# acids-ircam/RAVE

Measured on AMD Instinct MI355X. Metric: audio samples/sec/GPU (RAVE v2 training step, 44.1 kHz, n_signal=65536), higher is better.
Workload: dtype f32; 1 GPU; v2 config, batch 32 mono 44.1 kHz n_signal=65536, VAE-phase training step per GPU (--phase vae); global_batch=32, parallelism=dp1, phase=vae

## Files before the change

### include/rave_hip.h

```cpp
#ifndef RAVE_HIP_H
#define RAVE_HIP_H

#include <stddef.h>
#include <stdint.h>

#ifdef __cplusplus
extern "C" {
#endif

#define RH_VERSION 100

#define RH_OK 0
#define RH_ERR_INVALID (-1)
#define RH_ERR_UNSUPPORTED (-2)
#define RH_ERR_WORKSPACE (-3)

typedef void* rh_stream_t;

enum rh_act {
    RH_ACT_NONE = 0,
    RH_ACT_LEAKY = 1,
    RH_ACT_SNAKE = 2
};

typedef struct rh_conv1d_desc {
    int32_t batch;
    int32_t c_in;
    int32_t c_out;
    int32_t l_in;
    int32_t l_out;
    int32_t kernel;
    int32_t stride;
    int32_t dilation;
    int32_t pad_left;
    int32_t transposed;
    int32_t groups;
    int32_t inner;
    int32_t in_valid;
    int32_t act;
    float act_slope;
    int32_t out_act;
    float out_slope;
} rh_conv1d_desc;

int rh_version(void);
const char* rh_last_error(void);



int rh_weight_norm_fwd_f32(const float* v, const float* g, int64_t rows, int64_t cols, float* w,
                           float* norms, rh_stream_t stream);
int rh_weight_norm_bwd_f32(const float* dw, const float* v, const float* g, const float* norms,
                           int64_t rows, int64_t cols, float* dv, float* dg, rh_stream_t stream);
typedef struct rh_wn_bwd_item {
    const float* dw;
    const float* v;
    const float* g;
    const float* norms;
    float* dv;
    float* dg;
    int64_t rows;
    int64_t cols;
} rh_wn_bwd_item;
int rh_weight_norm_bwd_batched_f32(const rh_wn_bwd_item* items, int32_t n_items, rh_stream_t stream);
typedef struct rh_reduce_item {
    const float* part;
    float* out;
    int64_t n;
    int32_t Z;
    int32_t reserved;
} rh_reduce_item;
int rh_defer_reduce(rh_reduce_item* item);
int rh_reduce_partials_batched_f32(const rh_reduce_item* items, int32_t n_items, rh_stream_t stream);

int64_t rh_conv1d_packed_floats(const rh_conv1d_desc* d, int which);
int rh_conv1d_pack_f32(const rh_conv1d_desc* d, const float* w, float* wp_fwd, float* wp_bwd,
                       rh_stream_t stream);

int rh_conv1d_pack_wn_f32(const rh_conv1d_desc* d, const float* v, const float* g, float* norms,
                          float* scale, float* wp_fwd, float* wp_bwd, rh_stream_t stream);

int64_t rh_prep_item_bytes(void);
int64_t rh_prep_array_bytes(int32_t n);
int rh_prep_fill_item(const rh_conv1d_desc* d, const float* v, const float* g, float* norms, float* scale,
                      float* wp_fwd, float* wp_bwd, void* item_host);
int rh_prep_link(void* items_host, int32_t n, int64_t* total_rows, int64_t* total_blocks);
int rh_prep_run_f32(const void* items_dev, int32_t n, int64_t total_rows, int64_t total_blocks, rh_stream_t stream);


int rh_conv1d_fwd_f32(const rh_conv1d_desc* d, const float* x, const float* wp_fwd,
                      const float* bias, const float* snake_alpha, const float* residual,
                      float* y, void* workspace, int64_t workspace_bytes, rh_stream_t stream);
int64_t rh_conv1d_fwd_workspace_bytes(const rh_conv1d_desc* d);
int64_t rh_conv1d_bwd_data_workspace_bytes(const rh_conv1d_desc* d);
int rh_conv1d_kernel_family(const rh_conv1d_desc* d, int which, int has_bias, int has_add);
int rh_residual_unit_fused(const rh_conv1d_desc* d3, const rh_conv1d_desc* d1);
int rh_residual_unit_fwd_f32(const rh_conv1d_desc* d3, const rh_conv1d_desc* d1, const float* x, const float* wp3_fwd,
                             const float* wp1_fwd, float* h, float* y, rh_stream_t stream);

int rh_x6_uses_ranges(void);
int rh_x6_range_words(void);
int rh_x6_set_ranges(const uint32_t* in_a, const uint32_t* in_b, uint32_t* out, uint32_t* out2);
int rh_amax_f32(const float* x, int64_t n, uint32_t* slot, rh_stream_t stream);

int rh_conv1d_plan_info(const rh_conv1d_desc* d, int which, int has_bias, int has_add, int32_t* out8);
int rh_conv1d_bwd_weight_kernel_family(const rh_conv1d_desc* d);
int rh_conv1d_bwd_weight_plan_info(const rh_conv1d_desc* d, int32_t* out4);

int rh_conv1d_bwd_data_f32(const rh_conv1d_desc* d, const float* dy, const float* wp_bwd,
                           const float* x, const float* snake_alpha, const float* add, float* dx,
                           void* workspace, int64_t workspace_bytes, rh_stream_t stream);

int64_t rh_conv1d_workspace_bytes(const rh_conv1d_desc* d);
int rh_conv1d_bwd_weight_f32(const rh_conv1d_desc* d, const float* dy, const float* x,
                             const float* snake_alpha, float* dw, float* dbias, void* workspace,
                             int64_t workspace_bytes, rh_stream_t stream);
int rh_conv1d_bwd_weight_wn_f32(const rh_conv1d_desc* d, const float* dy, const float* x, const float* snake_alpha,
                                const float* v, const float* g, const float* norms, float* dw_scratch, float* dv,
                                float* dg, float* dbias, void* workspace, int64_t workspace_bytes, rh_stream_t stream);
int64_t rh_conv1d_bwd_weight_wn_fused_launches(void);


int rh_pqmf_analysis_fwd_f32(const float* x, const float* w, int32_t rows, int32_t t_len,
                             int32_t n_band, int32_t kernel, int32_t pad_left, int32_t n_frames,
                             float* y, rh_stream_t stream);
int rh_pqmf_analysis_bwd_f32(const float* dy, const float* w, int32_t rows, int32_t t_len,
                             int32_t n_band, int32_t kernel, int32_t pad_left, int32_t n_frames,
                             float* dx, rh_stream_t stream);
int rh_pqmf_synthesis_fwd_f32(const float* y, const float* w, int32_t rows, int32_t n_frames,
                              int32_t n_band, int32_t kernel, int32_t pad_left, int32_t n_out,
                              float* x, rh_stream_t stream);
int rh_pqmf_synthesis_bwd_f32(const float* dx, const float* w, int32_t rows, int32_t n_frames,
                              int32_t n_band, int32_t kernel, int32_t pad_left, int32_t n_out,
                              float* dy, rh_stream_t stream);

int rh_pqmf_fold_k1_f32(const float* in, const float* tab, int32_t rows, int32_t t_len, int32_t n_frames, int32_t o0,
                        float scale, float* out, rh_stream_t stream);
int rh_pqmf_fold_k2_f32(const float* in, const float* tab, int32_t rows, int32_t n_frames, int32_t n_out, int32_t dp,
                        float scale, float* out, rh_stream_t stream);


int rh_amp_tanh_fwd_f32(const float* x, int32_t batch, int32_t c, int32_t l, float* y,
                        rh_stream_t stream);
int rh_amp_tanh_bwd_f32(const float* dy, const float* x, int32_t batch, int32_t c, int32_t l,
                        float* dx, rh_stream_t stream);
int rh_act_fwd_f32(const float* x, const float* snake_alpha, int32_t act, float slope,
                   int32_t batch, int32_t c, int32_t l, float* y, rh_stream_t stream);
int64_t rh_snake_bwd_workspace_bytes(int32_t batch, int32_t c);
int rh_snake_bwd_f32(const float* dy, const float* x, const float* alpha, int32_t batch, int32_t c,
                     int32_t l, float* dx, float* dalpha, void* workspace, int64_t workspace_bytes,
                     rh_stream_t stream);
int rh_act_bwd_f32(const float* dy, const float* y, int32_t act, float slope, int64_t n, float* g, rh_stream_t stream);
int64_t rh_act_bwd_bias_workspace_bytes(int32_t M);
int rh_act_bwd_bias_f32(const float* dy, const float* y, int32_t act, float slope, int32_t B, int32_t M, int64_t plane, float* g,
                        float* dbias, void* workspace, int64_t workspace_bytes, rh_stream_t stream);
int rh_adain_stats_update_f32(const float* x, int64_t rows, int32_t l, const float* num_updates, float* mean_buf,
                              float* std_buf, rh_stream_t stream);
int rh_adain_transfer_f32(const float* x, int64_t rows, int32_t l, const float* mean_x, const float* std_x,
                          const float* mean_y, const float* std_y, float* y, rh_stream_t stream);
int rh_avgpool2_fwd_f32(const float* x, int64_t rows, int32_t l_in, float* y, rh_stream_t stream);
int rh_avgpool2_bwd_f32(const float* dy, int64_t rows, int32_t l_in, float* dx, rh_stream_t stream);


typedef struct rh_conv2d_desc {
    int32_t batch;
    int32_t c_in;
    int32_t c_out;
    int32_t h_in, w_in;
    int32_t h_out, w_out;
    int32_t kh, kw;
    int32_t sh, sw;
    int32_t dh, dw;
    int32_t ph, pw;
    int32_t act;
    float act_slope;
} rh_conv2d_desc;

int64_t rh_conv2d_packed_floats(const rh_conv2d_desc* d, int which);
int rh_conv2d_pack_f32(const rh_conv2d_desc* d, const float* w, float* wp_fwd, float* wp_bwd, rh_stream_t stream);
int rh_conv2d_fwd_f32(const rh_conv2d_desc* d, const float* x, const float* wp_fwd, const float* bias ,
                      float* y, rh_stream_t stream);
int rh_conv2d_bwd_data_f32(const rh_conv2d_desc* d, const float* dy, const float* y, const float* wp_bwd, float* dx,
                           rh_stream_t stream);
int rh_conv2d_plan_info(const rh_conv2d_desc* d, int32_t which, int64_t* out);
int rh_conv2d_bwd_weight_kernel_family(const rh_conv2d_desc* d);
int64_t rh_conv2d_workspace_bytes(const rh_conv2d_desc* d);
int rh_conv2d_bwd_weight_f32(const rh_conv2d_desc* d, const float* dy, const float* y, const float* x, float* dw,
                             float* dbias, void* workspace, int64_t workspace_bytes, rh_stream_t stream);


int64_t rh_vq_loss_partials(int64_t n_vectors);
int rh_vq_assign_f32(const float* x, const float* embed, int64_t n_vectors, int32_t dim, int32_t codebook_size,
                     int64_t* indices, float* residual, float* quantized_sum, float* loss_partials, rh_stream_t stream);
int64_t rh_vq_assign_workspace_bytes(int64_t n_vectors, int32_t dim, int32_t codebook_size);
int rh_vq_assign_ws_f32(const float* x, const float* embed, int64_t n_vectors, int32_t dim, int32_t codebook_size,
                        int64_t* indices, float* residual, float* quantized_sum, float* loss_partials, void* workspace,
                        int64_t workspace_bytes, rh_stream_t stream);
int rh_vq_ema_update_f32(const float* x, const int64_t* indices, int64_t n_vectors, int32_t dim, int32_t codebook_size,
                         float decay, float epsilon, float* cluster_size, float* embed_avg, float* embed,
                         rh_stream_t stream);


int rh_feed_batch_i16_f32(const int16_t* pcm, const int64_t* src_offset, const double* coef, const float* noise,
                          int32_t rows, int32_t n_signal, int32_t bit_depth, float* out, rh_stream_t stream);

typedef struct rh_feed_pitch_row {
    int64_t base;
    int64_t in_point;
    double mean;
    double coef[5];
    int32_t length;
    int32_t up, down;
    int32_t tap_offset;
    int32_t mute;
    int32_t reserved;
} rh_feed_pitch_row;
int rh_feed_batch_pitch_i16_f32(const int16_t* pcm, int64_t pcm_samples, const rh_feed_pitch_row* rows,
                                const rh_feed_pitch_row* rows_dev, const double* taps, int32_t n_taps, const float* noise,
                                int32_t n_rows, int32_t n_signal, int32_t bit_depth, float* out, rh_stream_t stream);


int rh_stft_frame_fwd_f32(const float* x, const float* window, int64_t rows, int32_t t_len, int32_t n_fft,
                          int32_t hop, int32_t n_frames, float* frames, rh_stream_t stream);
int rh_stft_frame_bwd_f32(const float* dframes, const float* window, int64_t rows, int32_t t_len, int32_t n_fft,
                          int32_t hop, int32_t n_frames, float* dx, rh_stream_t stream);
int rh_stft_frame_bwd_acc_f32(const float* dframes, const float* window, int64_t rows, int32_t t_len, int32_t n_fft,
                              int32_t hop, int32_t n_frames, float* dx, int32_t accumulate, rh_stream_t stream);

int64_t rh_spectral_distance_workspace_bytes(void);
int rh_spectral_distance_fwd_f32(const float* sx, const float* sy, int64_t n_complex, float eps, float* sums,
                                 void* workspace, int64_t workspace_bytes, rh_stream_t stream);
int rh_spectral_distance_bwd_f32(const float* sx, const float* sy, const float* sums, const float* grad_out,
                                 int64_t n_complex, float eps, float* dsx, float* dsy, int32_t half_bins,
                                 rh_stream_t stream);

int rh_spectral_total_f32(const float* sums, const float* inv_n, int32_t n_scales, float* out, rh_stream_t stream);

int rh_stft_loss_supported(int32_t n_fft, int32_t hop, int32_t t_len, int64_t rows);
int rh_stft_loss_plan_info(int32_t n_fft, int32_t t_len, int64_t rows, int64_t* out6);
int64_t rh_stft_loss_workspace_bytes(int32_t n_fft, int32_t t_len, int64_t rows);
int rh_stft_loss_fwd_f32(const float* x, const float* y, const float* window, const float* twiddle, int64_t rows,
                         int32_t t_len, int32_t n_fft, float eps, float* sums, void* workspace, int64_t workspace_bytes,
                         rh_stream_t stream);
int rh_stft_loss_finalize_all_f32(const float* const* partials, const int64_t* partial_bytes, int32_t n_scales,
                                  const float* inv_n, float* sums, float* total, rh_stream_t stream);
int rh_stft_loss_bwd_f32(const float* x, const float* y, const float* window, const float* twiddle, int64_t rows,
                         int32_t t_len, int32_t n_fft, float eps, const float* sums, const float* grad_out, float* dx,
                         float* dy, int32_t accumulate, rh_stream_t stream);

int rh_mel_supported(int32_t n_fft, int32_t hop, int32_t n_mels, int32_t t_len, int64_t rows);
int rh_mel_fwd_f32(const float* x, const float* window, const float* twiddle, const float* fb, const int32_t* bins,
                   int64_t rows, int32_t t_len, int32_t n_fft, int32_t hop, int32_t n_mels, int32_t n_frames, float scale,
                   int32_t log1p, float* y, rh_stream_t stream);

int rh_set_kernel_events(void* start_event, void* stop_event);
int rh_kernel_events_used(void);
int rh_event_create(void** event);
int rh_event_destroy(void* event);
int rh_event_elapsed_ms(void* start_event, void* stop_event, float* ms);

typedef struct rh_loss_item {
    const float* value;
    const float* w1_dev;
    float w1;
    float w2;
} rh_loss_item;
int rh_loss_combine_fwd_f32(const rh_loss_item* items, int32_t n_items, float* scaled, float* total, rh_stream_t stream);
int rh_loss_combine_bwd_f32(const rh_loss_item* items, int32_t n_items, const float* grad_total, float* grads,
                            rh_stream_t stream);

typedef struct rh_adam_item {
    float* p;
    const float* g;
    float* m;
    float* v;
    int64_t n;
    float* step;
} rh_adam_item;
int rh_adam_step_f32(const rh_adam_item* items, int32_t n_items, const float* lr, float beta1, float beta2, float eps,
                     float* aux, rh_stream_t stream);

typedef struct rh_pair_item {
    float* a;
    float* b;
    int64_t n;
} rh_pair_item;
int rh_ema_update_f32(const rh_pair_item* items, int32_t n_items, double factor, rh_stream_t stream);
int rh_swap_f32(const rh_pair_item* items, int32_t n_items, rh_stream_t stream);

typedef struct rh_gru_item {
    const float* w_ih;
    const float* w_hh;
    const float* b_ih;
    const float* b_hh;
    float* dw_ih;
    float* dw_hh;
    float* db_ih;
    float* db_hh;
} rh_gru_item;
int rh_gru_supported(int32_t hidden, int32_t layers);
int rh_gru_workspace_bytes(int32_t batch, int32_t hidden, int32_t t_len, int32_t layers, int32_t training, int64_t* bytes);
int rh_gru_fwd_f32(const float* x, const rh_gru_item* layers, int32_t n_layers, int32_t batch, int32_t hidden, int32_t t_len,
                   int32_t training, float* y, void* workspace, int64_t workspace_bytes, rh_stream_t stream);
int rh_gru_bwd_f32(const float* dy, const float* x, const rh_gru_item* layers, int32_t n_layers, int32_t batch, int32_t hidden,
                   int32_t t_len, float* dx, void* workspace, int64_t workspace_bytes, rh_stream_t stream);

typedef struct rh_fm_item {
    const float* f;
    float* df;
    int64_t half;
    float w;
} rh_fm_item;
int64_t rh_feature_matching_workspace_bytes(const rh_fm_item* items, int32_t n_items);
int rh_feature_matching_fwd_f32(const rh_fm_item* items, int32_t n_items, int32_t relative, void* workspace,
                                int64_t workspace_bytes, float* sums, float* out, rh_stream_t stream);
int rh_feature_matching_bwd_f32(const rh_fm_item* items, int32_t n_items, int32_t relative, const float* sums,
                                const float* grad_out, rh_stream_t stream);

int64_t rh_reparam_workspace_bytes(void);
int rh_reparam_fwd_f32(const float* z, const float* eps, int32_t batch, int32_t c, int32_t l, float* zs, float* kl,
                       void* workspace, int64_t workspace_bytes, rh_stream_t stream);
int rh_reparam_bwd_f32(const float* z, const float* eps, const float* dzs, const float* dkl, int32_t batch, int32_t c,
                       int32_t l, float* dz, rh_stream_t stream);

#ifdef __cplusplus
}
#endif
#endif
```

### rave_amd/_lib.py

```python
from __future__ import annotations

import ctypes as C
import os

import torch

_HERE = os.path.dirname(os.path.abspath(__file__))
LIB_PATH = os.environ.get("RAVE_HIP_LIB") or os.path.join(_HERE, "librave_hip.so")

ACT_NONE, ACT_LEAKY, ACT_SNAKE = 0, 1, 2


class ConvDesc(C.Structure):
    _fields_ = [
        ("batch", C.c_int32), ("c_in", C.c_int32), ("c_out", C.c_int32),
        ("l_in", C.c_int32), ("l_out", C.c_int32), ("kernel", C.c_int32),
        ("stride", C.c_int32), ("dilation", C.c_int32), ("pad_left", C.c_int32),
        ("transposed", C.c_int32), ("groups", C.c_int32), ("inner", C.c_int32),
        ("in_valid", C.c_int32), ("act", C.c_int32), ("act_slope", C.c_float),
        ("out_act", C.c_int32), ("out_slope", C.c_float),
    ]


class AdamItem(C.Structure):
    _fields_ = [("p", C.c_void_p), ("g", C.c_void_p), ("m", C.c_void_p), ("v", C.c_void_p), ("n", C.c_int64), ("step", C.c_void_p)]


class PairItem(C.Structure):
    _fields_ = [("a", C.c_void_p), ("b", C.c_void_p), ("n", C.c_int64)]


class GruItem(C.Structure):
    _fields_ = [(n, C.c_void_p) for n in ("w_ih", "w_hh", "b_ih", "b_hh", "dw_ih", "dw_hh", "db_ih", "db_hh")]


class WnBwdItem(C.Structure):
    _fields_ = [("dw", C.c_void_p), ("v", C.c_void_p), ("g", C.c_void_p), ("norms", C.c_void_p), ("dv", C.c_void_p),
                ("dg", C.c_void_p), ("rows", C.c_int64), ("cols", C.c_int64)]


class ReduceItem(C.Structure):
    _fields_ = [("part", C.c_void_p), ("out", C.c_void_p), ("n", C.c_int64), ("Z", C.c_int32), ("reserved", C.c_int32)]


class LossItem(C.Structure):
    _fields_ = [("value", C.c_void_p), ("w1_dev", C.c_void_p), ("w1", C.c_float), ("w2", C.c_float)]


class FmItem(C.Structure):
    _fields_ = [("f", C.c_void_p), ("df", C.c_void_p), ("half", C.c_int64), ("w", C.c_float)]


class Conv2dDesc(C.Structure):
    _fields_ = [(n, C.c_int32) for n in (
        "batch", "c_in", "c_out", "h_in", "w_in", "h_out", "w_out", "kh", "kw", "sh", "sw", "dh", "dw", "ph", "pw",
        "act")] + [("act_slope", C.c_float)]


def _load() -> C.CDLL:
    if not os.path.exists(LIB_PATH):
        raise RuntimeError(
            f"rave_amd: {LIB_PATH} not found. Build it with `python -m rave_amd.build` "
            "(or __graft_entry__.build()). There is no CPU / PyTorch fallback for the HIP hot path.")
    lib = C.CDLL(LIB_PATH)
    P, I32, I64, F = C.c_void_p, C.c_int32, C.c_int64, C.c_float
    D = C.POINTER(ConvDesc)
    D2 = C.POINTER(Conv2dDesc)
    sig = {
        "rh_version": ([], C.c_int),
        "rh_last_error": ([], C.c_char_p),
        "rh_weight_norm_fwd_f32": ([P, P, I64, I64, P, P, P], C.c_int),
        "rh_weight_norm_bwd_f32": ([P, P, P, P, I64, I64, P, P, P], C.c_int),
        "rh_weight_norm_bwd_batched_f32": ([C.POINTER(WnBwdItem), I32, P], C.c_int),
        "rh_defer_reduce": ([C.POINTER(ReduceItem)], C.c_int),
        "rh_reduce_partials_batched_f32": ([C.POINTER(ReduceItem), I32, P], C.c_int),
        "rh_conv1d_packed_floats": ([D, C.c_int], I64),
        "rh_conv1d_pack_f32": ([D, P, P, P, P], C.c_int),
        "rh_conv1d_pack_wn_f32": ([D, P, P, P, P, P, P, P], C.c_int),
        "rh_prep_item_bytes": ([], I64),
        "rh_prep_array_bytes": ([I32], I64),
        "rh_prep_fill_item": ([D, P, P, P, P, P, P, P], C.c_int),
        "rh_prep_link": ([P, I32, C.POINTER(I64), C.POINTER(I64)], C.c_int),
        "rh_prep_run_f32": ([P, I32, I64, I64, P], C.c_int),
        "rh_conv1d_fwd_f32": ([D, P, P, P, P, P, P, P, I64, P], C.c_int),
        "rh_conv1d_bwd_data_f32": ([D, P, P, P, P, P, P, P, I64, P], C.c_int),
        "rh_conv1d_kernel_family": ([D, C.c_int, C.c_int, C.c_int], C.c_int),
        "rh_conv1d_bwd_weight_kernel_family": ([D], C.c_int),
        "rh_conv1d_bwd_weight_plan_info": ([D, C.POINTER(C.c_int32)], C.c_int),
        "rh_residual_unit_fused": ([D, D], C.c_int),
        "rh_residual_unit_fwd_f32": ([D, D, P, P, P, P, P, P], C.c_int),
        "rh_conv1d_plan_info": ([D, C.c_int, C.c_int, C.c_int, C.POINTER(C.c_int32)], C.c_int),
        "rh_conv1d_fwd_workspace_bytes": ([D], I64),
        "rh_conv1d_bwd_data_workspace_bytes": ([D], I64),
        "rh_conv1d_workspace_bytes": ([D], I64),
        "rh_conv1d_bwd_weight_f32": ([D, P, P, P, P, P, P, I64, P], C.c_int),
        "rh_conv1d_bwd_weight_wn_f32": ([D, P, P, P, P, P, P, P, P, P, P, P, I64, P], C.c_int),
        "rh_conv1d_bwd_weight_wn_fused_launches": ([], I64),
        "rh_conv2d_packed_floats": ([D2, C.c_int], I64),
        "rh_conv2d_pack_f32": ([D2, P, P, P, P], C.c_int),
        "rh_conv2d_fwd_f32": ([D2, P, P, P, P, P], C.c_int),
        "rh_conv2d_bwd_data_f32": ([D2, P, P, P, P, P], C.c_int),
        "rh_conv2d_workspace_bytes": ([D2], I64),
        "rh_conv2d_plan_info": ([D2, I32, C.POINTER(I64)], C.c_int),
        "rh_conv2d_bwd_weight_kernel_family": ([D2], C.c_int),
        "rh_conv2d_bwd_weight_f32": ([D2, P, P, P, P, P, P, I64, P], C.c_int),
        "rh_feed_batch_i16_f32": ([P, P, P, P, I32, I32, I32, P, P], C.c_int),
        "rh_feed_batch_pitch_i16_f32": ([P, I64, P, P, P, I32, P, I32, I32, I32, P, P], C.c_int),
        "rh_vq_loss_partials": ([I64], I64),
        "rh_vq_assign_f32": ([P, P, I64, I32, I32, P, P, P, P, P], C.c_int),
        "rh_vq_assign_workspace_bytes": ([I64, I32, I32], I64),
        "rh_vq_assign_ws_f32": ([P, P, I64, I32, I32, P, P, P, P, P, I64, P], C.c_int),
        "rh_vq_ema_update_f32": ([P, P, I64, I32, I32, F, F, P, P, P, P], C.c_int),
        "rh_pqmf_analysis_fwd_f32": ([P, P, I32, I32, I32, I32, I32, I32, P, P], C.c_int),
        "rh_pqmf_analysis_bwd_f32": ([P, P, I32, I32, I32, I32, I32, I32, P, P], C.c_int),
        "rh_pqmf_synthesis_fwd_f32": ([P, P, I32, I32, I32, I32, I32, I32, P, P], C.c_int),
        "rh_pqmf_synthesis_bwd_f32": ([P, P, I32, I32, I32, I32, I32, I32, P, P], C.c_int),
        "rh_pqmf_fold_k1_f32": ([P, P, I32, I32, I32, I32, F, P, P], C.c_int),
        "rh_pqmf_fold_k2_f32": ([P, P, I32, I32, I32, I32, F, P, P], C.c_int),
        "rh_amp_tanh_fwd_f32": ([P, I32, I32, I32, P, P], C.c_int),
        "rh_amp_tanh_bwd_f32": ([P, P, I32, I32, I32, P, P], C.c_int),
        "rh_act_fwd_f32": ([P, P, I32, F, I32, I32, I32, P, P], C.c_int),
        "rh_act_bwd_f32": ([P, P, I32, F, I64, P, P], C.c_int),
        "rh_act_bwd_bias_workspace_bytes": ([I32], I64),
        "rh_act_bwd_bias_f32": ([P, P, I32, F, I32, I32, I64, P, P, P, I64, P], C.c_int),
        "rh_snake_bwd_workspace_bytes": ([I32, I32], I64),
        "rh_snake_bwd_f32": ([P, P, P, I32, I32, I32, P, P, P, I64, P], C.c_int),
        "rh_stft_frame_fwd_f32": ([P, P, I64, I32, I32, I32, I32, P, P], C.c_int),
        "rh_stft_frame_bwd_f32": ([P, P, I64, I32, I32, I32, I32, P, P], C.c_int),
        "rh_stft_frame_bwd_acc_f32": ([P, P, I64, I32, I32, I32, I32, P, I32, P], C.c_int),
        "rh_spectral_total_f32": ([P, P, I32, P, P], C.c_int),
        "rh_feature_matching_workspace_bytes": ([C.POINTER(FmItem), I32], I64),
        "rh_feature_matching_fwd_f32": ([C.POINTER(FmItem), I32, I32, P, I64, P, P, P], C.c_int),
        "rh_feature_matching_bwd_f32": ([C.POINTER(FmItem), I32, I32, P, P, P], C.c_int),
        "rh_reparam_workspace_bytes": ([], I64),
        "rh_reparam_fwd_f32": ([P, P, I32, I32, I32, P, P, P, I64, P], C.c_int),
        "rh_reparam_bwd_f32": ([P, P, P, P, I32, I32, I32, P, P], C.c_int),
        "rh_loss_combine_fwd_f32": ([C.POINTER(LossItem), I32, P, P, P], C.c_int),
        "rh_loss_combine_bwd_f32": ([C.POINTER(LossItem), I32, P, P, P], C.c_int),
        "rh_adam_step_f32": ([C.POINTER(AdamItem), I32, P, F, F, F, P, P], C.c_int),
        "rh_ema_update_f32": ([C.POINTER(PairItem), I32, C.c_double, P], C.c_int),
        "rh_swap_f32": ([C.POINTER(PairItem), I32, P], C.c_int),
        "rh_gru_supported": ([I32, I32], C.c_int),
        "rh_gru_workspace_bytes": ([I32, I32, I32, I32, I32, C.POINTER(I64)], C.c_int),
        "rh_gru_fwd_f32": ([P, C.POINTER(GruItem), I32, I32, I32, I32, I32, P, P, I64, P], C.c_int),
        "rh_gru_bwd_f32": ([P, P, C.POINTER(GruItem), I32, I32, I32, I32, P, P, I64, P], C.c_int),
        "rh_x6_uses_ranges": ([], C.c_int),
        "rh_x6_range_words": ([], C.c_int),
        "rh_x6_set_ranges": ([P, P, P, P], C.c_int),
        "rh_amax_f32": ([P, I64, P, P], C.c_int),
        "rh_set_kernel_events": ([P, P], C.c_int),
        "rh_kernel_events_used": ([], C.c_int),
        "rh_event_create": ([C.POINTER(C.c_void_p)], C.c_int),
        "rh_event_destroy": ([P], C.c_int),
        "rh_event_elapsed_ms": ([P, P, C.POINTER(C.c_float)], C.c_int),
        "rh_stft_loss_supported": ([I32, I32, I32, I64], C.c_int),
        "rh_stft_loss_plan_info": ([I32, I32, I64, C.POINTER(I64)], C.c_int),
        "rh_stft_loss_workspace_bytes": ([I32, I32, I64], I64),
        "rh_stft_loss_fwd_f32": ([P, P, P, P, I64, I32, I32, F, P, P, I64, P], C.c_int),
        "rh_stft_loss_finalize_all_f32": ([C.POINTER(C.c_void_p), C.POINTER(I64), I32, P, P, P, P], C.c_int),
        "rh_stft_loss_bwd_f32": ([P, P, P, P, I64, I32, I32, F, P, P, P, P, I32, P], C.c_int),
        "rh_mel_supported": ([I32, I32, I32, I32, I64], C.c_int),
        "rh_mel_fwd_f32": ([P, P, P, P, P, I64, I32, I32, I32, I32, I32, F, I32, P, P], C.c_int),
        "rh_spectral_distance_workspace_bytes": ([], I64),
        "rh_spectral_distance_fwd_f32": ([P, P, I64, F, P, P, I64, P], C.c_int),
        "rh_spectral_distance_bwd_f32": ([P, P, P, P, I64, F, P, P, I32, P], C.c_int),
        "rh_adain_stats_update_f32": ([P, I64, I32, P, P, P, P], C.c_int),
        "rh_adain_transfer_f32": ([P, I64, I32, P, P, P, P, P, P], C.c_int),
        "rh_avgpool2_fwd_f32": ([P, I64, I32, P, P], C.c_int),
        "rh_avgpool2_bwd_f32": ([P, I64, I32, P, P], C.c_int),
    }
    for name, (args, res) in sig.items():
        fn = getattr(lib, name)
        fn.argtypes = args
        fn.restype = res
    return lib


lib = _load()


def check(rc: int, what: str = "") -> None:
    if rc != 0:
        msg = lib.rh_last_error().decode(errors="replace")
        raise RuntimeError(f"librave_hip {what} failed (code {rc}): {msg}")


def ptr(t) -> int | None:
    return None if t is None else t.data_ptr()


def stream() -> int:
    return torch.cuda.current_stream().cuda_stream
```

### rave_amd/csrc/conv_host.hip

```cpp
#include "conv_params.hpp"

int64_t rh_wgrad_workspace(const rh_conv1d_desc* d);

namespace {

struct TapPlan {
    int nphase = 0;
    int oph[kMaxPhases], ntaps[kMaxPhases], tap0[kMaxPhases], minoff[kMaxPhases], maxoff[kMaxPhases];
    int nslots = 0;
    int kk[kMaxTaps], off[kMaxTaps];
    int is = 1, os = 1;
    int rows = 0;
    int C = 0, M = 0;
    bool src_m_major = true;
};

int validate(const rh_conv1d_desc* d) {
    RH_REQUIRE(d, RH_ERR_INVALID, "conv1d: null descriptor");
    RH_REQUIRE(d->batch >= 0 && d->c_in > 0 && d->c_out > 0 && d->l_in >= 0 && d->l_out >= 0,
               RH_ERR_INVALID, "conv1d: bad sizes");
    RH_REQUIRE(d->kernel >= 1 && d->stride >= 1 && d->dilation >= 1 && d->inner >= 1,
               RH_ERR_INVALID, "conv1d: kernel/stride/dilation/inner must be >= 1");
    RH_REQUIRE(d->groups == 1, RH_ERR_UNSUPPORTED, "conv1d: groups = %d not implemented", d->groups);
    RH_REQUIRE(d->kernel <= kMaxTaps, RH_ERR_UNSUPPORTED, "conv1d: kernel %d > %d", d->kernel, kMaxTaps);
    RH_REQUIRE(d->act >= RH_ACT_NONE && d->act <= RH_ACT_SNAKE, RH_ERR_INVALID, "conv1d: bad act");
    RH_REQUIRE(d->out_act == RH_ACT_NONE || d->out_act == RH_ACT_LEAKY, RH_ERR_UNSUPPORTED,
               "conv1d: out_act must be none or leaky");
    RH_REQUIRE(d->in_valid >= 0 && d->in_valid <= (int64_t)d->l_in * d->inner, RH_ERR_INVALID,
               "conv1d: in_valid out of range");
    if (d->transposed) {
        RH_REQUIRE(d->dilation == 1 && d->inner == 1, RH_ERR_UNSUPPORTED,
                   "conv_transpose1d: dilation/inner must be 1");
        RH_REQUIRE(d->stride <= kMaxPhases, RH_ERR_UNSUPPORTED, "conv_transpose1d: stride > %d", kMaxPhases);
    } else if (d->stride > 1) {
        RH_REQUIRE(d->stride <= kMaxPhases, RH_ERR_UNSUPPORTED, "conv1d: stride > %d", kMaxPhases);
    }
    return RH_OK;
}

int build_plan(const rh_conv1d_desc* d, int which, TapPlan* tp) {
    TapPlan& t = *tp;
    const int k = d->kernel, s = d->stride, dil = d->dilation, P = d->pad_left;
    auto phases = [&](int pad) {
        t.nphase = s;
        t.is = 1;
        t.os = s;
        for (int ph = 0; ph < s; ++ph) {
            const int r0 = ((ph + pad) % s + s) % s;
            const int base = (ph + pad - r0) / s;
            t.oph[ph] = ph;
            t.tap0[ph] = t.nslots;
            int n = 0;
            for (int m = 0; r0 + m * s < k; ++m, ++n) {
                t.kk[t.nslots] = r0 + m * s;
                t.off[t.nslots] = base - m;
                ++t.nslots;
            }
            t.ntaps[ph] = n;
        }
    };
    auto single = [&]() {
        t.nphase = 1;
        t.oph[0] = 0;
        t.tap0[0] = 0;
        t.ntaps[0] = k;
        t.nslots = k;
    };
    if (which == 0) {
        t.C = d->c_in;
        t.M = d->c_out;
        if (!d->transposed) {
            single();
            for (int i = 0; i < k; ++i) { t.kk[i] = i; t.off[i] = i * dil - P; }
            t.is = s; t.os = 1; t.rows = d->l_out;
            t.src_m_major = true;
        } else {
            phases(P);
            t.rows = rh_cdiv(d->l_out, s);
            t.src_m_major = false;
        }
    } else {
        t.C = d->c_out;
        t.M = d->c_in;
        if (!d->transposed) {
            if (s == 1) {
                single();
                for (int i = 0; i < k; ++i) { t.kk[i] = i; t.off[i] = P - i * dil; }
                t.is = 1; t.os = 1; t.rows = d->l_in;
            } else {
                RH_REQUIRE(dil == 1, RH_ERR_UNSUPPORTED, "conv1d bwd_data: stride > 1 with dilation > 1");
                phases(P);
                t.rows = rh_cdiv(d->l_in, s);
            }
            t.src_m_major = false;
        } else {
            single();
            for (int i = 0; i < k; ++i) { t.kk[i] = i; t.off[i] = i - P; }
            t.is = s; t.os = 1; t.rows = d->l_in;
            t.src_m_major = true;
        }
    }
    for (int ph = 0; ph < t.nphase; ++ph) {
        int lo = 0, hi = 0;
        for (int i = 0; i < t.ntaps[ph]; ++i) {
            const int o = t.off[t.tap0[ph] + i];
            if (i == 0 || o < lo) lo = o;
            if (i == 0 || o > hi) hi = o;
        }
        t.minoff[ph] = lo;
        t.maxoff[ph] = hi;
    }
    return RH_OK;
}

inline int round32(int m) { return (m + 31) & ~31; }

void plan_to_params(const TapPlan& t, ConvP* p) {
    p->C = t.C;
    p->M = t.M;
    p->Mp = round32(t.M);
    p->is = t.is;
    p->os = t.os;
    p->nphase = t.nphase;
    long wofs = 0;
    for (int ph = 0; ph < t.nphase; ++ph) {
        p->ph_oph[ph] = t.oph[ph];
        p->ph_ntaps[ph] = t.ntaps[ph];
        p->ph_tap0[ph] = t.tap0[ph];
        p->ph_minoff[ph] = t.minoff[ph];
        p->ph_maxoff[ph] = t.maxoff[ph];
        p->ph_wofs[ph] = wofs;
        wofs += (long)t.ntaps[ph] * t.C * p->Mp;
    }
    for (int i = 0; i < t.nslots; ++i) p->off[i] = t.off[i];
}

struct VPlan { int s, U, phstar, o0, b0, jof[kMaxPhases]; };
bool vplan_of(const TapPlan& t, int inner, VPlan* v) {
    static const bool on = [] { const char* e = getenv("RH_X6_VROWS"); return !(e && atoi(e) == 0); }();
    const int s = t.nphase;
    if (!on || (s != 2 && s != 4) || t.os != s || t.is != 1 || inner != 1 || (t.C & 15) || ((t.M * s) & 31)) return false;
    int U = 0;
    for (int ph = 0; ph < s; ++ph) {
        if (t.ntaps[ph] < 1) return false;
        for (int m = 0; m < t.ntaps[ph]; ++m)
            if (t.off[t.tap0[ph] + m] != t.off[t.tap0[ph]] - m) return false;
        U = U > t.ntaps[ph] ? U : t.ntaps[ph];
    }
    const int b0 = t.off[t.tap0[0]];
    int phstar = 0;
    for (int ph = 0; ph < s; ++ph) {
        const int b = t.off[t.tap0[ph]];
        if (b == b0 + 1) { if (!phstar) phstar = ph; }
        else if (b != b0 || phstar) return false;
    }
    v->s = s; v->U = U; v->phstar = phstar; v->b0 = b0;
    v->o0 = phstar ? phstar - s : 0;
    for (int ph = 0; ph < s; ++ph) v->jof[ph] = (ph - phstar + s) % s;
    return true;
}

int x6_mode_of(const TapPlan& t, int inner) {
    return rh_x6_mode(t.C, t.nphase, t.is, inner, t.ntaps[0], t.off, t.kk);
}
long x6_units(const TapPlan& t, int mode, long* ph_ofs = nullptr, int inner = 1, long* vofs = nullptr) {
    const long Mp = round32(t.M);
    if (vofs) *vofs = -1;
    if (mode == 0) return 0;
    if (mode == 1) {
        long u = 0;
        for (int ph = 0; ph < t.nphase; ++ph) {
            if (ph_ofs) ph_ofs[ph] = u;
            u += (long)(t.C >> 4) * t.ntaps[ph] * 2 * kX6P * Mp;
        }
        VPlan v;
        if (vplan_of(t, inner, &v)) {
            if (vofs) *vofs = u;
            u += (long)(t.C >> 4) * v.U * 2 * kX6P * round32(t.M * v.s);
        }
        return u;
    }
    if (ph_ofs) ph_ofs[0] = 0;
    return (long)((t.C * mode) >> 4) * rh_cdiv(t.ntaps[0], mode) * 2 * kX6P * Mp;
}
void plan_to_x6(const TapPlan& t, int inner, ConvP* p) {
    p->x6_mode = x6_mode_of(t, inner);
    long vofs = -1;
    long units = x6_units(t, p->x6_mode, p->ph_q2ofs, inner, &vofs);
    if (units * 4 >= 0x7fffffffl) { p->x6_mode = 0; units = 0; vofs = -1; }
    p->x6_nu = p->x6_mode > 1 ? rh_cdiv(t.ntaps[0], p->x6_mode) : 0;
    p->vs = 0;
    p->v_s = 0;
    if (vofs >= 0) {
        VPlan v;
        vplan_of(t, inner, &v);
        p->v_s = v.s; p->v_q2ofs = vofs;
        p->v_o0 = v.o0; p->v_U = v.U; p->v_b0 = v.b0;
    }
    p->x6_wofs = (long)t.nslots * t.C * round32(t.M);
    p->wq_bytes = units * 16 < 0xffffffffl ? (unsigned)(units * 16) : 0xffffffffu;
}

constexpr int kPackSlots = 4;

__host__ __device__ __forceinline__ long pack_tiles(const PackP& q) {
    return q.total ? (long)(q.Mp / 32) * ((q.C + 31) / 32) : 0;
}

__device__ __forceinline__ void emit_fragment_bf3(const float (&v)[8], unsigned* dst, long piece_stride_u32) {
    typedef unsigned u32x4 __attribute__((ext_vector_type(4)));
    unsigned h[3][8];
#pragma unroll
    for (int i = 0; i < 8; ++i) {
        rh_bf3_split(v[i], h[0][i], h[1][i], h[2][i]);
        h[0][i] &= 0xffff0000u; h[1][i] &= 0xffff0000u; h[2][i] &= 0xffff0000u;
    }
#pragma unroll
    for (int s3 = 0; s3 < 3; ++s3) {
        u32x4 pk;
#pragma unroll
        for (int k = 0; k < 4; ++k) pk[k] = (h[s3][2 * k] >> 16) | h[s3][2 * k + 1];
        *reinterpret_cast<u32x4*>(dst + s3 * piece_stride_u32) = pk;
    }
}
__device__ __forceinline__ void emit_fragment(const float (&v)[8], unsigned* dst, long piece_stride_u32, float sc) {
    typedef unsigned u32x4 __attribute__((ext_vector_type(4)));
#if RH_X6_F16
    u32x4 hi, lo;
#pragma unroll
    for (int k = 0; k < 4; ++k) {
        const rh_h2 h = rh_h2_split(v[2 * k] * sc, v[2 * k + 1] * sc);
        hi[k] = h.hi; lo[k] = h.lo;
    }
    *reinterpret_cast<u32x4*>(dst) = hi;
    *reinterpret_cast<u32x4*>(dst + piece_stride_u32) = lo;
#else
    unsigned h[3][8];
#pragma unroll
    for (int i = 0; i < 8; ++i) {
        rh_bf3_split(v[i], h[0][i], h[1][i], h[2][i]);
        h[0][i] &= 0xffff0000u; h[1][i] &= 0xffff0000u; h[2][i] &= 0xffff0000u;
    }
#pragma unroll
    for (int s3 = 0; s3 < 3; ++s3) {
        u32x4 pk;
#pragma unroll
        for (int k = 0; k < 4; ++k) pk[k] = (h[s3][2 * k] >> 16) | h[s3][2 * k + 1];
        *reinterpret_cast<u32x4*>(dst + s3 * piece_stride_u32) = pk;
    }
#endif
}

__device__ __forceinline__ void pack_tile(const PackP& q, long tile, float* lds , int sg = 0, int sn = 1) {
    const int ct = (q.C + 31) / 32;
    const int c0 = (int)(tile % ct) * 32;
    const int m0 = (int)(tile / ct) * 32;
    const int tid = threadIdx.x;
    float fsc = 1.f;
#if RH_X6_F16
    if (q.wq && !q.bf16x3) {
        int inv;
        fsc = __uint_as_float(rh_x6_scale_bits(q.range[0], &inv));
    }
#endif
    for (int s0 = sg * kPackSlots; s0 < q.nslots; s0 += sn * kPackSlots) {
        const int ns = min(kPackSlots, q.nslots - s0);
        constexpr int U = 8;
        int kks[kPackSlots];
#pragma unroll
        for (int j = 0; j < kPackSlots; ++j) kks[j] = q.kk[min(s0 + j, q.nslots - 1)];
        const int total = ns * 1024;
        for (int e0 = tid; e0 < total; e0 += 256 * U) {
            float v[U], sc[U];
            int dst[U];
#pragma unroll
            for (int u = 0; u < U; ++u) {
                const int e = e0 + 256 * u;
                int sl, r;
                if (ns == 4) { sl = e & 3; r = e >> 2; }
                else if (ns == 3) { r = e / 3; sl = e - 3 * r; }
                else if (ns == 2) { sl = e & 1; r = e >> 1; }
                else { sl = 0; r = e; }
                int cl, ml;
                if (q.m_major) { cl = r & 31; ml = r >> 5; }
                else { ml = r & 31; cl = r >> 5; }
                const int m = m0 + ml, c = c0 + cl;
                const bool in = e < total;
                const bool ok = in && m < q.M && c < q.C;
                const int kk = sl == 0 ? kks[0] : (sl == 1 ? kks[1] : (sl == 2 ? kks[2] : kks[3]));
                const long idx = q.m_major ? ((long)m * q.C + c) * q.k + kk : ((long)c * q.M + m) * q.k + kk;
                v[u] = ok ? q.w[idx] : 0.f;
                sc[u] = (ok && q.scale) ? q.scale[q.m_major ? m : c] : 1.f;
                dst[u] = in ? (sl * 32 + cl) * 33 + ml : -1;
            }
#pragma unroll
            for (int u = 0; u < U; ++u)
                if (dst[u] >= 0) lds[dst[u]] = v[u] * sc[u];
        }
        __syncthreads();
        for (int e = tid; e < ns * 1024; e += 256) {
            const int ml = e & 31, cl = (e >> 5) & 31, sl = e >> 10;
            const int c = c0 + cl;
            if (c < q.C) q.wp[((long)(s0 + sl) * q.C + c) * q.Mp + m0 + ml] = lds[(sl * 32 + cl) * 33 + ml];
        }
        if (q.wq && q.x6_mode == 1) {
            for (int e = tid; e < ns * 128; e += 256) {
                const int ml = e & 31, oct = (e >> 5) & 3, sl = e >> 7;
                const int cb = c0 + oct * 8;
                if (cb >= q.C) continue;
                float v[8];
#pragma unroll
                for (int i = 0; i < 8; ++i) v[i] = lds[(sl * 32 + oct * 8 + i) * 33 + ml];
                const int slot = s0 + sl;
                if (q.bf16x3) {
                    const long unit3 = (long)q.q2a[slot] + (long)(cb >> 4) * q.q2n[slot] + (long)(((cb >> 3) & 1) * 3) * q.Mp + m0 + ml;
                    emit_fragment_bf3(v, q.wq + unit3 * 4, (long)q.Mp * 4);
                    continue;
                }
                const long unit = (long)q.q2a[slot] + (long)(cb >> 4) * q.q2n[slot] + (long)(((cb >> 3) & 1) * kX6P) * q.Mp + m0 + ml;
                emit_fragment(v, q.wq + unit * 4, (long)q.Mp * 4, fsc);
            }
        }
        if (q.wq && q.x6_vs > 1) {
            const int vs = q.x6_vs;
            for (int e = tid; e < ns * 128; e += 256) {
                const int ml = e & 31, oct = (e >> 5) & 3, sl = e >> 7;
                const int cb = c0 + oct * 8;
                const int r = (m0 + ml) * vs + q.q2j[s0 + sl];
                if (cb >= q.C || r >= q.x6_Mvp) continue;
                float v[8];
#pragma unroll
                for (int i = 0; i < 8; ++i) v[i] = lds[(sl * 32 + oct * 8 + i) * 33 + ml];
                const int slot = s0 + sl;
                const long unit = q.x6_vofs + q.vq2a[slot] + (long)(cb >> 4) * q.x6_U * 2 * kX6P * q.x6_Mvp + (long)(((cb >> 3) & 1) * kX6P) * q.x6_Mvp + r;
                emit_fragment(v, q.wq + unit * 4, (long)q.x6_Mvp * 4, fsc);
            }
            if (s0 == 0) {
                const float zero[8] = {0.f, 0.f, 0.f, 0.f, 0.f, 0.f, 0.f, 0.f};
                for (int e = tid; e < q.vz_n * 128; e += 256) {
                    const int ml = e & 31, oct = (e >> 5) & 3, zi = e >> 7;
                    const int cb = c0 + oct * 8;
                    const int r = (m0 + ml) * vs + q.vz_j[zi];
                    if (cb >= q.C || r >= q.x6_Mvp) continue;
                    const long unit = q.x6_vofs + (long)q.vz_u[zi] * 2 * kX6P * q.x6_Mvp + (long)(cb >> 4) * q.x6_U * 2 * kX6P * q.x6_Mvp +
                                      (long)(((cb >> 3) & 1) * kX6P) * q.x6_Mvp + r;
                    emit_fragment(zero, q.wq + unit * 4, (long)q.x6_Mvp * 4, fsc);
                }
            }
        }
        if (q.wq && q.x6_mode > 1) {
            const int IS = q.x6_mode, cpc = 16 / IS, nvc = 32 / cpc;
            const int nug = (ns + IS - 1) / IS;
            for (int e = tid; e < nug * nvc * 64; e += 256) {
                const int ml = e & 31, g = (e >> 5) & 1;
                const int r = e >> 6;
                const int cv = r % nvc, ul = r / nvc;
                const int cbase = c0 + cv * cpc;
                if (cbase >= q.C) continue;
                float v[8];
#pragma unroll
                for (int i = 0; i < 8; ++i) {
                    const int kap = 8 * g + i;
                    const int cl = cv * cpc + kap / IS, sl = ul * IS + kap % IS;
                    v[i] = sl < ns ? lds[(sl * 32 + cl) * 33 + ml] : 0.f;
                }
                const long unit = ((long)(cbase / cpc) * q.x6_nu + (s0 / IS + ul)) * 2 * kX6P * q.Mp + (long)(g * kX6P) * q.Mp + m0 + ml;
                emit_fragment(v, q.wq + unit * 4, (long)q.Mp * 4, fsc);
            }
        }
        __syncthreads();
    }
}

__global__ __launch_bounds__(256) void pack_kernel(const PackP a, const PackP b) {
    __shared__ float lds[kPackSlots * 32 * 33];
    const long t = blockIdx.x;
    const long na = pack_tiles(a);
    if (t < na) pack_tile(a, t, lds, blockIdx.y, gridDim.y);
    else if (t - na < pack_tiles(b)) pack_tile(b, t - na, lds, blockIdx.y, gridDim.y);
}

inline unsigned pack_slot_groups(const PackP& a, const PackP& b, long tiles) {
    if (tiles >= 64) return 1;
    const int ns = a.nslots > b.nslots ? a.nslots : b.nslots;
    const int g = (ns + kPackSlots - 1) / kPackSlots;
    return (unsigned)(g < 1 ? 1 : (g > 8 ? 8 : g));
}

int fill_pack(const rh_conv1d_desc* d, int which, const float* w, const float* scale, float* wp, PackP* p) {
    *p = PackP{};
    if (!wp) return RH_OK;
    TapPlan t;
    if (int e = build_plan(d, which, &t)) return e;
    p->w = w; p->scale = scale; p->wp = wp; p->C = t.C; p->M = t.M; p->Mp = round32(t.M); p->k = d->kernel;
    p->m_major = t.src_m_major ? 1 : 0;
    p->total = (long)t.nslots * t.C * p->Mp;
    p->nslots = t.nslots;
    for (int i = 0; i < t.nslots; ++i) p->kk[i] = t.kk[i];
    const int mode = x6_mode_of(t, d->inner);
    long ph_ofs[kMaxPhases];
    long vofs = -1;
    const long units = x6_units(t, mode, ph_ofs, d->inner, &vofs);
    if (mode && units * 4 < 0x7fffffffl) {
        p->wq = reinterpret_cast<unsigned*>(wp + p->total);
        p->range = p->wq + units * 4;
        p->x6_mode = mode;
        if (vofs >= 0) {
            VPlan v;
            vplan_of(t, d->inner, &v);
            p->x6_vs = v.s;
            p->x6_vofs = vofs;
            p->x6_U = v.U;
            p->x6_Mvp = round32(t.M * v.s);
            bool have[kMaxPhases][kMaxTaps] = {};
            for (int ph = 0; ph < t.nphase; ++ph)
                for (int tl = 0; tl < t.ntaps[ph]; ++tl) {
                    const int slot = t.tap0[ph] + tl;
                    p->vq2a[slot] = tl * 2 * kX6P * p->x6_Mvp;
                    p->q2j[slot] = v.jof[ph];
                    have[v.jof[ph]][tl] = true;
                }
            for (int j = 0; j < v.s; ++j)
                for (int u = 0; u < v.U; ++u)
                    if (!have[j][u]) {
                        RH_REQUIRE(p->vz_n < 2 * kMaxPhases, RH_ERR_UNSUPPORTED, "conv1d_pack: too many empty (phase, tap) pairs");
                        p->vz_j[p->vz_n] = j; p->vz_u[p->vz_n] = u; ++p->vz_n;
                    }
        }
        if (mode == 1) {
            for (int ph = 0; ph < t.nphase; ++ph)
                for (int tl = 0; tl < t.ntaps[ph]; ++tl) {
                    p->q2a[t.tap0[ph] + tl] = (int)(ph_ofs[ph] + (long)tl * 2 * kX6P * p->Mp);
                    p->q2n[t.tap0[ph] + tl] = t.ntaps[ph] * 2 * kX6P * p->Mp;
                }
        } else {
            p->x6_nu = rh_cdiv(t.ntaps[0], mode);
        }
    }
    return RH_OK;
}

__global__ __launch_bounds__(256) void pack_range_kernel(const float* __restrict__ w, const float* __restrict__ scale, long cols,
                                                         unsigned* ra, unsigned* rb) {
    __shared__ float red[8];
    const long r = blockIdx.x;
    const float* wr = w + r * cols;
    float mx = 0.f, sm = 0.f;
    for (long e = threadIdx.x; e < cols; e += 256) { const float a = fabsf(wr[e]); mx = fmaxf(mx, a); sm += a; }
#pragma unroll
    for (int o = 32; o > 0; o >>= 1) { mx = fmaxf(mx, __shfl_down(mx, o, 64)); sm += __shfl_down(sm, o, 64); }
    if ((threadIdx.x & 63) == 0) { red[threadIdx.x >> 6] = mx; red[4 + (threadIdx.x >> 6)] = sm; }
    __syncthreads();
    if (threadIdx.x == 0) {
        const float sc = scale ? fabsf(scale[r]) : 1.f;
        const float m = sc * fmaxf(fmaxf(red[0], red[1]), fmaxf(red[2], red[3]));
        const float l1 = sc * ((red[4] + red[5]) + (red[6] + red[7]));
        if (ra) { atomicMax(ra, __float_as_uint(m)); atomicMax(ra + 1, __float_as_uint(l1)); }
        if (rb) { atomicMax(rb, __float_as_uint(m)); atomicMax(rb + 1, __float_as_uint(l1)); }
    }
}

int pack_both(const rh_conv1d_desc* d, const float* w, const float* scale, float* wp_fwd, float* wp_bwd,
              hipStream_t stream) {
    PackP a, b;
    if (int e = fill_pack(d, 0, w, scale, wp_fwd, &a)) return e;
    if (int e = fill_pack(d, 1, w, scale, wp_bwd, &b)) return e;
    const long tiles = pack_tiles(a) + pack_tiles(b);
    if (tiles == 0) return RH_OK;
    if (a.range || b.range) {
        if (a.range && hipMemsetAsync(a.range, 0, 16, stream) != hipSuccess) return rh_check_launch("conv1d_pack_range");
        if (b.range && hipMemsetAsync(b.range, 0, 16, stream) != hipSuccess) return rh_check_launch("conv1d_pack_range");
        const long rows = d->transposed ? d->c_in : d->c_out;
        const long cols = (long)(d->transposed ? d->c_out : d->c_in) * d->kernel;
        hipLaunchKernelGGL(pack_range_kernel, dim3((unsigned)rows), dim3(256), 0, stream, w, scale, cols, a.range, b.range);
        if (int e = rh_check_launch("conv1d_pack_range")) return e;
    }
    hipLaunchKernelGGL(pack_kernel, dim3((unsigned)tiles, pack_slot_groups(a, b, tiles)), dim3(256), 0, stream, a, b);
    return rh_check_launch("conv1d_pack");
}

}

int rh_pack_launch(const PackP& a, const PackP& b, hipStream_t stream, const char* what, const float* w, long rows, long cols) {
    const long tiles = pack_tiles(a) + pack_tiles(b);
    if (tiles == 0) return RH_OK;
    if (w && (a.range || b.range)) {
        if (a.range && hipMemsetAsync(a.range, 0, 16, stream) != hipSuccess) return rh_check_launch(what);
        if (b.range && hipMemsetAsync(b.range, 0, 16, stream) != hipSuccess) return rh_check_launch(what);
        hipLaunchKernelGGL(pack_range_kernel, dim3((unsigned)rows), dim3(256), 0, stream, w, (const float*)nullptr, cols, a.range, b.range);
        if (int e = rh_check_launch(what)) return e;
    }
    hipLaunchKernelGGL(pack_kernel, dim3((unsigned)tiles, pack_slot_groups(a, b, tiles)), dim3(256), 0, stream, a, b);
    return rh_check_launch(what);
}

int rh_conv_fill_fwd(const rh_conv1d_desc* d, ConvP* p) {
    if (int e = validate(d)) return e;
    TapPlan t;
    if (int e = build_plan(d, 0, &t)) return e;
    plan_to_params(t, p);
    p->B = d->batch;
    p->inner = d->inner;
    const int in_full = d->l_in * d->inner;
    p->in_valid = d->in_valid ? d->in_valid : in_full;
    p->in_row = p->in_valid;
    p->out_row = d->l_out * d->inner;
    p->out_valid = p->out_row;
    p->ncols = t.rows * d->inner;
    p->in_act = d->act;
    p->in_slope = d->act_slope;
    p->epi_act = RH_ACT_NONE;
    p->epi_slope = 0.f;
    p->out_act = d->out_act;
    p->out_slope = d->out_slope;
    plan_to_x6(t, d->inner, p);
    return RH_OK;
}

int rh_conv_fill_dgrad(const rh_conv1d_desc* d, ConvP* p) {
    if (int e = validate(d)) return e;
    TapPlan t;
    if (int e = build_plan(d, 1, &t)) return e;
    plan_to_params(t, p);
    p->B = d->batch;
    p->inner = d->inner;
    p->in_row = d->l_out * d->inner;
    p->in_valid = p->in_row;
    const int x_full = d->l_in * d->inner;
    p->out_valid = d->in_valid ? d->in_valid : x_full;
    p->out_row = p->out_valid;
    p->ncols = t.rows * d->inner;
    p->in_act = RH_ACT_NONE;
    p->in_slope = 0.f;
    p->epi_act = d->act;
    p->epi_slope = d->act_slope;
    p->out_act = RH_ACT_NONE;
    p->out_slope = 0.f;
    plan_to_x6(t, d->inner, p);
    return RH_OK;
}

extern "C" int64_t rh_conv1d_packed_floats(const rh_conv1d_desc* d, int which) {
    if (validate(d)) return -1;
    const int64_t M = which == 0 ? d->c_out : d->c_in;
    const int64_t C = which == 0 ? d->c_in : d->c_out;
    const int64_t n32 = (int64_t)d->kernel * C * round32((int)M);
    TapPlan t;
    if (build_plan(d, which, &t)) return -1;
    const long units = x6_units(t, x6_mode_of(t, d->inner), nullptr, d->inner);
    return (units > 0 && units * 4 < 0x7fffffffl) ? n32 + units * 4 + 4 : n32;
}

extern "C" int rh_conv1d_pack_f32(const rh_conv1d_desc* d, const float* w, float* wp_fwd,
                                  float* wp_bwd, rh_stream_t stream) {
    if (int e = validate(d)) return e;
    RH_REQUIRE(w, RH_ERR_INVALID, "conv1d_pack: null weight");
    return pack_both(d, w, nullptr, wp_fwd, wp_bwd, (hipStream_t)stream);
}

int rh_weight_norm_scales(const float* v, const float* g, int64_t rows, int64_t cols, float* norms, float* scale,
                          hipStream_t stream);

struct PrepItem {
    const float* v;
    const float* g;
    float* norms;
    float* scale;
    PackP fwd, bwd;
    long rows, cols;
    long row_begin;
    long blk_begin;
};

namespace {

__device__ __forceinline__ int find_item(const PrepItem* items, int n, long key, bool rows) {
    const long* tab = reinterpret_cast<const long*>(items + n) + (rows ? 0 : n);
    int lo = 0, hi = n - 1;
    while (lo < hi) {
        const int mid = (lo + hi + 1) >> 1;
        if (tab[mid] <= key) lo = mid; else hi = mid - 1;
    }
    return lo;
}

__global__ __launch_bounds__(256) void prep_range_kernel(const PrepItem* __restrict__ items, int n) {
    __shared__ float red[8];
    const PrepItem& p = items[blockIdx.x];
    float mx = 0.f, l1 = 0.f;
    for (long r = threadIdx.x; r < p.rows; r += 256) { mx = fmaxf(mx, p.scale[p.rows + r]); l1 = fmaxf(l1, p.scale[2 * p.rows + r]); }
#pragma unroll
    for (int o = 32; o > 0; o >>= 1) { mx = fmaxf(mx, __shfl_down(mx, o, 64)); l1 = fmaxf(l1, __shfl_down(l1, o, 64)); }
    if ((threadIdx.x & 63) == 0) { red[threadIdx.x >> 6] = mx; red[4 + (threadIdx.x >> 6)] = l1; }
    __syncthreads();
    if (threadIdx.x == 0) {
        const unsigned m = __float_as_uint(fmaxf(fmaxf(red[0], red[1]), fmaxf(red[2], red[3])));
        const unsigned l = __float_as_uint(fmaxf(fmaxf(red[4], red[5]), fmaxf(red[6], red[7])));
        for (unsigned* r : {p.fwd.range, p.bwd.range})
            if (r) { r[0] = m; r[1] = l; r[2] = 0u; r[3] = 0u; }
    }
}

__global__ __launch_bounds__(256) void prep_scales_kernel(const PrepItem* __restrict__ items, int n) {
    __shared__ float red[12];
    const int it = find_item(items, n, blockIdx.x, true);
    const PrepItem& p = items[it];
    const long r = (long)blockIdx.x - p.row_begin;
    const float* vr = p.v + r * p.cols;
    float s = 0.f, mx = 0.f, sm = 0.f;
    long e = threadIdx.x;
    for (; e + 768 < p.cols; e += 1024) {
        const float a0 = vr[e], a1 = vr[e + 256], a2 = vr[e + 512], a3 = vr[e + 768];
        s += a0 * a0; s += a1 * a1; s += a2 * a2; s += a3 * a3;
        mx = fmaxf(fmaxf(mx, fmaxf(fabsf(a0), fabsf(a1))), fmaxf(fabsf(a2), fabsf(a3)));
        sm += fabsf(a0); sm += fabsf(a1); sm += fabsf(a2); sm += fabsf(a3);
    }
    for (; e < p.cols; e += 256) {
        const float a = vr[e];
        s += a * a;
        mx = fmaxf(mx, fabsf(a));
        sm += fabsf(a);
    }
#pragma unroll
    for (int o = 32; o > 0; o >>= 1) {
        s += __shfl_down(s, o, 64);
        mx = fmaxf(mx, __shfl_down(mx, o, 64));
        sm += __shfl_down(sm, o, 64);
    }
    if ((threadIdx.x & 63) == 0) { red[threadIdx.x >> 6] = s; red[4 + (threadIdx.x >> 6)] = mx; red[8 + (threadIdx.x >> 6)] = sm; }
    __syncthreads();
    if (threadIdx.x == 0) {
        const float norm = sqrtf(red[0] + red[1] + red[2] + red[3]);
        const float sc = p.g[r] / norm;
        p.norms[r] = norm;
        p.scale[r] = sc;
        const float m = fabsf(sc) * fmaxf(fmaxf(red[4], red[5]), fmaxf(red[6], red[7]));
        const float l1 = fabsf(sc) * ((red[8] + red[9]) + (red[10] + red[11]));
        p.scale[p.rows + r] = m;
        p.scale[2 * p.rows + r] = l1;
    }
}

__global__ __launch_bounds__(256) void prep_pack_kernel(const PrepItem* __restrict__ items, int n) {
    __shared__ float lds[kPackSlots * 32 * 33];
    const int it = find_item(items, n, blockIdx.x, false);
    const PrepItem& p = items[it];
    const long t = (long)blockIdx.x - p.blk_begin;
    const long nf = pack_tiles(p.fwd);
    if (t < nf) pack_tile(p.fwd, t, lds);
    else if (t - nf < pack_tiles(p.bwd)) pack_tile(p.bwd, t - nf, lds);
}

}

extern "C" int64_t rh_prep_item_bytes(void) { return (int64_t)sizeof(PrepItem); }
extern "C" int64_t rh_prep_array_bytes(int32_t n) { return (int64_t)n * (int64_t)sizeof(PrepItem) + 2 * (int64_t)n * (int64_t)sizeof(long); }

extern "C" int rh_prep_fill_item(const rh_conv1d_desc* d, const float* v, const float* g, float* norms, float* scale,
                                 float* wp_fwd, float* wp_bwd, void* item) {
    if (int e = validate(d)) return e;
    RH_REQUIRE(v && g && norms && scale && wp_fwd && item, RH_ERR_INVALID, "prep_fill_item: null pointer");
    PrepItem* p = (PrepItem*)item;
    *p = PrepItem{};
    p->v = v; p->g = g; p->norms = norms; p->scale = scale;
    p->rows = d->transposed ? d->c_in : d->c_out;
    p->cols = (long)(d->transposed ? d->c_out : d->c_in) * d->kernel;
    if (int e = fill_pack(d, 0, v, scale, wp_fwd, &p->fwd)) return e;
    if (int e = fill_pack(d, 1, v, scale, wp_bwd, &p->bwd)) return e;
    return RH_OK;
}

extern "C" int rh_prep_link(void* items, int32_t n, int64_t* total_rows, int64_t* total_blocks) {
    RH_REQUIRE(items && total_rows && total_blocks && n >= 0, RH_ERR_INVALID, "prep_link: bad arguments");
    PrepItem* p = (PrepItem*)items;
    long rows = 0, blks = 0;
    for (int i = 0; i < n; ++i) {
        p[i].row_begin = rows;
        p[i].blk_begin = blks;
        rows += p[i].rows;
        for (const PackP* q : {&p[i].fwd, &p[i].bwd}) blks += pack_tiles(*q);
    }
    long* tab = reinterpret_cast<long*>(p + n);
    for (int i = 0; i < n; ++i) { tab[i] = p[i].row_begin; tab[n + i] = p[i].blk_begin; }
    *total_rows = rows;
    *total_blocks = blks;
    return RH_OK;
}

extern "C" int rh_prep_run_f32(const void* items_dev, int32_t n, int64_t total_rows, int64_t total_blocks,
                               rh_stream_t stream) {
    RH_REQUIRE(items_dev && n > 0, RH_ERR_INVALID, "prep_run: bad arguments");
    if (total_rows > 0) {
        hipLaunchKernelGGL(prep_scales_kernel, dim3((unsigned)total_rows), dim3(256), 0, (hipStream_t)stream,
                           (const PrepItem*)items_dev, n);
        if (int e = rh_check_launch("prep_scales")) return e;
        hipLaunchKernelGGL(prep_range_kernel, dim3((unsigned)n), dim3(256), 0, (hipStream_t)stream, (const PrepItem*)items_dev, n);
        if (int e = rh_check_launch("prep_range")) return e;
    }
    if (total_blocks > 0) {
        hipLaunchKernelGGL(prep_pack_kernel, dim3((unsigned)total_blocks), dim3(256), 0, (hipStream_t)stream,
                           (const PrepItem*)items_dev, n);
        return rh_check_launch("prep_pack");
    }
    return RH_OK;
}

extern "C" int rh_conv1d_pack_wn_f32(const rh_conv1d_desc* d, const float* v, const float* g, float* norms,
                                     float* scale, float* wp_fwd, float* wp_bwd, rh_stream_t stream) {
    if (int e = validate(d)) return e;
    RH_REQUIRE(v && g && norms && scale, RH_ERR_INVALID, "conv1d_pack_wn: null pointer");
    const int64_t rows = d->transposed ? d->c_in : d->c_out;
    const int64_t cols = (int64_t)(d->transposed ? d->c_out : d->c_in) * d->kernel;
    if (int e = rh_weight_norm_scales(v, g, rows, cols, norms, scale, (hipStream_t)stream)) return e;
    return pack_both(d, v, scale, wp_fwd, wp_bwd, (hipStream_t)stream);
}

extern "C" int64_t rh_conv1d_fwd_workspace_bytes(const rh_conv1d_desc* d) {
    ConvP p{};
    if (rh_conv_fill_fwd(d, &p)) return -1;
    return rh_conv_splitk_workspace(p);
}

extern "C" int64_t rh_conv1d_bwd_data_workspace_bytes(const rh_conv1d_desc* d) {
    ConvP p{};
    if (rh_conv_fill_dgrad(d, &p)) return -1;
    p.epi_act = d->act;
    return rh_conv_splitk_workspace(p);
}

extern "C" int rh_conv1d_kernel_family(const rh_conv1d_desc* d, int which, int has_bias, int has_add) {
    ConvP p{};
    if (int e = which == 0 ? rh_conv_fill_fwd(d, &p) : rh_conv_fill_dgrad(d, &p)) return e;
    if (which == 0 ? rh_smallc_fwd_eligible(d, has_add != 0) : rh_smallc_dgrad_eligible(d, has_add != 0)) return 2;
    alignas(16) static const float dummy[4] = {0.f, 0.f, 0.f, 0.f};
    p.in = dummy; p.wp = dummy; p.wq = reinterpret_cast<const unsigned*>(dummy);
    p.bias = has_bias ? dummy : nullptr;
    p.add = has_add ? dummy : nullptr;
    p.mul_src = (which == 1 && d->act != RH_ACT_NONE) ? dummy : nullptr;
    if (p.B <= 0 || p.ncols <= 0 || p.M <= 0 || !rh_conv_dma_eligible(p)) return 0;
    return (rh_conv_x6_workspace(p) >= 0 || rh_conv_c2x_query(p)) ? 1 : 0;
}

extern "C" int rh_conv1d_plan_info(const rh_conv1d_desc* d, int which, int has_bias, int has_add, int32_t* out8) {
    RH_REQUIRE(out8, RH_ERR_INVALID, "conv1d_plan_info: null output");
    for (int i = 0; i < 8; ++i) out8[i] = 0;
    ConvP p{};
    if (int e = which == 0 ? rh_conv_fill_fwd(d, &p) : rh_conv_fill_dgrad(d, &p)) return e;
    if (which == 0 ? rh_smallc_fwd_eligible(d, has_add != 0) : rh_smallc_dgrad_eligible(d, has_add != 0)) { out8[0] = 2; return RH_OK; }
    alignas(16) static const float dummy[4] = {0.f, 0.f, 0.f, 0.f};
    p.in = dummy; p.wp = dummy; p.wq = reinterpret_cast<const unsigned*>(dummy);
    p.bias = has_bias ? dummy : nullptr;
    p.add = has_add ? dummy : nullptr;
    p.mul_src = (which == 1 && d->act != RH_ACT_NONE) ? dummy : nullptr;
    if (p.B <= 0 || p.ncols <= 0 || p.M <= 0 || !rh_conv_dma_eligible(p)) return RH_OK;
    int q[7];
    if (rh_conv_x6_plan_query(p, q)) {
        out8[0] = 1;
        for (int i = 0; i < 7; ++i) out8[i + 1] = q[i];
    }
    return RH_OK;
}

extern "C" int rh_conv1d_fwd_f32(const rh_conv1d_desc* d, const float* x, const float* wp_fwd,
                                 const float* bias, const float* snake_alpha, const float* residual,
                                 float* y, void* workspace, int64_t workspace_bytes, rh_stream_t stream) {
    const RhKernelEventsScope events;
    ConvP p{};
    rh_take_ranges(nullptr, &p.in_range, &p.out_range, nullptr);
    const unsigned* const in_range = p.in_range;
    unsigned* const out_range = p.out_range;
    if (int e = rh_conv_fill_fwd(d, &p)) return e;
    p.in_range = in_range; p.out_range = out_range;
    if (d->batch == 0 || d->l_out == 0) return RH_OK;
    RH_REQUIRE(x && wp_fwd && y, RH_ERR_INVALID, "conv1d_fwd: null pointer");
    RH_REQUIRE(d->act != RH_ACT_SNAKE || snake_alpha, RH_ERR_INVALID, "conv1d_fwd: snake needs alpha");
    if (rh_smallc_fwd_eligible(d, residual != nullptr)) {
        return rh_smallc_fwd(d, x, wp_fwd, bias, y, (hipStream_t)stream, p.out_range);
    }
    p.in = x; p.wp = wp_fwd; p.out = y; p.bias = bias; p.add = residual; p.mul_src = nullptr;
    p.wq = reinterpret_cast<const unsigned*>(wp_fwd + p.x6_wofs);
    p.in_alpha = snake_alpha; p.mul_alpha = nullptr;
    return rh_conv_launch(p, (hipStream_t)stream, d->transposed ? "conv_transpose1d_fwd" : "conv1d_fwd", workspace,
                          workspace_bytes);
}

extern "C" int rh_conv1d_bwd_data_f32(const rh_conv1d_desc* d, const float* dy, const float* wp_bwd,
                                      const float* x, const float* snake_alpha, const float* add,
                                      float* dx, void* workspace, int64_t workspace_bytes,
                                      rh_stream_t stream) {
    const RhKernelEventsScope events;
    ConvP p{};
    rh_take_ranges(nullptr, &p.in_range, &p.out_range, nullptr);
    const unsigned* const in_range = p.in_range;
    unsigned* const out_range = p.out_range;
    if (int e = rh_conv_fill_dgrad(d, &p)) return e;
    p.in_range = in_range; p.out_range = out_range;
    if (d->batch == 0 || d->l_in == 0) return RH_OK;
    RH_REQUIRE(dy && wp_bwd && dx, RH_ERR_INVALID, "conv1d_bwd_data: null pointer");
    RH_REQUIRE(d->act == RH_ACT_NONE || x, RH_ERR_INVALID, "conv1d_bwd_data: act needs the forward input");
    RH_REQUIRE(d->act != RH_ACT_SNAKE || snake_alpha, RH_ERR_INVALID, "conv1d_bwd_data: snake needs alpha");
    if (rh_smallc_dgrad_eligible(d, add != nullptr)) {
        TapPlan t;
        if (int e = build_plan(d, 1, &t)) return e;
        int slot_of_tap[kMaxTaps];
        for (int i = 0; i < t.nslots; ++i) slot_of_tap[t.kk[i]] = i;
        if (int e = rh_smallc_dgrad(d, dy, wp_bwd, slot_of_tap, dx, (hipStream_t)stream)) return e;
        p.out = dx;
        return rh_range_after(p, (hipStream_t)stream);
    }
    p.in = dy; p.wp = wp_bwd; p.out = dx; p.bias = nullptr; p.add = add;
    p.wq = reinterpret_cast<const unsigned*>(wp_bwd + p.x6_wofs);
    p.mul_src = d->act == RH_ACT_NONE ? nullptr : x;
    p.in_alpha = nullptr; p.mul_alpha = snake_alpha;
    return rh_conv_launch(p, (hipStream_t)stream, d->transposed ? "conv_transpose1d_bwd_data" : "conv1d_bwd_data",
                          workspace, workspace_bytes);
}

extern "C" int64_t rh_conv1d_workspace_bytes(const rh_conv1d_desc* d) {
    if (validate(d)) return -1;
    return rh_wgrad_workspace(d);
}

extern "C" int rh_conv1d_bwd_weight_f32(const rh_conv1d_desc* d, const float* dy, const float* x,
                                        const float* snake_alpha, float* dw, float* dbias,
                                        void* workspace, int64_t workspace_bytes, rh_stream_t stream) {
    const RhKernelEventsScope events;
    const RhWgradArmed armed = rh_wgrad_take_armed(true);
    if (int e = validate(d)) return e;
    RH_REQUIRE(dw && (d->batch == 0 || (dy && x)), RH_ERR_INVALID, "conv1d_bwd_weight: null pointer");
    RH_REQUIRE(d->act != RH_ACT_SNAKE || snake_alpha, RH_ERR_INVALID, "conv1d_bwd_weight: snake needs alpha");
    return rh_wgrad_run(d, dy, x, snake_alpha, dw, dbias, workspace, workspace_bytes, (hipStream_t)stream, armed);
}

extern "C" int rh_conv1d_bwd_weight_wn_f32(const rh_conv1d_desc* d, const float* dy, const float* x, const float* snake_alpha,
                                           const float* v, const float* g, const float* norms, float* dw_scratch, float* dv,
                                           float* dg, float* dbias, void* workspace, int64_t workspace_bytes, rh_stream_t stream) {
    const RhKernelEventsScope events;
    const RhWgradArmed armed = rh_wgrad_take_armed(false);
    if (int e = validate(d)) return e;
    RH_REQUIRE(dw_scratch && v && g && norms && dv && dg && (d->batch == 0 || (dy && x)), RH_ERR_INVALID,
               "conv1d_bwd_weight_wn: null pointer");
    RH_REQUIRE(d->act != RH_ACT_SNAKE || snake_alpha, RH_ERR_INVALID, "conv1d_bwd_weight_wn: snake needs alpha");
    const RhWnTail tail{v, g, norms, dv, dg};
    return rh_wgrad_run(d, dy, x, snake_alpha, dw_scratch, dbias, workspace, workspace_bytes, (hipStream_t)stream, armed, &tail);
}
```

### rave_amd/csrc/conv_igemm.hip

```cpp
#include <mutex>
#include "conv_params.hpp"

namespace {

__device__ __forceinline__ int ibase_of(int n, int inner, int is) {
    if (inner == 1) return n * is;
    const int r = n / inner;
    return r * is * inner + (n - r * inner);
}
__device__ __forceinline__ int oidx_of(int n, int inner, int os, int oph) {
    if (inner == 1) return n * os + oph;
    const int r = n / inner;
    return (r * os + oph) * inner + (n - r * inner);
}

template <int TM, int TN, int WM, int WN>
__global__ __launch_bounds__(WM* WN * 64) void conv_igemm_kernel(const ConvP p) {
    constexpr int BM = TM * WM * 32;
    constexpr int NT = WM * WN * 64;
    constexpr int NW = WM * WN;
    extern __shared__ __attribute__((aligned(16))) float smem[];
    float* w_lds = smem;
    float* x_lds = smem + p.wlds_floats;

    const int tid = threadIdx.x, lane = tid & 63, wave = tid >> 6;
    const int j = lane & 31, kh = lane >> 5;
    const int wm = wave / WN, wn = wave - wm * WN;

    const int phase = blockIdx.z;
    const int ntaps = p.ph_ntaps[phase];
    const int tap0 = p.ph_tap0[phase];
    const int minoff = p.ph_minoff[phase];
    const int maxoff = p.ph_maxoff[phase];
    const int oph = p.ph_oph[phase];
    const float* __restrict__ wp = p.wp + p.ph_wofs[phase];

    const int bt = blockIdx.x / p.tiles_per_b;
    const int nt = blockIdx.x - bt * p.tiles_per_b;
    const int b0 = bt * p.nb;
    const int n0 = nt * p.bnl;
    const int m0 = blockIdx.y * BM;
    const int inner = p.inner, is = p.is;

    const int nlast = min(n0 + p.bnl, p.ncols) - 1;
    const int ib0 = ibase_of(n0, inner, is);
    const int lo = ib0 + minoff * inner;
    const int width = ibase_of(nlast, inner, is) - ib0 + (maxoff - minoff) * inner + 1;

    int xb[TN];
#pragma unroll
    for (int tn = 0; tn < TN; ++tn) {
        const int col = (wn * TN + tn) * 32 + j;
        const int bl = col >> p.bnl_shift;
        const int nl = col & (p.bnl - 1);
        const int n = min(n0 + nl, p.ncols - 1);
        xb[tn] = (bl * p.ck + kh) * p.pitch + ibase_of(n, inner, is) - ib0;
    }
    const int arow = wm * TM * 32 + j + kh * BM;

    f32x16 acc[TM][TN];
#pragma unroll
    for (int tm = 0; tm < TM; ++tm)
#pragma unroll
        for (int tn = 0; tn < TN; ++tn)
#pragma unroll
            for (int r = 0; r < 16; ++r) acc[tm][tn][r] = 0.f;

    for (int c0 = 0; c0 < p.C; c0 += p.ck) {
        __syncthreads();
        const int nrows = p.nb * p.ck;
        for (int r = wave; r < nrows; r += NW) {
            const int bl = r / p.ck, c = r - bl * p.ck;
            const int b = b0 + bl, ch = c0 + c;
            float* dst = x_lds + r * p.pitch;
            if (b < p.B && ch < p.C) {
                const float* __restrict__ src = p.in + ((long)b * p.C + ch) * p.in_row;
                const float alpha = (p.in_act == RH_ACT_SNAKE) ? p.in_alpha[ch] : 0.f;
                for (int w = lane; w < width; w += 64) {
                    const int f = lo + w;
                    const float v = (f >= 0 && f < p.in_valid) ? src[f] : 0.f;
                    dst[w] = rh_act_apply(v, p.in_act, p.in_slope, alpha);
                }
            } else {
                for (int w = lane; w < width; w += 64) dst[w] = 0.f;
            }
        }
        constexpr int V = BM / 4;
        const int wrows = ntaps * p.ck;
        for (int e = tid; e < wrows * V; e += NT) {
            const int kr = e / V, v4 = e - kr * V;
            const int t = kr / p.ck, c = kr - t * p.ck;
            const int ch = c0 + c;
            const int m = m0 + v4 * 4;
            f32x4 val = {0.f, 0.f, 0.f, 0.f};
            if (ch < p.C && m < p.Mp)
                val = *reinterpret_cast<const f32x4*>(wp + ((long)t * p.C + ch) * p.Mp + m);
            *reinterpret_cast<f32x4*>(w_lds + kr * BM + v4 * 4) = val;
        }
        __syncthreads();
        for (int t = 0; t < ntaps; ++t) {
            const int toff = (p.off[tap0 + t] - minoff) * inner;
            const float* wl = w_lds + t * p.ck * BM + arow;
            const float* xl = x_lds + toff;
            for (int c = 0; c < p.ck; c += 2) {
                float a[TM], b[TN];
#pragma unroll
                for (int tm = 0; tm < TM; ++tm) a[tm] = wl[c * BM + tm * 32];
#pragma unroll
                for (int tn = 0; tn < TN; ++tn) b[tn] = xl[xb[tn] + c * p.pitch];
#pragma unroll
                for (int tm = 0; tm < TM; ++tm)
#pragma unroll
                    for (int tn = 0; tn < TN; ++tn)
                        acc[tm][tn] = __builtin_amdgcn_mfma_f32_32x32x2f32(a[tm], b[tn], acc[tm][tn], 0, 0, 0);
            }
        }
    }

#pragma unroll
    for (int tn = 0; tn < TN; ++tn) {
        const int col = (wn * TN + tn) * 32 + j;
        const int bl = col >> p.bnl_shift;
        const int nl = col & (p.bnl - 1);
        const int n = n0 + nl, b = b0 + bl;
        if (n >= p.ncols || b >= p.B) continue;
        const int oi = oidx_of(n, inner, p.os, oph);
        if (oi >= p.out_valid) continue;
#pragma unroll
        for (int tm = 0; tm < TM; ++tm) {
#pragma unroll
            for (int r = 0; r < 16; ++r) {
                const int m = m0 + (wm * TM + tm) * 32 + (r & 3) + 8 * (r >> 2) + 4 * kh;
                if (m < p.M) {
                    const long idx = ((long)b * p.M + m) * p.out_row + oi;
                    float v = acc[tm][tn][r];
                    if (p.bias) v += p.bias[m];
                    if (p.mul_src) {
                        const float al = (p.epi_act == RH_ACT_SNAKE) ? p.mul_alpha[m] : 0.f;
                        v *= rh_act_grad(p.mul_src[idx], p.epi_act, p.epi_slope, al);
                    }
                    if (p.add) v += p.add[idx];
                    if (p.out_act == RH_ACT_LEAKY) v = v > 0.f ? v : v * p.out_slope;
                    p.out[idx] = v;
                }
            }
        }
    }
}

template <int TM, int TN, int WM, int WN>
int launch_cfg(ConvP& p, hipStream_t stream, const char* what) {
    constexpr int BM = TM * WM * 32, BN = TN * WN * 32;
    int bnl = BN;
    if (p.ncols < BN) {
        bnl = 32;
        while (bnl < p.ncols) bnl <<= 1;
    }
    p.bnl = bnl;
    p.bnl_shift = __builtin_ctz(bnl);
    p.nb = BN / bnl;
    p.tiles_per_b = rh_cdiv(p.ncols, bnl);
    int span = 0, maxtaps = 0;
    for (int i = 0; i < p.nphase; ++i) {
        span = span > p.ph_maxoff[i] - p.ph_minoff[i] ? span : p.ph_maxoff[i] - p.ph_minoff[i];
        maxtaps = maxtaps > p.ph_ntaps[i] ? maxtaps : p.ph_ntaps[i];
    }
    if (p.inner == 1)
        p.pitch = (bnl - 1) * p.is + span + 1;
    else
        p.pitch = ((bnl - 1) / p.inner + 1) * p.is * p.inner + p.inner + span * p.inner + 1;
    p.pitch |= 1;
    const int budget = 15 * 1024;
    const int per_ch = (maxtaps > 0 ? maxtaps : 1) * BM + p.nb * p.pitch;
    int ck = budget / per_ch;
    ck &= ~1;
    if (ck > 32) ck = 32;
    if (ck < 2) ck = 2;
    const int cmax = (p.C + 1) & ~1;
    if (ck > cmax) ck = cmax;
    p.ck = ck;
    p.wlds_floats = (maxtaps > 0 ? maxtaps : 1) * ck * BM;
    const size_t lds = sizeof(float) * ((size_t)p.wlds_floats + (size_t)p.nb * ck * p.pitch);
    RH_REQUIRE(lds <= 160 * 1024, RH_ERR_UNSUPPORTED, "%s: tile needs %zu B of LDS", what, lds);
    auto kern = conv_igemm_kernel<TM, TN, WM, WN>;
    static std::once_flag once;
    std::call_once(once, [&] {
        (void)hipFuncSetAttribute(reinterpret_cast<const void*>(kern),
                                  hipFuncAttributeMaxDynamicSharedMemorySize, 160 * 1024);
    });
    dim3 grid(rh_cdiv(p.B, p.nb) * p.tiles_per_b, rh_cdiv(p.M, BM), p.nphase);
    hipLaunchKernelGGL(kern, grid, dim3(WM * WN * 64), lds, stream, p);
    return rh_check_launch(what);
}

}

int rh_conv_launch(ConvP& p, hipStream_t stream, const char* what, void* ws, int64_t ws_bytes) {
    if (p.B <= 0 || p.ncols <= 0 || p.M <= 0) return RH_OK;
    if (rh_conv_dma_eligible(p)) return rh_conv_launch_dma(p, stream, what, ws, ws_bytes);
    return rh_conv_launch_sync(p, stream, what);
}

int rh_conv_launch_sync(ConvP& p, hipStream_t stream, const char* what) {
    if (p.B <= 0 || p.ncols <= 0 || p.M <= 0) return RH_OK;
    int rc;
    if (p.M <= 32) rc = launch_cfg<1, 2, 1, 4>(p, stream, what);
    else if (p.M <= 64) rc = launch_cfg<2, 1, 1, 4>(p, stream, what);
    else if (p.M % 96 == 0 || p.M < 96) rc = launch_cfg<3, 1, 1, 4>(p, stream, what);
    else rc = launch_cfg<2, 2, 2, 2>(p, stream, what);
    return rc ? rc : rh_range_after(p, stream);
}

int rh_range_after(const ConvP& p, hipStream_t stream) {
    if (!p.out_range) return RH_OK;
    return rh_amax_f32(p.out, (int64_t)p.B * (p.Mr > 0 && p.vs > 1 ? p.Mr : p.M) * p.out_row, p.out_range, (rh_stream_t)stream);
}
```

### rave_amd/csrc/conv_igemm_dma.hip

```cpp
#include <cstdlib>
#include <mutex>
#include <type_traits>
#include "conv_params.hpp"

namespace {

typedef __attribute__((address_space(3))) void lds_void;

#ifndef RH_READS_FIRST
#define RH_READS_FIRST 1
#endif
constexpr bool READS_FIRST = RH_READS_FIRST != 0;

__device__ __forceinline__ int ibase_of(int n, int inner, int is) {
    if (inner == 1) return n * is;
    const int r = n / inner;
    return r * is * inner + (n - r * inner);
}
__device__ __forceinline__ int oidx_of(int n, int inner, int os, int oph) {
    if (inner == 1) return n * os + oph;
    const int r = n / inner;
    return (r * os + oph) * inner + (n - r * inner);
}
__device__ __forceinline__ unsigned mdiv(unsigned n, unsigned magic) { return (n * magic) >> 20; }

constexpr unsigned kOOB = 0x80000000u;

template <int TM, int TN, int WM, int WN, bool LEAKY, bool VEC, bool CTAIL>
__global__ __launch_bounds__(WM* WN * 64) void conv_igemm_dma_kernel(const ConvP p) {
    constexpr int BM = TM * WM * 32;
    constexpr int NW = WM * WN;
    extern __shared__ __attribute__((aligned(16))) float smem[];

    const int tid = threadIdx.x, lane = tid & 63;
    const int wave = __builtin_amdgcn_readfirstlane(tid >> 6);
    const int j = lane & 31, kh = lane >> 5;
    const int wm = wave / WN, wn = wave - wm * WN;

    const int zsl = blockIdx.z / p.nphase;
    const int phase = blockIdx.z - zsl * p.nphase;
    const int ntaps = p.ph_ntaps[phase];
    const int tap0 = p.ph_tap0[phase];
    const int minoff = p.ph_minoff[phase];
    const int oph = p.ph_oph[phase];
    const unsigned wofs = (unsigned)p.ph_wofs[phase];

    const int bt = blockIdx.x / p.tiles_per_b;
    const int nt = blockIdx.x - bt * p.tiles_per_b;
    const int b0 = bt * p.nb;
    const int n0 = nt * p.bnl;
    const int m0 = blockIdx.y * BM;
    const int inner = p.inner, is = p.is;
    const int pitch = VEC ? p.pitch : p.segs * 64;
    const int ib0 = ibase_of(n0, inner, is);
    const int lo_raw = ib0 + minoff * inner;
    const int lo = VEC ? lo_raw - ((lo_raw % 4 + 4) % 4) : lo_raw;

    const auto in_rsrc = __builtin_amdgcn_make_buffer_rsrc(const_cast<float*>(p.in), 0, p.in_bytes, 0x00020000);
    const auto w_rsrc = __builtin_amdgcn_make_buffer_rsrc(const_cast<float*>(p.wp), 0, p.w_bytes, 0x00020000);

    int xb[TN];
#pragma unroll
    for (int tn = 0; tn < TN; ++tn) {
        const int col = (wn * TN + tn) * 32 + j;
        const int bl = col >> p.bnl_shift;
        const int nl = col & (p.bnl - 1);
        const int n = min(n0 + nl, p.ncols - 1);
        xb[tn] = (bl * p.ck + kh) * pitch + ibase_of(n, inner, is) - ib0 + (lo_raw - lo);
    }
    const int arow = wm * TM * 32 + j + kh * BM;

    f32x16 acc[TM][TN];
#pragma unroll
    for (int tm = 0; tm < TM; ++tm)
#pragma unroll
        for (int tn = 0; tn < TN; ++tn)
#pragma unroll
            for (int r = 0; r < 16; ++r) acc[tm][tn][r] = 0.f;

    const int wrows = ntaps * p.ck;
    const int w_instrs = (wrows * BM + 255) >> 8;
    const int xrows = p.nb * p.ck;

    constexpr int kNX = 8, kNWS = 10;
    unsigned xo[VEC ? kNX : 1], xc[VEC && CTAIL ? kNX : 1], wo[VEC ? kNWS : 1], wc[VEC && CTAIL ? kNWS : 1];
    unsigned long long vm[TN];
    bool bnd = false;
    int nx = 0, nws = 0, x_floats = 0;
    if constexpr (VEC) {
        const int lpr = pitch >> 2;
        x_floats = xrows * pitch;
        nx = (xrows * lpr + 64 * NW - 1) / (64 * NW);
        nws = (w_instrs + NW - 1) / NW;
        bnd = lo < 0 || lo + 4 * lpr > p.in_valid;
#pragma unroll
        for (int i = 0; i < kNX; ++i) {
            const unsigned g = (unsigned)(wave + NW * i) * 64u + lane;
            const unsigned row = mdiv(g, p.magic_lpr);
            const unsigned v = g - row * lpr;
            const unsigned bl = mdiv(row, p.magic_ck);
            const unsigned c = row - bl * p.ck;
            const bool ok = row < (unsigned)xrows && b0 + bl < (unsigned)p.B;
            xo[i] = ok ? (bl * p.C + c) * (unsigned)p.in_row + 4u * v : kOOB;
            if (CTAIL) xc[i] = c;
        }
#pragma unroll
        for (int i = 0; i < kNWS; ++i) {
            const unsigned f = ((unsigned)(wave + NW * i) * 64u + lane) * 4u;
            const unsigned kr = f / (unsigned)BM;
            const unsigned col = f - kr * BM;
            const unsigned t = mdiv(kr, p.magic_ck);
            const unsigned c = kr - t * p.ck;
            const bool ok = kr < (unsigned)wrows && m0 + col < (unsigned)p.Mp;
            wo[i] = ok ? (t * p.C + c) * p.Mp + m0 + col : kOOB;
            if (CTAIL) wc[i] = c;
        }
#pragma unroll
        for (int tn = 0; tn < TN; ++tn) {
            const int col = (wn * TN + tn) * 32 + j;
            const int nl = col & (p.bnl - 1);
            const int n = min(n0 + nl, p.ncols - 1);
            unsigned long long m = 0;
            for (int t = 0; t < ntaps; ++t) {
                const int f = n * is + p.off[tap0 + t];
                if (f >= 0 && f < p.in_valid) m |= 1ull << t;
            }
            vm[tn] = m;
        }
    }

    auto issue = [&](int c0, float* stage) {
        if constexpr (VEC) {
            const unsigned wbase = wofs + (unsigned)c0 * p.Mp;
#pragma unroll
            for (int i = 0; i < kNWS; ++i) {
                if (i < nws && (wave + NW * i) < w_instrs) {
                    bool dead = wo[i] == kOOB;
                    if (CTAIL) dead = dead || c0 + wc[i] >= (unsigned)p.C;
                    const unsigned off = dead ? kOOB : (wbase + wo[i]) * 4u;
                    __builtin_amdgcn_raw_ptr_buffer_load_lds(w_rsrc, (lds_void*)(stage + (wave + NW * i) * 256), 16, off, 0, 0, 0);
                }
            }
            float* xs = stage + p.wlds_floats;
            const unsigned xbase = ((unsigned)b0 * p.C + (unsigned)c0) * (unsigned)p.in_row + (unsigned)lo;
#pragma unroll
            for (int i = 0; i < kNX; ++i) {
                if (i < nx && (wave + NW * i) * 256 < x_floats) {
                    bool dead = xo[i] == kOOB;
                    if (CTAIL) dead = dead || c0 + xc[i] >= (unsigned)p.C;
                    const unsigned off = dead ? kOOB : (xbase + xo[i]) * 4u;
                    __builtin_amdgcn_raw_ptr_buffer_load_lds(in_rsrc, (lds_void*)(xs + (wave + NW * i) * 256), 16, off, 0, 0, 0);
                }
            }
            return;
        }
        for (int q = wave; q < w_instrs; q += NW) {
            const unsigned f = (unsigned)q * 256u + (unsigned)lane * 4u;
            const unsigned kr = f / (unsigned)BM;
            const unsigned col = f - kr * BM;
            const unsigned t = mdiv(kr, p.magic_ck);
            const unsigned c = kr - t * p.ck;
            const unsigned ch = c0 + c, m = m0 + col;
            unsigned off = kOOB;
            if (kr < (unsigned)wrows && ch < (unsigned)p.C && m < (unsigned)p.Mp)
                off = (wofs + (t * p.C + ch) * p.Mp + m) * 4u;
            __builtin_amdgcn_raw_ptr_buffer_load_lds(w_rsrc, (lds_void*)(stage + q * 256), 16, off, 0, 0, 0);
        }
        float* xs = stage + p.wlds_floats;
        for (int row = wave; row < xrows; row += NW) {
            const unsigned bl = mdiv((unsigned)row, p.magic_ck);
            const unsigned c = row - bl * p.ck;
            const unsigned b = b0 + bl, ch = c0 + c;
            const bool rv = b < (unsigned)p.B && ch < (unsigned)p.C;
            const unsigned rbase = (b * p.C + ch) * (unsigned)p.in_row;
            float* dst = xs + row * pitch;
            for (int seg = 0; seg < p.segs; ++seg) {
                const int fpos = lo + seg * 64 + lane;
                unsigned off = kOOB;
                if (rv && fpos >= 0 && fpos < p.in_valid) off = (rbase + (unsigned)fpos) * 4u;
                __builtin_amdgcn_raw_ptr_buffer_load_lds(in_rsrc, (lds_void*)(dst + seg * 64), 4, off, 0, 0, 0);
            }
        }
    };

    const int total_chunks = (p.C + p.ck - 1) / p.ck;
    const int chunk0 = zsl * p.chunks_per_split;
    const int nchunks = min(p.chunks_per_split, total_chunks - chunk0);
    issue(chunk0 * p.ck, smem);
    for (int i = 0; i < nchunks; ++i) {
        asm volatile("s_waitcnt vmcnt(0)" ::: "memory");
        __syncthreads();
        if (i + 1 < nchunks) issue((chunk0 + i + 1) * p.ck, smem + ((i + 1) & 1) * p.stage_floats);
        const float* w_lds = smem + (i & 1) * p.stage_floats;
        const float* x_lds = w_lds + p.wlds_floats;
        for (int t = 0; t < ntaps; ++t) {
            const int toff = (p.off[tap0 + t] - minoff) * inner;
            const float* wl = w_lds + t * p.ck * BM + arow;
            const float* xl = x_lds + toff;
            bool keep[TN];
#pragma unroll
            for (int tn = 0; tn < TN; ++tn) keep[tn] = !(VEC && bnd) || ((vm[tn] >> t) & 1ull);
            int c = 0;
            for (; c + 8 <= p.ck; c += 8) {
                float a[4][TM], b[4][TN];
#pragma unroll
                for (int u = 0; u < 4; ++u) {
#pragma unroll
                    for (int tm = 0; tm < TM; ++tm) a[u][tm] = wl[(c + 2 * u) * BM + tm * 32];
#pragma unroll
                    for (int tn = 0; tn < TN; ++tn) b[u][tn] = xl[xb[tn] + (c + 2 * u) * pitch];
                }
                if (READS_FIRST) __builtin_amdgcn_sched_barrier(0);
#pragma unroll
                for (int u = 0; u < 4; ++u) {
#pragma unroll
                    for (int tn = 0; tn < TN; ++tn) {
                        float v = b[u][tn];
                        if (VEC) v = keep[tn] ? v : 0.f;
                        if (LEAKY) v = v > 0.f ? v : v * p.in_slope;
                        b[u][tn] = v;
                    }
#pragma unroll
                    for (int tm = 0; tm < TM; ++tm)
#pragma unroll
                        for (int tn = 0; tn < TN; ++tn)
                            acc[tm][tn] = __builtin_amdgcn_mfma_f32_32x32x2f32(a[u][tm], b[u][tn], acc[tm][tn], 0, 0, 0);
                }
                if (READS_FIRST) __builtin_amdgcn_sched_barrier(0);
            }
            for (; c < p.ck; c += 2) {
                float a[TM], b[TN];
#pragma unroll
                for (int tm = 0; tm < TM; ++tm) a[tm] = wl[c * BM + tm * 32];
#pragma unroll
                for (int tn = 0; tn < TN; ++tn) {
                    float v = xl[xb[tn] + c * pitch];
                    if (VEC) v = keep[tn] ? v : 0.f;
                    if (LEAKY) v = v > 0.f ? v : v * p.in_slope;
                    b[tn] = v;
                }
#pragma unroll
                for (int tm = 0; tm < TM; ++tm)
#pragma unroll
                    for (int tn = 0; tn < TN; ++tn)
                        acc[tm][tn] = __builtin_amdgcn_mfma_f32_32x32x2f32(a[tm], b[tn], acc[tm][tn], 0, 0, 0);
            }
        }
    }

    const bool full = m0 + BM <= p.M;
#pragma unroll
    for (int tn = 0; tn < TN; ++tn) {
        const int col = (wn * TN + tn) * 32 + j;
        const int bl = col >> p.bnl_shift;
        const int nl = col & (p.bnl - 1);
        const int n = n0 + nl, b = b0 + bl;
        if (n >= p.ncols || b >= p.B) continue;
        const int oi = oidx_of(n, inner, p.os, oph);
        if (oi >= p.out_valid) continue;
        const long cbase = (long)b * p.M * p.out_row + oi;
        float* __restrict__ outp = (p.ksplit > 1 ? p.part + (long)zsl * p.part_stride : p.out) + cbase;
        const float* __restrict__ mulp = p.mul_src ? p.mul_src + cbase : nullptr;
        const float* __restrict__ addp = p.add ? p.add + cbase : nullptr;
#pragma unroll
        for (int tm = 0; tm < TM; ++tm) {
            const int mb = m0 + (wm * TM + tm) * 32 + 4 * kh;
#pragma unroll
            for (int r = 0; r < 16; ++r) {
                const int m = mb + (r & 3) + 8 * (r >> 2);
                if (full || m < p.M) {
                    const int ro = m * p.out_row;
                    float v = acc[tm][tn][r];
                    if (p.ksplit > 1) {
                        outp[ro] = v;
                        continue;
                    }
                    if (p.bias) v += p.bias[m];
                    if (mulp) {
                        const float al = (p.epi_act == RH_ACT_SNAKE) ? p.mul_alpha[m] : 0.f;
                        v *= rh_act_grad(mulp[ro], p.epi_act, p.epi_slope, al);
                    }
                    if (addp) v += addp[ro];
                    if (p.out_act == RH_ACT_LEAKY) v = v > 0.f ? v : v * p.out_slope;
                    outp[ro] = v;
                }
            }
        }
    }
}

unsigned magic_of(int d) { return (unsigned)(((1u << 20) + d - 1) / d); }

__global__ __launch_bounds__(256) void splitk_finalize_kernel(const ConvP p, long total) {
    float mx = 0.f;
    for (long e = (long)blockIdx.x * 256 + threadIdx.x; e < total; e += (long)gridDim.x * 256) {
        const long row = e / p.out_valid;
        const int oi = (int)(e - row * p.out_valid);
        const int m = (int)(row % p.M);
        const long idx = row * p.out_row + oi;
        float v = 0.f;
        for (int z = 0; z < p.ksplit; ++z) v += p.part[(long)z * p.part_stride + idx];
        if (p.bias) v += p.bias[m];
        if (p.mul_src) {
            const float al = (p.epi_act == RH_ACT_SNAKE) ? p.mul_alpha[m] : 0.f;
            v *= rh_act_grad(p.mul_src[idx], p.epi_act, p.epi_slope, al);
        }
        if (p.add) v += p.add[idx];
        if (p.out_act == RH_ACT_LEAKY) v = v > 0.f ? v : v * p.out_slope;
        p.out[idx] = v;
        mx = rh_absmax(mx, v);
    }
    if (p.out_range) {
        __shared__ float red[4];
        rh_range_publish(p.out_range, mx, blockIdx.x, red);
    }
}

__global__ __launch_bounds__(256) void splitk_finalize4_kernel(const ConvP p, long total4) {
    float mx = 0.f;
    for (long t = (long)blockIdx.x * 256 + threadIdx.x; t < total4; t += (long)gridDim.x * 256) {
        const long e = 4 * t;
        const long row = e / p.out_valid;
        const int oi = (int)(e - row * p.out_valid);
        const int m = (int)(row % p.M);
        const long idx = row * p.out_row + oi;
        f32x4 v = {0.f, 0.f, 0.f, 0.f};
        for (int z = 0; z < p.ksplit; ++z) {
            const f32x4 q = *reinterpret_cast<const f32x4*>(p.part + (long)z * p.part_stride + idx);
#pragma unroll
            for (int i = 0; i < 4; ++i) v[i] += q[i];
        }
        if (p.bias) {
            const float b = p.bias[m];
#pragma unroll
            for (int i = 0; i < 4; ++i) v[i] += b;
        }
        if (p.mul_src) {
            const float al = (p.epi_act == RH_ACT_SNAKE) ? p.mul_alpha[m] : 0.f;
            const f32x4 q = *reinterpret_cast<const f32x4*>(p.mul_src + idx);
#pragma unroll
            for (int i = 0; i < 4; ++i) v[i] *= rh_act_grad(q[i], p.epi_act, p.epi_slope, al);
        }
        if (p.add) {
            const f32x4 q = *reinterpret_cast<const f32x4*>(p.add + idx);
#pragma unroll
            for (int i = 0; i < 4; ++i) v[i] += q[i];
        }
        if (p.out_act == RH_ACT_LEAKY) {
#pragma unroll
            for (int i = 0; i < 4; ++i) v[i] = v[i] > 0.f ? v[i] : v[i] * p.out_slope;
        }
        *reinterpret_cast<f32x4*>(p.out + idx) = v;
        mx = rh_absmax(rh_absmax(mx, v[0]), v[1]); mx = rh_absmax(rh_absmax(mx, v[2]), v[3]);
    }
    if (p.out_range) {
        __shared__ float red[4];
        rh_range_publish(p.out_range, mx, blockIdx.x, red);
    }
}

int finalize_launch(const ConvP& p, hipStream_t stream) {
    const long total = (long)p.B * p.M * p.out_valid;
    const bool vec = (p.out_valid & 3) == 0 && (p.out_row & 3) == 0 && (p.part_stride & 3) == 0 &&
                     (((uintptr_t)p.part | (uintptr_t)p.out | (uintptr_t)p.mul_src | (uintptr_t)p.add) & 15) == 0;
    const long items = vec ? total / 4 : total;
    long blocks = rh_cdiv64(items, 256);
    if (p.out_range && blocks > 4096) blocks = 4096;
    if (vec) hipLaunchKernelGGL(splitk_finalize4_kernel, dim3((unsigned)blocks), dim3(256), 0, stream, p, items);
    else hipLaunchKernelGGL(splitk_finalize_kernel, dim3((unsigned)blocks), dim3(256), 0, stream, p, items);
    return rh_check_launch("conv_splitk_finalize");
}

struct Plan { int blocks, total_chunks, ksplit, chunks_per_split; };

Plan plan_split(const ConvP& p, int BM, int col_tiles) {
    Plan pl{};
    pl.blocks = col_tiles * rh_cdiv(p.M, BM) * p.nphase;
    pl.total_chunks = rh_cdiv(p.C, p.ck);
    static const int split_below = [] { const char* e = getenv("RH_CONV_SPLIT_BELOW"); return e ? atoi(e) : 512; }();
    static const int split_target = [] { const char* e = getenv("RH_CONV_SPLIT_TARGET"); return e ? atoi(e) : 768; }();
    int z = 1;
    if (pl.blocks < split_below) {
        z = rh_cdiv(split_target, pl.blocks);
        const int zmax = pl.total_chunks / 2;
        if (z > zmax) z = zmax;
        if (z > 16) z = 16;
        if (z < 1) z = 1;
    }
    pl.chunks_per_split = rh_cdiv(pl.total_chunks, z);
    pl.ksplit = rh_cdiv(pl.total_chunks, pl.chunks_per_split);
    return pl;
}

template <int TM, int TN, int WM, int WN>
int launch_dma(ConvP& p, hipStream_t stream, const char* what, void* ws, int64_t ws_bytes, bool plan_only = false,
               int64_t* want = nullptr) {
    constexpr int BM = TM * WM * 32, BN = TN * WN * 32;
    int bnl = BN;
    if (p.ncols < BN) {
        bnl = 32;
        while (bnl < p.ncols) bnl <<= 1;
    }
    p.bnl = bnl;
    p.bnl_shift = __builtin_ctz(bnl);
    p.nb = BN / bnl;
    p.tiles_per_b = rh_cdiv(p.ncols, bnl);
    int span = 0, maxtaps = 1;
    for (int i = 0; i < p.nphase; ++i) {
        span = span > p.ph_maxoff[i] - p.ph_minoff[i] ? span : p.ph_maxoff[i] - p.ph_minoff[i];
        maxtaps = maxtaps > p.ph_ntaps[i] ? maxtaps : p.ph_ntaps[i];
    }
    int width;
    if (p.inner == 1)
        width = (bnl - 1) * p.is + span + 1;
    else
        width = ((bnl - 1) / p.inner + 1) * p.is * p.inner + p.inner + span * p.inner + 1;
    static const int novec = [] { const char* e = getenv("RH_CONV_NOVEC"); return e ? atoi(e) : 0; }();
    bool vec = !novec && p.inner == 1 && maxtaps <= 64 && (p.in_row % 4) == 0 && ((uintptr_t)p.in % 16) == 0 &&
               ((uintptr_t)p.wp % 16) == 0;
    static const int budget_env = [] { const char* e = getenv("RH_CONV_STAGE_FLOATS"); return e ? atoi(e) : 0; }();
    int ck = 2;
    for (int attempt = 0; attempt < 2; ++attempt) {
        p.segs = rh_cdiv(width, 64);
        p.pitch = vec ? ((width + 3 + 3) & ~3) : p.segs * 64;
        const int per_ch = maxtaps * BM + p.nb * p.pitch;
        int budget = budget_env > 0 ? budget_env : (p.C >= 192 ? 6 * 1024 : 5 * 1024);
        ck = ((budget - 512) / per_ch) & ~1;
        if (budget_env <= 0 && ck < (p.C >= 192 ? 4 : 8)) {
            budget = 10 * 1024;
            ck = ((budget - 512) / per_ch) & ~1;
        }
        if (ck > 32) ck = 32;
        if (ck < 2) ck = 2;
        const int cmax = (p.C + 1) & ~1;
        if (ck > cmax) ck = cmax;
        if (!vec) break;
        const int nx = rh_cdiv(p.nb * ck * (p.pitch >> 2), 64 * WM * WN);
        const int nws = rh_cdiv(rh_cdiv(maxtaps * ck * BM, 256), WM * WN);
        if (nx <= 8 && nws <= 10) break;
        vec = false;
    }
    p.ck = ck;
    p.wlds_floats = (maxtaps * ck * BM + 255) & ~255;
    p.stage_floats = p.wlds_floats + ((p.nb * ck * p.pitch + 255) & ~255);
    p.magic_segs = magic_of(p.segs);
    p.magic_ck = magic_of(ck);
    p.magic_lpr = magic_of(p.pitch >> 2);
    const size_t lds = sizeof(float) * 2 * (size_t)p.stage_floats;
    const int col_tiles = rh_cdiv(p.B, p.nb) * p.tiles_per_b;
    Plan pl = plan_split(p, BM, col_tiles);
    p.part_stride = (long)p.B * p.M * p.out_row;
    const int64_t need = pl.ksplit > 1 ? (int64_t)pl.ksplit * p.part_stride * (int64_t)sizeof(float) : 0;
    if (plan_only) {
        *want = lds > 160 * 1024 ? 0 : need;
        return RH_OK;
    }
    if (lds > 160 * 1024) return rh_conv_launch_sync(p, stream, what);
    if (need > 0 && (!ws || ws_bytes < need)) {
        pl.ksplit = 1;
        pl.chunks_per_split = pl.total_chunks;
    }
    p.ksplit = pl.ksplit;
    p.chunks_per_split = pl.chunks_per_split;
    p.part = (float*)ws;
    auto launch = [&](auto kern) {
        dim3 grid(col_tiles, rh_cdiv(p.M, BM), p.nphase * p.ksplit);
        rh_launch_main(kern, grid, dim3(WM * WN * 64), lds, stream, p);
    };
    auto go = [&](auto kern) {
        static std::once_flag once;
        std::call_once(once, [&] { (void)hipFuncSetAttribute(reinterpret_cast<const void*>(kern), hipFuncAttributeMaxDynamicSharedMemorySize, 160 * 1024); });
        launch(kern);
    };
    const bool leaky = p.in_act == RH_ACT_LEAKY;
    const bool ctail = (p.C % p.ck) != 0;
    if (vec && !ctail) {
        if (leaky) go(conv_igemm_dma_kernel<TM, TN, WM, WN, true, true, false>);
        else go(conv_igemm_dma_kernel<TM, TN, WM, WN, false, true, false>);
    } else if (vec) {
        if (leaky) go(conv_igemm_dma_kernel<TM, TN, WM, WN, true, true, true>);
        else go(conv_igemm_dma_kernel<TM, TN, WM, WN, false, true, true>);
    } else {
        if (leaky) go(conv_igemm_dma_kernel<TM, TN, WM, WN, true, false, true>);
        else go(conv_igemm_dma_kernel<TM, TN, WM, WN, false, false, true>);
    }
    if (int e = rh_check_launch(what)) return e;
    if (p.ksplit > 1) return finalize_launch(p, stream);
    return RH_OK;
}

void fill_sizes(ConvP& p) {
    unsigned long long wtaps = 0;
    for (int i = 0; i < p.nphase; ++i) wtaps += p.ph_ntaps[i];
    p.in_bytes = (unsigned)(4ull * p.B * p.C * (unsigned long long)p.in_row);
    p.w_bytes = (unsigned)(4ull * wtaps * p.C * p.Mp);
}

}

bool rh_conv_dma_eligible(const ConvP& p) {
    if (p.in_act == RH_ACT_SNAKE) return false;
    const unsigned long long in_b = 4ull * p.B * p.C * (unsigned long long)p.in_row;
    unsigned long long wtaps = 0;
    for (int i = 0; i < p.nphase; ++i) wtaps += p.ph_ntaps[i];
    const unsigned long long w_b = 4ull * wtaps * p.C * p.Mp;
    const unsigned long long row_span = (unsigned long long)p.M * (unsigned long long)p.out_row;
    return in_b < 0x7fffffffull && w_b < 0x7fffffffull && row_span < 0x7fffffffull;
}

int rh_splitk_finalize_launch(ConvP& p, hipStream_t stream) { return finalize_launch(p, stream); }

int rh_conv_launch_dma(ConvP& p, hipStream_t stream, const char* what, void* ws, int64_t ws_bytes) {
    fill_sizes(p);
    {
        bool used = false;
        if (int e = rh_conv_launch_x6(p, stream, what, ws, ws_bytes, &used)) return e;
        if (used) return RH_OK;
        if (int e = rh_conv_launch_c2x(p, stream, what, &used)) return e;
        if (used) return rh_range_after(p, stream);
    }
    unsigned* const orange = p.out_range;
    p.out_range = nullptr;
    int rc;
    if (p.M <= 32) rc = launch_dma<1, 2, 1, 4>(p, stream, what, ws, ws_bytes);
    else if (p.M <= 64) rc = launch_dma<2, 1, 1, 4>(p, stream, what, ws, ws_bytes);
    else if (p.M % 96 == 0 || p.M < 96) rc = launch_dma<3, 1, 1, 4>(p, stream, what, ws, ws_bytes);
    else rc = launch_dma<2, 2, 2, 2>(p, stream, what, ws, ws_bytes);
    p.out_range = orange;
    return rc ? rc : rh_range_after(p, stream);
}

int64_t rh_conv_splitk_workspace(ConvP p) {
    if (p.B <= 0 || p.ncols <= 0 || p.M <= 0 || !rh_conv_dma_eligible(p)) return 0;
    fill_sizes(p);
    int64_t want = 0;
    const int64_t x6 = rh_conv_x6_workspace(p);
    if (p.M <= 32) launch_dma<1, 2, 1, 4>(p, nullptr, "", nullptr, 0, true, &want);
    else if (p.M <= 64) launch_dma<2, 1, 1, 4>(p, nullptr, "", nullptr, 0, true, &want);
    else if (p.M % 96 == 0 || p.M < 96) launch_dma<3, 1, 1, 4>(p, nullptr, "", nullptr, 0, true, &want);
    else launch_dma<2, 2, 2, 2>(p, nullptr, "", nullptr, 0, true, &want);
    return want > x6 ? want : x6;
}
```

### rave_amd/csrc/conv_params.hpp

```cpp
#pragma once
#include "common.hpp"

constexpr int kMaxPhases = 8;
constexpr int kMaxTaps = 64;

struct ConvP {
    const float* in;
    const float* wp;
    float* out;
    const float* bias;
    const float* mul_src;
    const float* add;
    const float* in_alpha;
    const float* mul_alpha;
    int B, C, M, Mp;
    int in_row, in_valid, out_row, out_valid;
    int ncols, inner, is, os;
    int bnl, bnl_shift, nb, tiles_per_b;
    int pitch;
    int ck;
    int wlds_floats;
    int in_act, epi_act, out_act;
    float in_slope, epi_slope, out_slope;
    int segs;
    unsigned magic_segs, magic_ck, magic_lpr;
    int stage_floats;
    int ksplit;
    int chunks_per_split;
    float* part;
    unsigned* tickets;
    long part_stride;
    unsigned in_bytes, w_bytes;
    const unsigned* wq;
    unsigned wq_bytes;
    const unsigned* in_range;
    unsigned* out_range;
    const unsigned* w_range;
    int x6_mode;
    int x6_P;
    int x6_a_units, x6_b_units;
    int x6_nu;
    int v_s;
    long v_q2ofs;
    int vs;
    int Mr;
    int v_o0;
    int v_U, v_b0;
    long ph_q2ofs[kMaxPhases];
    long x6_wofs;
    int nphase;
    int ph_oph[kMaxPhases], ph_ntaps[kMaxPhases], ph_tap0[kMaxPhases], ph_minoff[kMaxPhases],
        ph_maxoff[kMaxPhases];
    long ph_wofs[kMaxPhases];
    int off[kMaxTaps];
};

struct WgradP {
    const float* R;
    const float* S;
    float* out;
    const float* r_alpha;
    const float* s_alpha;
    int B, M, C, T;
    int r_row;
    int s_row, s_valid;
    int inner, is;
    int r_act, s_act;
    float r_slope, s_slope;
    int rk;
    int chunks_per_b;
    int total_chunks;
    int chunks_per_z;
    int pr;
    int ps;
    int nc_max;
    int minoff, maxoff;
    unsigned magic_ps, magic_cpb, magic_pr, magic_lpr_r, magic_lpr_s;
    int vec;
    int r_floats, s_floats;
    int stage_floats;
    unsigned r_bytes, s_bytes;
    int off[kMaxTaps];
};

struct PackP {
    const float* w;
    const float* scale;
    float* wp;
    unsigned* wq;
    unsigned* range;
    long total;
    int C, M, Mp, k;
    int nslots;
    int m_major;
    int x6_mode;
    int x6_nu;
    int bf16x3;
    int x6_vs, x6_U, x6_Mvp, vz_n;
    long x6_vofs;
    int q2j[kMaxTaps], vq2a[kMaxTaps];
    int vz_j[2 * kMaxPhases], vz_u[2 * kMaxPhases];
    int kk[kMaxTaps];
    int q2a[kMaxTaps];
    int q2n[kMaxTaps];
};
int rh_pack_launch(const PackP& a, const PackP& b, hipStream_t stream, const char* what, const float* w = nullptr, long rows = 0,
                   long cols = 0);
int64_t rh_bias_grad_workspace(int M);
int rh_bias_grad_launch(const float* dy, const float* y, float* part, float* db, int B, int M, long plane, int act,
                        float slope, hipStream_t stream, float* g_out = nullptr, unsigned* g_range = nullptr);
int rh_reduce_partials_launch(const float* part, float* out, long n, int Z, hipStream_t stream, const char* what);
struct RhWnTail {
    const float* v;
    const float* g;
    const float* norms;
    float* dv;
    float* dg;
};
struct RhWgradArmed {
    rh_reduce_item* defer;
    const unsigned* dy_range;
    const unsigned* x_range;
};
RhWgradArmed rh_wgrad_take_armed(bool may_defer);
int rh_wgrad_run(const rh_conv1d_desc* d, const float* dy, const float* x, const float* alpha, float* dw, float* dbias, void* ws,
                 int64_t ws_bytes, hipStream_t stream, const RhWgradArmed& armed, const RhWnTail* tail = nullptr);

int rh_conv_fill_fwd(const rh_conv1d_desc* d, ConvP* p);
int rh_conv_fill_dgrad(const rh_conv1d_desc* d, ConvP* p);
int rh_conv_launch(ConvP& p, hipStream_t stream, const char* what, void* ws = nullptr, int64_t ws_bytes = 0);
int rh_conv_launch_sync(ConvP& p, hipStream_t stream, const char* what);
int rh_range_after(const ConvP& p, hipStream_t stream);
int rh_conv_launch_dma(ConvP& p, hipStream_t stream, const char* what, void* ws, int64_t ws_bytes);
bool rh_conv_dma_eligible(const ConvP& p);
int64_t rh_conv_splitk_workspace(ConvP p);
int64_t rh_conv_x6_workspace(ConvP p);
inline int rh_x6_mode(int C, int nphase, int is, int inner, int ntaps0, const int* off, const int* kk) {
    if (is == 1) return (C & 15) == 0 ? 1 : 0;
    if (is == 3) return (nphase == 1 && inner == 1 && (C & 15) == 0) ? 1 : 0;
    if (nphase != 1 || inner != 1 || (is != 2 && is != 4) || (C * is) % 16 != 0) return 0;
    for (int t = 0; t < ntaps0; ++t)
        if (off[t] != off[0] + t || kk[t] != t) return 0;
    return is;
}
inline bool rh_x6_epi_instantiated(int is, int tm, bool leaky, int epi) {
    const int m = epi & 15, v = epi >> 4;
    if (v) {
        if (is != 1 || tm < 2 || v > 2) return false;
        return leaky ? (m == 0 || m == 1 || m == 5) : (m == 0 || m == 1 || m == 2 || m == 4 || m == 5 || m == 6);
    }
    return leaky ? (m == 0 || m == 1 || m == 4 || m == 5) : (m == 0 || m == 1 || m == 2 || m == 4 || m == 5 || m == 6 || m == 9 || m == 13);
}
int rh_conv_launch_x6(ConvP& p, hipStream_t stream, const char* what, void* ws, int64_t ws_bytes, bool* used);
int rh_conv_launch_c2x(ConvP& p, hipStream_t stream, const char* what, bool* used);
bool rh_conv_c2x_query(ConvP p);
bool rh_conv_x6_plan_query(ConvP p, int* out7);

bool rh_smallc_fwd_eligible(const rh_conv1d_desc* d, bool has_residual);
int rh_smallc_fwd(const rh_conv1d_desc* d, const float* x, const float* wp_fwd, const float* bias, float* y, hipStream_t stream,
                  unsigned* out_range = nullptr);
bool rh_smallc_dgrad_eligible(const rh_conv1d_desc* d, bool has_add);
int rh_smallc_dgrad(const rh_conv1d_desc* d, const float* dy, const float* wp_bwd, const int* slot_of_tap, float* dx,
                    hipStream_t stream);
bool rh_smallc_wgrad_eligible(const rh_conv1d_desc* d);
int64_t rh_smallc_wgrad_workspace(const rh_conv1d_desc* d);
int rh_smallc_wgrad(const rh_conv1d_desc* d, const float* dy, const float* x, float* dw, float* dbias, void* ws,
                    hipStream_t stream);
```

### rave_amd/csrc/conv_x6.hip

```cpp
#include <atomic>
#include <cstdlib>
#include <mutex>
#include "conv_params.hpp"
#include "conv2d_x6.hpp"

int rh_splitk_finalize_launch(ConvP& p, hipStream_t stream);
bool rh_x6_launch_i1_121(const ConvP& q, int epi, dim3 grid, size_t lds, hipStream_t stream);
bool rh_x6_launch_i1_221(const ConvP& q, int epi, dim3 grid, size_t lds, hipStream_t stream);
bool rh_x6_launch_i1_321(const ConvP& q, int epi, dim3 grid, size_t lds, hipStream_t stream);
bool rh_x6_launch_i1_122(const ConvP& q, int epi, dim3 grid, size_t lds, hipStream_t stream);
bool rh_x6_launch_i1_222(const ConvP& q, int epi, dim3 grid, size_t lds, hipStream_t stream);
bool rh_x6_launch_i1_322(const ConvP& q, int epi, dim3 grid, size_t lds, hipStream_t stream);
bool rh_x6_launch_i1_211(const ConvP& q, int epi, dim3 grid, size_t lds, hipStream_t stream);
bool rh_x6_launch_i1_311(const ConvP& q, int epi, dim3 grid, size_t lds, hipStream_t stream);
bool rh_x6_launch_i1_212(const ConvP& q, int epi, dim3 grid, size_t lds, hipStream_t stream);
bool rh_x6_launch_i1_312(const ConvP& q, int epi, dim3 grid, size_t lds, hipStream_t stream);
bool rh_x6_launch_i2_121(const ConvP& q, int epi, dim3 grid, size_t lds, hipStream_t stream);
bool rh_x6_launch_i2_221(const ConvP& q, int epi, dim3 grid, size_t lds, hipStream_t stream);
bool rh_x6_launch_i2_321(const ConvP& q, int epi, dim3 grid, size_t lds, hipStream_t stream);
bool rh_x6_launch_i2_122(const ConvP& q, int epi, dim3 grid, size_t lds, hipStream_t stream);
bool rh_x6_launch_i2_222(const ConvP& q, int epi, dim3 grid, size_t lds, hipStream_t stream);
bool rh_x6_launch_i2_322(const ConvP& q, int epi, dim3 grid, size_t lds, hipStream_t stream);
bool rh_x6_launch_i2_211(const ConvP& q, int epi, dim3 grid, size_t lds, hipStream_t stream);
bool rh_x6_launch_i2_311(const ConvP& q, int epi, dim3 grid, size_t lds, hipStream_t stream);
bool rh_x6_launch_i2_212(const ConvP& q, int epi, dim3 grid, size_t lds, hipStream_t stream);
bool rh_x6_launch_i2_312(const ConvP& q, int epi, dim3 grid, size_t lds, hipStream_t stream);
bool rh_x6_launch_i4_121(const ConvP& q, int epi, dim3 grid, size_t lds, hipStream_t stream);
bool rh_x6_launch_i4_221(const ConvP& q, int epi, dim3 grid, size_t lds, hipStream_t stream);
bool rh_x6_launch_i4_321(const ConvP& q, int epi, dim3 grid, size_t lds, hipStream_t stream);
bool rh_x6_launch_i4_122(const ConvP& q, int epi, dim3 grid, size_t lds, hipStream_t stream);
bool rh_x6_launch_i4_222(const ConvP& q, int epi, dim3 grid, size_t lds, hipStream_t stream);
bool rh_x6_launch_i4_322(const ConvP& q, int epi, dim3 grid, size_t lds, hipStream_t stream);
bool rh_x6_launch_i4_211(const ConvP& q, int epi, dim3 grid, size_t lds, hipStream_t stream);
bool rh_x6_launch_i4_311(const ConvP& q, int epi, dim3 grid, size_t lds, hipStream_t stream);
bool rh_x6_launch_i4_212(const ConvP& q, int epi, dim3 grid, size_t lds, hipStream_t stream);
bool rh_x6_launch_i4_312(const ConvP& q, int epi, dim3 grid, size_t lds, hipStream_t stream);

namespace {

struct X6Plan {
    size_t lds;
    int64_t part_bytes;
    int tm, tn, wm, wn, ksplit, chunks_per_split, col_tiles, row_tiles;
};

typedef bool (*X6Launch)(const ConvP&, int, dim3, size_t, hipStream_t);
X6Launch x6_launcher(int is, int tm, int tn, int wm) {
#define RH_X6_S(IS_, TM_, TN_, WM_) if (is == IS_ && tm == TM_ && tn == TN_ && wm == WM_) return rh_x6_launch_i##IS_##_##TM_##TN_##WM_;
#define RH_X6_SHAPES(IS_) \
    RH_X6_S(IS_, 1, 2, 1) RH_X6_S(IS_, 2, 2, 1) RH_X6_S(IS_, 3, 2, 1) RH_X6_S(IS_, 1, 2, 2) RH_X6_S(IS_, 2, 2, 2) RH_X6_S(IS_, 3, 2, 2) \
    RH_X6_S(IS_, 2, 1, 1) RH_X6_S(IS_, 3, 1, 1) RH_X6_S(IS_, 2, 1, 2) RH_X6_S(IS_, 3, 1, 2)
    RH_X6_SHAPES(1) RH_X6_SHAPES(2) RH_X6_SHAPES(4)
#undef RH_X6_SHAPES
#undef RH_X6_S
    return nullptr;
}
constexpr unsigned kTicketPool = 1u << 20;
constexpr int kTicketDevices = 64;
struct TicketPool { unsigned* words = nullptr; std::atomic<unsigned> next{0}; std::once_flag once; };
TicketPool* ticket_pool() {
    static TicketPool pools[kTicketDevices];
    int dev = 0;
    if (hipGetDevice(&dev) != hipSuccess || dev < 0 || dev >= kTicketDevices) return nullptr;
    TicketPool* tp = &pools[dev];
    std::call_once(tp->once, [tp] {
        unsigned* q = nullptr;
        if (hipMalloc(&q, kTicketPool * sizeof(unsigned)) == hipSuccess && hipMemset(q, 0, kTicketPool * sizeof(unsigned)) == hipSuccess)
            tp->words = q;
    });
    return tp->words ? tp : nullptr;
}
unsigned* ticket_segment(unsigned n) {
    TicketPool* tp = ticket_pool();
    if (!tp || n > kTicketPool) return nullptr;
    for (;;) {
        unsigned at = tp->next.load(std::memory_order_relaxed);
        const unsigned start = at + n > kTicketPool ? 0u : at;
        if (tp->next.compare_exchange_weak(at, start + n, std::memory_order_relaxed)) return tp->words + start;
    }
}

int combine_max() {
    const char* e = getenv("RH_X6_COMBINE");
    return e ? atoi(e) : 8;
}

int epi_mode(const ConvP& p) { return (p.bias ? 1 : 0) | (p.mul_src ? 2 : 0) | (p.add ? 4 : 0) | (p.out_act == RH_ACT_LEAKY ? 8 : 0); }

bool x6_enabled() {
    const char* e = getenv("RH_CONV_X6");
    return !(e && atoi(e) == 0);
}

bool plan_x6(ConvP& p, X6Plan* pl) {
    if (!x6_enabled() || p.x6_mode == 0) return false;
    if (RH_X6_F16 && !p.in_range) return false;
    p.vs = 0;
    p.Mr = p.M;
    if (p.v_s > 1 && p.x6_mode == 1 && p.nphase == p.v_s && p.is == 1 && p.inner == 1) {
        const int s = p.v_s;
        const int extra = p.v_o0 ? 1 : 0;
        auto tiles = [](int n) {
            if (n >= 128) return (double)rh_cdiv(n, 128);
            int w = 32;
            while (w < n) w <<= 1;
            return w / 128.0;
        };
        const int mvp = (p.Mr * s + 31) & ~31;
        const int tmv = mvp % 96 == 0 ? 3 : (mvp % 64 == 0 ? 2 : 1);
        const bool epi_ok = rh_x6_epi_instantiated(1, tmv, p.in_act == RH_ACT_LEAKY, epi_mode(p) | (s == 2 ? 16 : 32));
        if (epi_ok && tiles(p.ncols + extra) <= 1.07 * tiles(p.ncols)) {
            p.vs = s;
            p.M = p.Mr * s;
            p.Mp = (p.M + 31) & ~31;
            p.ncols += extra;
            p.nphase = 1;
            p.ph_ntaps[0] = p.v_U; p.ph_tap0[0] = 0; p.ph_oph[0] = 0; p.ph_q2ofs[0] = p.v_q2ofs;
            p.ph_maxoff[0] = p.v_b0; p.ph_minoff[0] = p.v_b0 - p.v_U + 1;
            for (int u = 0; u < p.v_U; ++u) p.off[u] = p.v_b0 - u;
        }
    }
    if (p.x6_mode != p.is) return false;
    if (p.in_act == RH_ACT_SNAKE || p.epi_act == RH_ACT_SNAKE) return false;
    if (p.in_act == RH_ACT_LEAKY && !(p.in_slope >= 0.f && p.in_slope <= 1.f)) return false;
    if (!rh_x6_epi_instantiated(p.is, 3, p.in_act == RH_ACT_LEAKY, epi_mode(p))) return false;
    if (p.is != 1 && (p.inner != 1 || p.nphase != 1)) return false;
    if (((uintptr_t)p.wq & 15) || ((uintptr_t)p.in & 3)) return false;
    const int is = p.is;
    pl->tm = p.Mp % 96 == 0 ? 3 : (p.Mp % 64 == 0 ? 2 : 1);
    int span = 0;
    if (is == 1) {
        for (int i = 0; i < p.nphase; ++i) span = span > p.ph_maxoff[i] - p.ph_minoff[i] ? span : p.ph_maxoff[i] - p.ph_minoff[i];
        span *= p.inner;
    } else {
        span = p.x6_nu - 1;
    }
    auto shape = [&](int tn, int wm) -> int {
        pl->tn = tn; pl->wm = wm; pl->wn = 4 / wm;
        const int BM = 32 * pl->tm * wm, BN = 32 * tn * pl->wn;
        int bnl = BN;
        if (p.ncols < BN) {
            bnl = 32;
            while (bnl < p.ncols) bnl <<= 1;
        }
        p.bnl = bnl;
        p.bnl_shift = __builtin_ctz(bnl);
        p.nb = BN / bnl;
        p.tiles_per_b = rh_cdiv(p.ncols, bnl);
        p.pitch = bnl + span;
        p.x6_P = p.nb * p.pitch;
        const int nq = pl->wn * tn == 8 ? 3 : 2;
        if (2 * p.x6_P > 256 * nq) return 0;
        p.x6_a_units = 2 * kX6P * BM;
        p.x6_b_units = 2 * kX6P * p.x6_P;
        pl->lds = (size_t)(2 * p.x6_a_units + 2 * p.x6_b_units) * 16;
        if (pl->lds > 160 * 1024) return 0;
        pl->col_tiles = rh_cdiv(p.B, p.nb) * p.tiles_per_b;
        pl->row_tiles = rh_cdiv(p.Mp, BM);
        return pl->col_tiles * pl->row_tiles * p.nphase;
    };
    const int wm0 = p.Mp >= 64 * pl->tm ? 2 : 1;
    static const int tn_env = [] { const char* e = getenv("RH_X6_TN"); return e ? atoi(e) : 0; }();
    int blocks = shape(2, wm0);
    const int total_steps = ((p.C * is) >> 4) * (is == 1 ? p.ph_ntaps[0] : p.x6_nu);
    if (pl->tm >= 2 && (tn_env == 1 || (tn_env == 0 && ((blocks < 384 && total_steps <= 64) || blocks <= 64)))) {
        const int b1 = shape(1, wm0);
        if (b1 == 0) blocks = shape(2, wm0);
        else blocks = b1;
    }
    if (blocks == 0) return false;
    const int total_chunks = (p.C * is) >> 4;
    static const int split_env = [] { const char* e = getenv("RH_X6_SPLIT_BELOW"); return e ? atoi(e) : 0; }();
    static const int split_target = [] { const char* e = getenv("RH_X6_SPLIT_TARGET"); return e ? atoi(e) : 512; }();
    const int split_below = split_env > 0 ? split_env : 200;
    int z = 1;
    if (blocks < split_below) {
        z = rh_cdiv(split_target, blocks);
        if (z > total_chunks / 2) z = total_chunks / 2;
        if (z > 16) z = 16;
        if (z < 1) z = 1;
    }
    pl->chunks_per_split = rh_cdiv(total_chunks, z);
    pl->ksplit = rh_cdiv(total_chunks, pl->chunks_per_split);
    p.part_stride = (long)p.B * p.Mr * p.out_row;
    pl->part_bytes = 0;
    if (pl->ksplit > 1) {
        const int64_t tiled = (int64_t)pl->ksplit * blocks * (32 * pl->tm * pl->wm) * (32 * pl->tn * pl->wn) * (int64_t)sizeof(float);
        const int64_t flat = (int64_t)pl->ksplit * p.part_stride * (int64_t)sizeof(float);
        pl->part_bytes = tiled > flat ? tiled : flat;
    }
    const unsigned long long in_b = 4ull * p.B * p.C * (unsigned long long)p.in_row;
    const unsigned long long row_span = (unsigned long long)p.Mr * (unsigned long long)p.out_row;
    const unsigned long long out_b = 4ull * (unsigned long long)p.part_stride;
    return in_b < 0x7fffffffull && (unsigned long long)p.wq_bytes < 0x7fffffffull && row_span < 0x7fffffffull && out_b < 0x7fffffffull;
}

}

bool rh_conv_x6_plan_fixed(ConvP& p, int tm, int tn, int wm, size_t* lds, dim3* grid) {
    if (!x6_enabled() || p.x6_mode != 1 || p.is != 1 || p.inner != 1 || p.nphase != 1) return false;
    if (((uintptr_t)p.in & 3)) return false;
    if (RH_X6_F16 && !p.in_range) return false;
    p.vs = 0;
    p.Mr = p.M;
    const int wn = 4 / wm;
    const int BM = 32 * tm * wm, BN = 32 * tn * wn;
    if (BM != p.Mp) return false;
    int bnl = BN;
    if (p.ncols < BN) {
        bnl = 32;
        while (bnl < p.ncols) bnl <<= 1;
    }
    p.bnl = bnl;
    p.bnl_shift = __builtin_ctz(bnl);
    p.nb = BN / bnl;
    p.tiles_per_b = rh_cdiv(p.ncols, bnl);
    const int span = (p.ph_maxoff[0] - p.ph_minoff[0]) * p.inner;
    p.pitch = bnl + span;
    p.x6_P = p.nb * p.pitch;
    const int nq = wn * tn == 8 ? 3 : 2;
    if (2 * p.x6_P > 256 * nq) return false;
    p.x6_a_units = 2 * kX6P * BM;
    p.x6_b_units = 2 * kX6P * p.x6_P;
    *lds = (size_t)(2 * p.x6_a_units + 2 * p.x6_b_units) * 16;
    if (*lds > 160 * 1024) return false;
    p.ksplit = 1;
    p.chunks_per_split = p.C >> 4;
    p.part_stride = (long)p.B * p.Mr * p.out_row;
    const unsigned long long in_b = 4ull * p.B * p.C * (unsigned long long)p.in_row;
    const unsigned long long out_b = 4ull * (unsigned long long)p.part_stride;
    if (!(in_b < 0x7fffffffull && (unsigned long long)p.wq_bytes < 0x7fffffffull && out_b < 0x7fffffffull)) return false;
    *grid = dim3(rh_cdiv(p.B, p.nb) * p.tiles_per_b, 1, 1);
    return true;
}

int64_t rh_conv_x6_workspace(ConvP p) {
    X6Plan pl{};
    static const unsigned any_range[kRangeSlotWords] = {};
    if (!p.in_range) p.in_range = any_range;
    if (!plan_x6(p, &pl)) return -1;
    if (pl.part_bytes > 0) (void)ticket_pool();
    return pl.part_bytes;
}

bool rh_conv_x6_plan_query(ConvP p, int* out) {
    X6Plan pl{};
    static const unsigned any_range[kRangeSlotWords] = {};
    if (!p.in_range) p.in_range = any_range;
    if (!plan_x6(p, &pl)) return false;
    out[0] = pl.tm; out[1] = pl.tn; out[2] = pl.wm; out[3] = pl.ksplit;
    out[4] = p.is;
    out[5] = p.vs;
    out[6] = pl.col_tiles * pl.row_tiles * p.nphase * pl.ksplit;
    return true;
}

int rh_conv_launch_x6(ConvP& p, hipStream_t stream, const char* what, void* ws, int64_t ws_bytes, bool* used) {
    *used = false;
    ConvP q = p;
    X6Plan pl{};
    if (!plan_x6(q, &pl)) return RH_OK;
    if (pl.part_bytes > 0 && (!ws || ws_bytes < pl.part_bytes || ((uintptr_t)ws & 15) || pl.part_bytes >= 0x7fffffffll)) {
        pl.ksplit = 1;
        pl.chunks_per_split = (q.C * q.is) >> 4;
    }
    q.in_bytes = (unsigned)(4ull * q.B * q.C * (unsigned long long)q.in_row);
    q.w_range = q.wq + q.wq_bytes / 4;
    q.tickets = nullptr;
    if (pl.ksplit > 1 && pl.ksplit <= combine_max()) {
        q.tickets = ticket_segment((unsigned)(pl.col_tiles * pl.row_tiles * q.nphase));
        RH_REQUIRE(q.tickets, RH_ERR_INVALID, "%s: no arrival counters for a K-split launch (hipMalloc failed, or first use under stream capture)", what);
    }
    q.part = (float*)ws;
    q.ksplit = pl.ksplit;
    q.chunks_per_split = pl.chunks_per_split;
    dim3 grid(pl.col_tiles, pl.row_tiles, q.nphase * q.ksplit);
    const int epi = (q.ksplit > 1 && !q.tickets ? 0 : epi_mode(q)) | (q.vs == 2 ? 16 : (q.vs == 4 ? 32 : 0));
    const X6Launch go = x6_launcher(q.is, pl.tm, pl.tn, pl.wm);
    RH_REQUIRE(go && go(q, epi, grid, pl.lds, stream), RH_ERR_UNSUPPORTED, "%s: no conv_x6_kernel instance for stride %d tile %d%d%d epilogue %d",
               what, q.is, pl.tm, pl.tn, pl.wm, epi);
    if (int e = rh_check_launch(what)) return e;
    *used = true;
    if (q.ksplit > 1 && !q.tickets) {
        ConvP f = p;
        f.part = q.part; f.ksplit = q.ksplit; f.part_stride = q.part_stride;
        f.out_range = q.out_range;
        return rh_splitk_finalize_launch(f, stream);
    }
    return RH_OK;
}

namespace {
bool fill_c2x_from_1d(const ConvP& p, C2X* q) {
    if (p.x6_mode != 1 || p.is == 1 || p.is == 2 || p.is == 4 || p.inner != 1 || p.nphase != 1 || p.os != 1) return false;
    if (p.in_act != RH_ACT_NONE || p.epi_act != RH_ACT_NONE || p.mul_src || p.add || p.in_alpha || p.mul_alpha) return false;
    if (p.in_row != p.in_valid || p.out_row != p.out_valid || p.ph_ntaps[0] < 1 || p.ph_ntaps[0] > kMaxTaps) return false;
    *q = C2X{};
    q->in = p.in; q->wq = p.wq; q->out = p.out; q->bias = p.bias;
    q->B = p.B; q->C = p.C; q->M = p.M; q->Mp = p.Mp;
    q->in_h = p.in_row; q->in_w = 1; q->out_h = p.out_row; q->out_w = 1;
    q->rows = p.ncols; q->qcols = 1;
    q->is_h = p.is; q->is_w = 1; q->os_h = 1; q->os_w = 1;
    q->out_act = p.out_act; q->out_slope = p.out_slope;
    q->nphase = 1;
    q->ph_oph_h[0] = p.ph_oph[0]; q->ph_oph_w[0] = 0;
    q->ph_ntaps[0] = p.ph_ntaps[0]; q->ph_tap0[0] = 0;
    q->ph_minh[0] = p.ph_minoff[0]; q->ph_maxh[0] = p.ph_maxoff[0]; q->ph_minw[0] = q->ph_maxw[0] = 0;
    q->ph_q2ofs[0] = p.ph_q2ofs[0];
    for (int t = 0; t < p.ph_ntaps[0]; ++t) { q->offh[t] = p.off[p.ph_tap0[0] + t]; q->offw[t] = 0; }
    q->wq_bytes = p.wq_bytes;
    q->in_range = p.in_range; q->out_range = p.out_range;
    return true;
}
}

bool rh_conv_c2x_query(ConvP p) {
    C2X q;
    long v[8];
    return x6_enabled() && fill_c2x_from_1d(p, &q) && rh_conv2d_x6_plan_query(q, v);
}

int rh_conv_launch_c2x(ConvP& p, hipStream_t stream, const char* what, bool* used) {
    *used = false;
    C2X q;
    if (!x6_enabled() || !fill_c2x_from_1d(p, &q)) return RH_OK;
    return rh_conv2d_x6_launch(q, stream, what, used);
}
```

### rave_amd/csrc/unit_x6.hip

```cpp
#include <cstdlib>
#include <mutex>
#include <type_traits>
#include "conv_params.hpp"
#include "conv_x6_kernel.inc"

bool rh_conv_x6_plan_fixed(ConvP& p, int tm, int tn, int wm, size_t* lds, dim3* grid);

namespace {

struct UnitP {
    ConvP c;
    const unsigned* wq1;
    unsigned wq1_bytes;
    float slope2;
    float* h_out;
    const unsigned* w1_range;
    unsigned* h_range;
};

template <int TM, int TN>
__global__ __launch_bounds__(256, 2) void unit_x6_kernel(const UnitP u) {
    const ConvP& p = u.c;
    constexpr int WN = 4;
    constexpr int BM = 32 * TM;
    constexpr int A_UNITS = 2 * kX6P * BM;
    constexpr int NAL = (A_UNITS + 255) / 256;
    constexpr int NQ = WN * TN == 8 ? 3 : 2;
    extern __shared__ __attribute__((aligned(16))) unsigned char smem_raw[];
    u32x4* const a_st = reinterpret_cast<u32x4*>(smem_raw);
    u32x4* const b_st = a_st + 2 * A_UNITS;

    const int tid = threadIdx.x, lane = tid & 63;
    const int wn = __builtin_amdgcn_readfirstlane(tid >> 6);
    const int j = lane & 31, g = lane >> 5;

    const int tap0 = p.ph_tap0[0];
    const int minoff = p.ph_minoff[0];
    const int nu = p.ph_ntaps[0];
    const int bt = blockIdx.x / p.tiles_per_b;
    const int nt = blockIdx.x - bt * p.tiles_per_b;
    const int b0 = bt * p.nb;
    const int n0 = nt * p.bnl;
    const int pitch = p.pitch, P = p.x6_P;
    const float slope1 = p.in_act == RH_ACT_LEAKY ? p.in_slope : 1.f;

    const auto in_rsrc = __builtin_amdgcn_make_buffer_rsrc(const_cast<float*>(p.in), 0, p.in_bytes, 0x00020000);
    const auto w_rsrc = __builtin_amdgcn_make_buffer_rsrc(const_cast<unsigned*>(p.wq), 0, p.wq_bytes, 0x00020000);
#if RH_X6_F16
    int inv_x, inv_w3, inv_h, inv_w1;
    const unsigned xmax = rh_range_max(p.in_range);
    const float xsc = __uint_as_float(rh_x6_scale_bits(xmax, &inv_x));
    (void)rh_x6_scale_bits(p.w_range[0], &inv_w3);
    const float osc1 = __uint_as_float(rh_x6_unscale_bits(inv_w3, inv_x));
    const float hbound = __uint_as_float(xmax) * __uint_as_float(p.w_range[1]);
    const unsigned hsc_bits = rh_x6_scale_bits(__float_as_uint(hbound), &inv_h);
    (void)rh_x6_scale_bits(u.w1_range[0], &inv_w1);
    const float osc2 = __uint_as_float(rh_x6_unscale_bits(inv_w1, inv_h));
    const float h2sc = __uint_as_float(rh_x6_unscale_bits(inv_w3 + (int)(hsc_bits >> 23) - 127, inv_x));
#else
    const float xsc = 1.f, osc1 = 1.f, osc2 = 1.f, h2sc = 1.f;
#endif

    int bpos[TN];
#pragma unroll
    for (int tn = 0; tn < TN; ++tn) {
        const int col = (wn * TN + tn) * 32 + j;
        const int bl = col >> p.bnl_shift;
        const int nl = col & (p.bnl - 1);
        const int n = min(n0 + nl, p.ncols - 1);
        bpos[tn] = g * kX6P * P + bl * pitch + (n - n0);
    }
    const int arow = g * kX6P * BM + j;

    f32x16 acc[TM][TN];
#pragma unroll
    for (int tm = 0; tm < TM; ++tm)
#pragma unroll
        for (int tn = 0; tn < TN; ++tn)
#pragma unroll
            for (int r = 0; r < 16; ++r) acc[tm][tn][r] = 0.f;

    unsigned aoff[NAL];
#pragma unroll
    for (int r = 0; r < NAL; ++r) {
        const int uu = tid + 256 * r;
        const int gs = uu / BM, mrow = uu - gs * BM;
        aoff[r] = (uu < A_UNITS && mrow < p.Mp) ? (unsigned)((gs * p.Mp + mrow) * 16) : kOOB;
    }
    const unsigned step_bytes = (unsigned)(2 * kX6P * p.Mp * 16);
    unsigned xoff[NQ];
    int xdst[NQ];
#pragma unroll
    for (int q = 0; q < NQ; ++q) {
        const int e = tid + 256 * q;
        const int o = e >= P ? 1 : 0;
        const int pp = e - o * P;
        const int bl = pp / pitch, qq = pp - bl * pitch;
        const bool task = e < 2 * P;
        const bool bok = task && b0 + bl < p.B;
        xdst[q] = task ? o * kX6P * P + pp : -1;
        const int f = n0 + minoff + qq;
        const bool ok = bok && f >= 0 && f < p.in_valid;
        xoff[q] = ok ? (unsigned)((((b0 + bl) * p.C + 8 * o) * p.in_row + f) * 4) : kOOB;
    }
    const unsigned chunk_bytes = (unsigned)(16 * p.in_row * 4);
    unsigned rowc[8];
#pragma unroll
    for (int i = 0; i < 8; ++i) rowc[i] = (unsigned)(i * p.in_row * 4);

    float xr[NQ][8];
    u32x4 ar[NAL];
    auto load_x = [&](int chunk) {
        const unsigned cbv = (unsigned)chunk * chunk_bytes;
#pragma unroll
        for (int q = 0; q < NQ; ++q)
#pragma unroll
            for (int i = 0; i < 8; ++i)
                xr[q][i] = __builtin_bit_cast(float, __builtin_amdgcn_raw_buffer_load_b32(in_rsrc, xoff[q], cbv + rowc[i], 0));
    };
    auto split8 = [&](const float (&v)[8], float slope, float sc, u32x4 (&pk)[kX6P]) {
#if RH_X6_F16
#pragma unroll
        for (int k = 0; k < 4; ++k) {
            float a = v[2 * k] * sc, b = v[2 * k + 1] * sc;
            a = rh_max1(a, a * slope);
            b = rh_max1(b, b * slope);
            const rh_h2 h = rh_h2_split(a, b);
            pk[0][k] = h.hi; pk[1][k] = h.lo;
        }
#else
        unsigned h[3][8];
#pragma unroll
        for (int i = 0; i < 8; ++i) {
            const float a = rh_max1(v[i], v[i] * slope);
            rh_bf3_split(a, h[0][i], h[1][i], h[2][i]);
        }
#pragma unroll
        for (int s3 = 0; s3 < 3; ++s3)
#pragma unroll
            for (int k = 0; k < 4; ++k) pk[s3][k] = __builtin_amdgcn_perm(h[s3][2 * k + 1], h[s3][2 * k], 0x07060302u);
#endif
    };
    auto convert_x = [&](int stage) {
        u32x4* dst0 = b_st + stage * 2 * kX6P * P;
#pragma unroll
        for (int q = 0; q < NQ; ++q) {
            if (xdst[q] < 0) continue;
            u32x4 pk[kX6P];
            split8(xr[q], slope1, xsc, pk);
#pragma unroll
            for (int s3 = 0; s3 < kX6P; ++s3) dst0[xdst[q] + s3 * P] = pk[s3];
        }
    };
    const int nchunks = p.C >> 4;
    const int S = nchunks * nu;
    const unsigned sbytes0 = (unsigned)(p.ph_q2ofs[0] * 16);
    auto load_a = [&](int step) {
        const unsigned sb = sbytes0 + (unsigned)step * step_bytes;
#pragma unroll
        for (int r = 0; r < NAL; ++r) {
            if (r * 256 >= A_UNITS) continue;
            ar[r] = __builtin_bit_cast(u32x4, __builtin_amdgcn_raw_buffer_load_b128(w_rsrc, aoff[r], sb, 0));
        }
    };
    auto store_a = [&](int stage) {
#pragma unroll
        for (int r = 0; r < NAL; ++r) {
            const int uu = tid + 256 * r;
            if (uu < A_UNITS) a_st[stage * A_UNITS + uu] = ar[r];
        }
    };
    load_a(0);
    load_x(0);
    store_a(0);
    if (S > 1) load_a(1);
    convert_x(0);
    if (nchunks > 1) load_x(1);
    __syncthreads();
    constexpr int SA[RH_X6_NPROD] = RH_X6_SA, SB[RH_X6_NPROD] = RH_X6_SB;
    int st = 0;
    int toff_next = p.off[tap0] - minoff;
    for (int ci = 0; ci < nchunks; ++ci) {
        const u32x4* bl_ = b_st + (ci & 1) * 2 * kX6P * P;
        for (int t = 0; t < nu; ++t, ++st) {
            const int toff = toff_next;
            {
                const int t1 = t + 1 < nu ? t + 1 : 0;
                toff_next = p.off[tap0 + t1] - minoff;
            }
            const u32x4* al = a_st + (st & 1) * A_UNITS + arow;
            rh_x6_frag bfr[TN][kX6P], afr[TM][kX6P];
#pragma unroll
            for (int tn = 0; tn < TN; ++tn)
#pragma unroll
                for (int s3 = 0; s3 < kX6P; ++s3) bfr[tn][s3] = __builtin_bit_cast(rh_x6_frag, bl_[bpos[tn] + s3 * P + toff]);
#pragma unroll
            for (int tm = 0; tm < TM; ++tm)
#pragma unroll
                for (int s3 = 0; s3 < kX6P; ++s3) afr[tm][s3] = __builtin_bit_cast(rh_x6_frag, al[s3 * BM + tm * 32]);
            if (st + 1 < S) {
                store_a((st + 1) & 1);
                if (st + 2 < S) load_a(st + 2);
            }
            if (t == nu - 1 && ci + 1 < nchunks) {
                convert_x((ci + 1) & 1);
                if (ci + 2 < nchunks) load_x(ci + 2);
            }
#pragma unroll
            for (int q = 0; q < RH_X6_NPROD; ++q)
#pragma unroll
                for (int tm = 0; tm < TM; ++tm)
#pragma unroll
                    for (int tn = 0; tn < TN; ++tn)
                        acc[tm][tn] = RH_X6_MFMA(afr[tm][SA[q]], bfr[tn][SB[q]], acc[tm][tn]);
            __syncthreads();
        }
    }

    unsigned cb[TN];
#pragma unroll
    for (int tn = 0; tn < TN; ++tn) {
        const int col = (wn * TN + tn) * 32 + j;
        const int bl = col >> p.bnl_shift;
        const int nl = col & (p.bnl - 1);
        const int n = n0 + nl, b = b0 + bl;
        const bool ok = n < p.ncols && b < p.B && n < p.out_valid;
        cb[tn] = ok ? (unsigned)(((long)b * p.M * p.out_row + n) * 4) : kOOB;
    }
    const unsigned obytes = (unsigned)(p.part_stride * 4);
    const auto y_r = __builtin_amdgcn_make_buffer_rsrc(p.out, 0, obytes, 0x00020000);
    const auto x_r = __builtin_amdgcn_make_buffer_rsrc(const_cast<float*>(p.add), 0, obytes, 0x00020000);
    const auto none_r = __builtin_amdgcn_make_buffer_rsrc(static_cast<float*>(nullptr), 0, 0, 0x00020000);
    const bool full = BM <= p.M;
    float hmax_all = 0.f;
    if (u.h_out) {
        const auto h_r = __builtin_amdgcn_make_buffer_rsrc(u.h_out, 0, obytes, 0x00020000);
        x6_store_tile<0, TM, TN>(acc, cb, 0, g, p.M, full, p.out_row, h_r, none_r, none_r, none_r, 1.f, 0.f, osc1, hmax_all);
    }

    constexpr int W1_UNITS = (BM / 16) * 2 * kX6P * BM;
    u32x4* const w1s = reinterpret_cast<u32x4*>(smem_raw);
    {
        const auto w1_r = __builtin_amdgcn_make_buffer_rsrc(const_cast<unsigned*>(u.wq1), 0, u.wq1_bytes, 0x00020000);
        constexpr int NW = (W1_UNITS + 255) / 256;
        u32x4 wv[NW];
#pragma unroll
        for (int r = 0; r < NW; ++r) {
            const int uu = tid + 256 * r;
            wv[r] = __builtin_bit_cast(u32x4, __builtin_amdgcn_raw_buffer_load_b128(w1_r, uu < W1_UNITS ? (unsigned)(uu * 16) : kOOB, 0, 0));
        }
#pragma unroll
        for (int r = 0; r < NW; ++r) {
            const int uu = tid + 256 * r;
            if (uu < W1_UNITS) w1s[uu] = wv[r];
        }
    }
    __syncthreads();

    float ymax = 0.f;
#pragma unroll
    for (int tn = 0; tn < TN; ++tn) {
        f32x16 acc2[TM][1];
#pragma unroll
        for (int tm = 0; tm < TM; ++tm)
#pragma unroll
            for (int r = 0; r < 16; ++r) acc2[tm][0][r] = 0.f;
#pragma unroll
        for (int b = 0; b < 2 * TM; ++b) {
            const int tmh = b >> 1, hf = b & 1;
            float v[8];
#pragma unroll
            for (int i = 0; i < 8; ++i) v[i] = acc[tmh][tn][8 * hf + i];
            u32x4 pk[kX6P];
            split8(v, u.slope2, h2sc, pk);
            rh_x6_frag bfr2[kX6P], afr2[TM][kX6P];
#pragma unroll
            for (int s3 = 0; s3 < kX6P; ++s3) {
                auto r0 = __builtin_amdgcn_permlane32_swap(pk[s3][0], pk[s3][2], false, false);
                auto r1 = __builtin_amdgcn_permlane32_swap(pk[s3][1], pk[s3][3], false, false);
                u32x4 f;
                f[0] = r0[0]; f[2] = r0[1]; f[1] = r1[0]; f[3] = r1[1];
                bfr2[s3] = __builtin_bit_cast(rh_x6_frag, f);
            }
            const u32x4* al = w1s + (b * 2 * kX6P + g * kX6P) * BM + j;
#pragma unroll
            for (int tm = 0; tm < TM; ++tm)
#pragma unroll
                for (int s3 = 0; s3 < kX6P; ++s3) afr2[tm][s3] = __builtin_bit_cast(rh_x6_frag, al[s3 * BM + tm * 32]);
#pragma unroll
            for (int q = 0; q < RH_X6_NPROD; ++q)
#pragma unroll
                for (int tm = 0; tm < TM; ++tm)
                    acc2[tm][0] = RH_X6_MFMA(afr2[tm][SA[q]], bfr2[SB[q]], acc2[tm][0]);
        }
        const unsigned cb1[1] = {cb[tn]};
        x6_store_tile<4, TM, 1>(acc2, cb1, 0, g, p.M, full, p.out_row, y_r, none_r, x_r, none_r, 1.f, 0.f, osc2, ymax);
    }
    if (RH_X6_F16 && (p.out_range || u.h_range)) {
        __syncthreads();
        float* red = reinterpret_cast<float*>(smem_raw);
        if (p.out_range) rh_range_publish(p.out_range, ymax, blockIdx.x, red);
        if (u.h_range) rh_range_publish(u.h_range, hmax_all, blockIdx.x + 5u, red + 4);
    }
}

bool unit_enabled() {
    const char* e = getenv("RH_UNIT_FUSED");
    if (e && atoi(e) == 0) return false;
    const char* x6 = getenv("RH_CONV_X6");
    return !(x6 && atoi(x6) == 0);
}

bool unit_shape_ok(const rh_conv1d_desc* d3, const rh_conv1d_desc* d1) {
    if (!d3 || !d1) return false;
    const int C = d3->c_in;
    auto act_ok = [](const rh_conv1d_desc* d) {
        return d->act == RH_ACT_NONE || (d->act == RH_ACT_LEAKY && d->act_slope >= 0.f && d->act_slope <= 1.f);
    };
    return (C == 32 || C == 64 || C == 96) && d3->c_out == C && d1->c_in == C && d1->c_out == C && !d3->transposed &&
           !d1->transposed && d3->stride == 1 && d1->stride == 1 && d3->inner == 1 && d1->inner == 1 && d3->groups == 1 &&
           d1->groups == 1 && d1->kernel == 1 && d1->dilation == 1 && d1->pad_left == 0 && d3->in_valid == 0 &&
           d1->in_valid == 0 && d3->out_act == RH_ACT_NONE && d1->out_act == RH_ACT_NONE && act_ok(d3) && act_ok(d1) &&
           d3->batch > 0 && d3->batch == d1->batch && d3->l_in > 0 && d3->l_out == d3->l_in && d1->l_in == d3->l_in &&
           d1->l_out == d3->l_in;
}

int fill_unit(const rh_conv1d_desc* d3, const rh_conv1d_desc* d1, UnitP* u, size_t* lds, dim3* grid) {
    ConvP& p = u->c;
    if (int e = rh_conv_fill_fwd(d3, &p)) return e;
    ConvP p1{};
    if (int e = rh_conv_fill_fwd(d1, &p1)) return e;
    if (p.x6_mode != 1 || p1.x6_mode != 1 || p.nphase != 1) return RH_ERR_UNSUPPORTED;
    const int tm = p.M / 32;
    if (!rh_conv_x6_plan_fixed(p, tm, 2, 1, lds, grid)) return RH_ERR_UNSUPPORTED;
    const size_t w1_bytes = (size_t)(p.M / 16) * 2 * kX6P * p.M * 16;
    if (w1_bytes > *lds) *lds = w1_bytes;
    if (*lds > 160 * 1024 || (unsigned long long)p1.wq_bytes < w1_bytes) return RH_ERR_UNSUPPORTED;
    u->wq1_bytes = p1.wq_bytes;
    u->slope2 = d1->act == RH_ACT_LEAKY ? d1->act_slope : 1.f;
    u->h_out = nullptr;
    u->wq1 = reinterpret_cast<const unsigned*>((uintptr_t)p1.x6_wofs);
    return RH_OK;
}

}

extern "C" int rh_residual_unit_fused(const rh_conv1d_desc* d3, const rh_conv1d_desc* d1) {
    if (!unit_enabled() || !unit_shape_ok(d3, d1)) return 0;
    UnitP u{};
    size_t lds = 0;
    dim3 grid;
    static const unsigned any_range[kRangeSlotWords] = {};
    u.c.in_range = any_range;
    return fill_unit(d3, d1, &u, &lds, &grid) == RH_OK ? 1 : 0;
}

extern "C" int rh_residual_unit_fwd_f32(const rh_conv1d_desc* d3, const rh_conv1d_desc* d1, const float* x, const float* wp3_fwd,
                                        const float* wp1_fwd, float* h, float* y, rh_stream_t stream) {
    const RhKernelEventsScope events;
    const unsigned* x_range = nullptr;
    unsigned *y_range = nullptr, *h_range = nullptr;
    rh_take_ranges(nullptr, &x_range, &y_range, &h_range);
    RH_REQUIRE(unit_enabled() && unit_shape_ok(d3, d1), RH_ERR_UNSUPPORTED, "residual_unit_fwd: geometry not fusable");
    RH_REQUIRE(x && wp3_fwd && wp1_fwd && y, RH_ERR_INVALID, "residual_unit_fwd: null pointer");
    UnitP u{};
    size_t lds = 0;
    dim3 grid;
    RH_REQUIRE(!RH_X6_F16 || x_range, RH_ERR_INVALID, "residual_unit_fwd: the f16 kernels need the input's range slot (rh_x6_set_ranges)");
    u.c.in_range = x_range;
    if (int e = fill_unit(d3, d1, &u, &lds, &grid)) {
        rh_set_error("residual_unit_fwd: geometry not fusable");
        return e;
    }
    ConvP& p = u.c;
    p.in_range = x_range; p.out_range = y_range; u.h_range = h ? h_range : nullptr;
    RH_REQUIRE((((uintptr_t)wp3_fwd | (uintptr_t)wp1_fwd) & 15) == 0 && ((uintptr_t)x & 3) == 0, RH_ERR_INVALID,
               "residual_unit_fwd: misaligned operand");
    p.in = x; p.wp = wp3_fwd; p.out = y; p.bias = nullptr; p.add = x; p.mul_src = nullptr;
    p.wq = reinterpret_cast<const unsigned*>(wp3_fwd + p.x6_wofs);
    p.in_alpha = nullptr; p.mul_alpha = nullptr;
    p.in_bytes = (unsigned)(4ull * p.B * p.C * (unsigned long long)p.in_row);
    u.wq1 = reinterpret_cast<const unsigned*>(wp1_fwd + (long)(uintptr_t)u.wq1);
    p.w_range = p.wq + p.wq_bytes / 4;
    u.w1_range = u.wq1 + u.wq1_bytes / 4;
    u.h_out = h;
    auto go = [&](auto kern) {
        static std::once_flag once;
        std::call_once(once, [&] {
            (void)hipFuncSetAttribute(reinterpret_cast<const void*>(kern), hipFuncAttributeMaxDynamicSharedMemorySize, 160 * 1024);
        });
        rh_launch_main(kern, grid, dim3(256), lds, (hipStream_t)stream, u);
    };
    const int tm = p.M / 32;
    if (tm == 1) go(unit_x6_kernel<1, 2>);
    else if (tm == 2) go(unit_x6_kernel<2, 2>);
    else go(unit_x6_kernel<3, 2>);
    return rh_check_launch("residual_unit_fwd");
}
```

### rave_amd/prep.py

```python
from __future__ import annotations

import ctypes as C
from typing import List

import torch
import torch.nn as nn

from . import _lib as L
from . import cc
from .ops import ConvGeom, _desc


def _geom_of(m: nn.Module) -> ConvGeom:
    if isinstance(m, (cc.Conv1d, cc.ConvTranspose1d)):
        return m.geom()
    if isinstance(m, cc.PlainConv1d):
        return ConvGeom(stride=m.stride[0], dilation=m.dilation[0], pad_left=m.padding[0], pad_right=m.padding[0])
    if isinstance(m, cc.Conv2dK1):
        return ConvGeom(stride=m.stride[0], pad_left=m.padding[0], pad_right=m.padding[0])
    raise TypeError(type(m))


class WeightPrep:
    def __init__(self, model: nn.Module):
        self.mods: List[nn.Module] = [m for m in model.modules()
                                      if isinstance(m, (cc.Conv1d, cc.ConvTranspose1d, cc.PlainConv1d, cc.Conv2dK1))
                                      and getattr(m, "weight_g", None) is not None and m.groups == 1
                                      and m.weight_v.is_cuda]
        self.n = len(self.mods)
        self.bufs = []
        if self.n == 0:
            return
        isz = L.lib.rh_prep_item_bytes()
        host = (C.c_uint8 * L.lib.rh_prep_array_bytes(self.n))()
        dev = self.mods[0].weight_v.device
        for i, m in enumerate(self.mods):
            v, g = m.weight_v, m.weight_g
            k = v.shape[2]
            transposed = isinstance(m, cc.ConvTranspose1d)
            c_in, c_out = (v.shape[0], v.shape[1]) if transposed else (v.shape[1], v.shape[0])
            d = _desc(_geom_of(m), 1, c_in, c_out, 1, 1, k)
            dref = C.byref(d)
            rows = v.shape[0]
            ns = torch.empty(4, rows, device=dev, dtype=torch.float32)
            wp_f = torch.empty(L.lib.rh_conv1d_packed_floats(dref, 0), device=dev, dtype=torch.float32)
            wp_b = torch.empty(L.lib.rh_conv1d_packed_floats(dref, 1), device=dev, dtype=torch.float32)
            item = C.cast(C.byref(host, i * isz), C.c_void_p)
            L.check(L.lib.rh_prep_fill_item(dref, L.ptr(v), L.ptr(g), L.ptr(ns[0]), L.ptr(ns[1]), L.ptr(wp_f),
                                            L.ptr(wp_b), item), "prep_fill_item")
            self.bufs.append((wp_f, wp_b, ns[0], ns, v.data_ptr(), g.data_ptr()))
        tr, tb = C.c_int64(0), C.c_int64(0)
        L.check(L.lib.rh_prep_link(C.cast(host, C.c_void_p), self.n, C.byref(tr), C.byref(tb)), "prep_link")
        self.total_rows, self.total_blocks = tr.value, tb.value
        self.items = torch.frombuffer(bytearray(host), dtype=torch.uint8).to(dev)

    def _versions(self):
        return tuple((m.weight_v._version, m.weight_g._version) for m in self.mods)

    def invalidate(self) -> None:
        self._packed_versions = None

    def run(self, reuse: bool = False) -> None:
        if self.n == 0:
            return
        for m, b in zip(self.mods, self.bufs):
            if m.weight_v.data_ptr() != b[4] or m.weight_g.data_ptr() != b[5]:
                raise RuntimeError("rave_amd.WeightPrep: a parameter was re-allocated; rebuild the WeightPrep")
        capturing = torch.cuda.is_current_stream_capturing()
        ver = self._versions()
        if not reuse or capturing or ver != getattr(self, "_packed_versions", None):
            L.check(L.lib.rh_prep_run_f32(self.items.data_ptr(), self.n, self.total_rows, self.total_blocks, L.stream()),
                    "prep_run")
            self._packed_versions = None if capturing else ver
        for m, b in zip(self.mods, self.bufs):
            m._prepacked = (b[0], b[1], b[2])

    def release(self) -> None:
        for m in self.mods:
            m._prepacked = None
```

Baseline: 245.6 million samples/s.

## Pack only needed weight sections and share fwd/bwd pack tiles per layer

Weight prep now plans which packed sections (f32 and/or x6) each conv actually uses, and skips packing sections it does not need. Those are packed lazily through an on-demand ensure hook in the x6 launch paths. Forward and backward packs of the same layer can share one tile pass that writes both layouts from one LDS tile. A separate no-backward table is kept for no-grad runs. The aim is to cut the per-step weight-prep kernel work, at the cost of host-side bookkeeping, a mutex lookup per launch, and extra complexity around graph capture. For v2 models with Snake, all sections are still packed, so only the shared-tile path changes.

Result: no change. 247.6 million samples/s (median of 6 runs) (+0.8%).

```diff
diff --git a/include/rave_hip.h b/include/rave_hip.h
--- a/include/rave_hip.h
+++ b/include/rave_hip.h
@@ -86,6 +86,13 @@
                       float* wp_fwd, float* wp_bwd, void* item_host);
 int rh_prep_link(void* items_host, int32_t n, int64_t* total_rows, int64_t* total_blocks);
 int rh_prep_run_f32(const void* items_dev, int32_t n, int64_t total_rows, int64_t total_blocks, rh_stream_t stream);
+#define RH_PACK_F32 1
+#define RH_PACK_X6 2
+int rh_prep_set_sections(void* item_host, int32_t which, int32_t sections);
+int32_t rh_prep_item_sections(const void* item_host, int32_t which);
+int rh_prep_bind(const void* items_host, int32_t n, const void* items_dev);
+int rh_prep_unbind(const void* items_dev);
+int64_t rh_prep_on_demand_packs(void);
 
 
 int rh_conv1d_fwd_f32(const rh_conv1d_desc* d, const float* x, const float* wp_fwd,
diff --git a/rave_amd/_lib.py b/rave_amd/_lib.py
--- a/rave_amd/_lib.py
+++ b/rave_amd/_lib.py
@@ -82,6 +82,11 @@
         "rh_prep_fill_item": ([D, P, P, P, P, P, P, P], C.c_int),
         "rh_prep_link": ([P, I32, C.POINTER(I64), C.POINTER(I64)], C.c_int),
         "rh_prep_run_f32": ([P, I32, I64, I64, P], C.c_int),
+        "rh_prep_set_sections": ([P, I32, I32], C.c_int),
+        "rh_prep_item_sections": ([P, I32], I32),
+        "rh_prep_bind": ([P, I32, P], C.c_int),
+        "rh_prep_unbind": ([P], C.c_int),
+        "rh_prep_on_demand_packs": ([], I64),
         "rh_conv1d_fwd_f32": ([D, P, P, P, P, P, P, P, I64, P], C.c_int),
         "rh_conv1d_bwd_data_f32": ([D, P, P, P, P, P, P, P, I64, P], C.c_int),
         "rh_conv1d_kernel_family": ([D, C.c_int, C.c_int, C.c_int], C.c_int),
diff --git a/rave_amd/csrc/conv_host.hip b/rave_amd/csrc/conv_host.hip
--- a/rave_amd/csrc/conv_host.hip
+++ b/rave_amd/csrc/conv_host.hip
@@ -1,4 +1,11 @@
 #include "conv_params.hpp"
+
+#include <atomic>
+#include <mutex>
+#include <type_traits>
+#include <unordered_map>
+#include <utility>
+#include <vector>
 
 int64_t rh_wgrad_workspace(const rh_conv1d_desc* d);
 
@@ -204,7 +211,8 @@
 constexpr int kPackSlots = 4;
 
 __host__ __device__ __forceinline__ long pack_tiles(const PackP& q) {
-    return q.total ? (long)(q.Mp / 32) * ((q.C + 31) / 32) : 0;
+    if (!q.total || (q.skip & kPackF32 && (q.skip & kPackX6 || !q.wq))) return 0;
+    return (long)(q.Mp / 32) * ((q.C + 31) / 32);
 }
 
 __device__ __forceinline__ void emit_fragment_bf3(const float (&v)[8], unsigned* dst, long piece_stride_u32) {
@@ -251,20 +259,25 @@
 #endif
 }
 
-__device__ __forceinline__ void pack_tile(const PackP& q, long tile, float* lds , int sg = 0, int sn = 1) {
+__device__ __forceinline__ float piece_scale(const PackP& q) {
+#if RH_X6_F16
+    if (q.wq && !q.bf16x3) {
+        int inv;
+        return __uint_as_float(rh_x6_scale_bits(q.range[0], &inv));
+    }
+#endif
+    return 1.f;
+}
+
+__device__ __forceinline__ void pack_tile(const PackP& q, long tile, float* lds , int sg = 0, int sn = 1,
+                                          const PackP* f = nullptr, const int* fslot = nullptr) {
     const int ct = (q.C + 31) / 32;
     const int c0 = (int)(tile % ct) * 32;
     const int m0 = (int)(tile / ct) * 32;
     const int tid = threadIdx.x;
-    float fsc = 1.f;
-#if RH_X6_F16
-    if (q.wq && !q.bf16x3) {
-        int inv;
-        fsc = __uint_as_float(rh_x6_scale_bits(q.range[0], &inv));
-    }
-#endif
     for (int s0 = sg * kPackSlots; s0 < q.nslots; s0 += sn * kPackSlots) {
         const int ns = min(kPackSlots, q.nslots - s0);
+        const bool first = s0 == 0;
         constexpr int U = 8;
         int kks[kPackSlots];
 #pragma unroll
@@ -298,75 +311,95 @@
                 if (dst[u] >= 0) lds[dst[u]] = v[u] * sc[u];
         }
         __syncthreads();
-        for (int e = tid; e < ns * 1024; e += 256) {
-            const int ml = e & 31, cl = (e >> 5) & 31, sl = e >> 10;
-            const int c = c0 + cl;
-            if (c < q.C) q.wp[((long)(s0 + sl) * q.C + c) * q.Mp + m0 + ml] = lds[(sl * 32 + cl) * 33 + ml];
-        }
-        if (q.wq && q.x6_mode == 1) {
-            for (int e = tid; e < ns * 128; e += 256) {
-                const int ml = e & 31, oct = (e >> 5) & 3, sl = e >> 7;
-                const int cb = c0 + oct * 8;
-                if (cb >= q.C) continue;
-                float v[8];
-#pragma unroll
-                for (int i = 0; i < 8; ++i) v[i] = lds[(sl * 32 + oct * 8 + i) * 33 + ml];
-                const int slot = s0 + sl;
-                if (q.bf16x3) {
-                    const long unit3 = (long)q.q2a[slot] + (long)(cb >> 4) * q.q2n[slot] + (long)(((cb >> 3) & 1) * 3) * q.Mp + m0 + ml;
-                    emit_fragment_bf3(v, q.wq + unit3 * 4, (long)q.Mp * 4);
-                    continue;
-                }
-                const long unit = (long)q.q2a[slot] + (long)(cb >> 4) * q.q2n[slot] + (long)(((cb >> 3) & 1) * kX6P) * q.Mp + m0 + ml;
-                emit_fragment(v, q.wq + unit * 4, (long)q.Mp * 4, fsc);
-            }
-        }
-        if (q.wq && q.x6_vs > 1) {
-            const int vs = q.x6_vs;
-            for (int e = tid; e < ns * 128; e += 256) {
-                const int ml = e & 31, oct = (e >> 5) & 3, sl = e >> 7;
-                const int cb = c0 + oct * 8;
-                const int r = (m0 + ml) * vs + q.q2j[s0 + sl];
-                if (cb >= q.C || r >= q.x6_Mvp) continue;
-                float v[8];
-#pragma unroll
-                for (int i = 0; i < 8; ++i) v[i] = lds[(sl * 32 + oct * 8 + i) * 33 + ml];
-                const int slot = s0 + sl;
-                const long unit = q.x6_vofs + q.vq2a[slot] + (long)(cb >> 4) * q.x6_U * 2 * kX6P * q.x6_Mvp + (long)(((cb >> 3) & 1) * kX6P) * q.x6_Mvp + r;
-                emit_fragment(v, q.wq + unit * 4, (long)q.x6_Mvp * 4, fsc);
-            }
-            if (s0 == 0) {
-                const float zero[8] = {0.f, 0.f, 0.f, 0.f, 0.f, 0.f, 0.f, 0.f};
-                for (int e = tid; e < q.vz_n * 128; e += 256) {
-                    const int ml = e & 31, oct = (e >> 5) & 3, zi = e >> 7;
-                    const int cb = c0 + oct * 8;
-                    const int r = (m0 + ml) * vs + q.vz_j[zi];
-                    if (cb >= q.C || r >= q.x6_Mvp) continue;
-                    const long unit = q.x6_vofs + (long)q.vz_u[zi] * 2 * kX6P * q.x6_Mvp + (long)(cb >> 4) * q.x6_U * 2 * kX6P * q.x6_Mvp +
-                                      (long)(((cb >> 3) & 1) * kX6P) * q.x6_Mvp + r;
-                    emit_fragment(zero, q.wq + unit * 4, (long)q.x6_Mvp * 4, fsc);
+        auto store = [&](const PackP& q, auto tr, const int c0, const int m0, const int (&slots)[kPackSlots], const float fsc) {
+            auto at = [&](int row, int ml) -> float {
+                return decltype(tr)::value ? lds[((row & ~31) + ml) * 33 + (row & 31)] : lds[row * 33 + ml];
+            };
+            auto slot_of = [&](int sl) { return sl == 0 ? slots[0] : (sl == 1 ? slots[1] : (sl == 2 ? slots[2] : slots[3])); };
+            const int s0 = slots[0];
+            if (!(q.skip & kPackF32)) {
+                for (int e = tid; e < ns * 1024; e += 256) {
+                    const int ml = e & 31, cl = (e >> 5) & 31, sl = e >> 10;
+                    const int c = c0 + cl;
+                    if (c < q.C) q.wp[((long)slot_of(sl) * q.C + c) * q.Mp + m0 + ml] = at(sl * 32 + cl, ml);
                 }
             }
-        }
-        if (q.wq && q.x6_mode > 1) {
-            const int IS = q.x6_mode, cpc = 16 / IS, nvc = 32 / cpc;
-            const int nug = (ns + IS - 1) / IS;
-            for (int e = tid; e < nug * nvc * 64; e += 256) {
-                const int ml = e & 31, g = (e >> 5) & 1;
-                const int r = e >> 6;
-                const int cv = r % nvc, ul = r / nvc;
-                const int cbase = c0 + cv * cpc;
-                if (cbase >= q.C) continue;
-                float v[8];
-#pragma unroll
-                for (int i = 0; i < 8; ++i) {
-                    const int kap = 8 * g + i;
-                    const int cl = cv * cpc + kap / IS, sl = ul * IS + kap % IS;
-                    v[i] = sl < ns ? lds[(sl * 32 + cl) * 33 + ml] : 0.f;
+            const bool x6 = q.wq && !(q.skip & kPackX6);
+            if (x6 && q.x6_mode == 1) {
+                for (int e = tid; e < ns * 128; e += 256) {
+                    const int ml = e & 31, oct = (e >> 5) & 3, sl = e >> 7;
+                    const int cb = c0 + oct * 8;
+                    if (cb >= q.C) continue;
+                    float v[8];
+#pragma unroll
+                    for (int i = 0; i < 8; ++i) v[i] = at(sl * 32 + oct * 8 + i, ml);
+                    const int slot = slot_of(sl);
+                    if (q.bf16x3) {
+                        const long unit3 = (long)q.q2a[slot] + (long)(cb >> 4) * q.q2n[slot] + (long)(((cb >> 3) & 1) * 3) * q.Mp + m0 + ml;
+                        emit_fragment_bf3(v, q.wq + unit3 * 4, (long)q.Mp * 4);
+                        continue;
+                    }
+                    const long unit = (long)q.q2a[slot] + (long)(cb >> 4) * q.q2n[slot] + (long)(((cb >> 3) & 1) * kX6P) * q.Mp + m0 + ml;
+                    emit_fragment(v, q.wq + unit * 4, (long)q.Mp * 4, fsc);
                 }
-                const long unit = ((long)(cbase / cpc) * q.x6_nu + (s0 / IS + ul)) * 2 * kX6P * q.Mp + (long)(g * kX6P) * q.Mp + m0 + ml;
-                emit_fragment(v, q.wq + unit * 4, (long)q.Mp * 4, fsc);
             }
+            if (x6 && q.x6_vs > 1) {
+                const int vs = q.x6_vs;
+                for (int e = tid; e < ns * 128; e += 256) {
+                    const int ml = e & 31, oct = (e >> 5) & 3, sl = e >> 7;
+                    const int cb = c0 + oct * 8;
+                    const int r = (m0 + ml) * vs + q.q2j[slot_of(sl)];
+                    if (cb >= q.C || r >= q.x6_Mvp) continue;
+                    float v[8];
+#pragma unroll
+                    for (int i = 0; i < 8; ++i) v[i] = at(sl * 32 + oct * 8 + i, ml);
+                    const int slot = slot_of(sl);
+                    const long unit = q.x6_vofs + q.vq2a[slot] + (long)(cb >> 4) * q.x6_U * 2 * kX6P * q.x6_Mvp + (long)(((cb >> 3) & 1) * kX6P) * q.x6_Mvp + r;
+                    emit_fragment(v, q.wq + unit * 4, (long)q.x6_Mvp * 4, fsc);
+                }
+                if (first) {
+                    const float zero[8] = {0.f, 0.f, 0.f, 0.f, 0.f, 0.f, 0.f, 0.f};
+                    for (int e = tid; e < q.vz_n * 128; e += 256) {
+                        const int ml = e & 31, oct = (e >> 5) & 3, zi = e >> 7;
+                        const int cb = c0 + oct * 8;
+                        const int r = (m0 + ml) * vs + q.vz_j[zi];
+                        if (cb >= q.C || r >= q.x6_Mvp) continue;
+                        const long unit = q.x6_vofs + (long)q.vz_u[zi] * 2 * kX6P * q.x6_Mvp + (long)(cb >> 4) * q.x6_U * 2 * kX6P * q.x6_Mvp +
+                                          (long)(((cb >> 3) & 1) * kX6P) * q.x6_Mvp + r;
+                        emit_fragment(zero, q.wq + unit * 4, (long)q.x6_Mvp * 4, fsc);
+                    }
+                }
+            }
+            if (x6 && q.x6_mode > 1) {
+                const int IS = q.x6_mode, cpc = 16 / IS, nvc = 32 / cpc;
+                const int nug = (ns + IS - 1) / IS;
+                for (int e = tid; e < nug * nvc * 64; e += 256) {
+                    const int ml = e & 31, g = (e >> 5) & 1;
+                    const int r = e >> 6;
+                    const int cv = r % nvc, ul = r / nvc;
+                    const int cbase = c0 + cv * cpc;
+                    if (cbase >= q.C) continue;
+                    float v[8];
+#pragma unroll
+                    for (int i = 0; i < 8; ++i) {
+                        const int kap = 8 * g + i;
+                        const int cl = cv * cpc + kap / IS, sl = ul * IS + kap % IS;
+                        v[i] = sl < ns ? at(sl * 32 + cl, ml) : 0.f;
+                    }
+                    const long unit = ((long)(cbase / cpc) * q.x6_nu + (s0 / IS + ul)) * 2 * kX6P * q.Mp + (long)(g * kX6P) * q.Mp + m0 + ml;
+                    emit_fragment(v, q.wq + unit * 4, (long)q.Mp * 4, fsc);
+                }
+            }
+        };
+        int own[kPackSlots];
+#pragma unroll
+        for (int j = 0; j < kPackSlots; ++j) own[j] = s0 + j;
+        store(q, std::false_type{}, c0, m0, own, piece_scale(q));
+        if (f) {
+            int theirs[kPackSlots];
+#pragma unroll
+            for (int j = 0; j < kPackSlots; ++j) theirs[j] = fslot[min(s0 + j, q.nslots - 1)];
+            store(*f, std::true_type{}, m0, c0, theirs, piece_scale(*f));
         }
         __syncthreads();
     }
@@ -570,6 +603,8 @@
     long rows, cols;
     long row_begin;
     long blk_begin;
+    int shared;
+    int fslot[kMaxTaps];
 };
 
 namespace {
@@ -646,11 +681,42 @@
     const int it = find_item(items, n, blockIdx.x, false);
     const PrepItem& p = items[it];
     const long t = (long)blockIdx.x - p.blk_begin;
+    if (p.shared) {
+        const bool fw = p.shared == 1;
+        pack_tile(fw ? p.fwd : p.bwd, t, lds, 0, 1, fw ? &p.bwd : &p.fwd, p.fslot);
+        return;
+    }
     const long nf = pack_tiles(p.fwd);
     if (t < nf) pack_tile(p.fwd, t, lds);
     else if (t - nf < pack_tiles(p.bwd)) pack_tile(p.bwd, t - nf, lds);
 }
 
+}
+
+static int pack_pair_shares(const PackP& a, const PackP& b, int* fslot) {
+    static const bool on = [] { const char* e = getenv("RH_PREP_SHARED"); return !(e && atoi(e) == 0); }();
+    if (!on || !pack_tiles(a) || !pack_tiles(b)) return 0;
+    if (a.nslots != b.nslots || a.nslots != a.k || a.k != b.k || a.C != b.M || a.M != b.C || a.m_major == b.m_major ||
+        a.w != b.w || a.scale != b.scale) return 0;
+    bool same = true;
+    for (int i = 0; i < a.nslots; ++i) same = same && a.kk[i] == b.kk[i];
+    const bool a_il = a.wq && a.x6_mode > 1, b_il = b.wq && b.x6_mode > 1;
+    if (a_il && b_il && !same) return 0;
+    const int walker = (b_il && !same) ? 2 : 1;
+    const PackP& w = walker == 1 ? a : b;
+    const PackP& f = walker == 1 ? b : a;
+    int at[kMaxTaps];
+    for (int i = 0; i < kMaxTaps; ++i) at[i] = -1;
+    for (int i = 0; i < f.nslots; ++i) {
+        if (f.kk[i] < 0 || f.kk[i] >= f.k || at[f.kk[i]] >= 0) return 0;
+        at[f.kk[i]] = i;
+    }
+    for (int i = 0; i < w.nslots; ++i) {
+        if (w.kk[i] < 0 || w.kk[i] >= w.k || at[w.kk[i]] < 0) return 0;
+        fslot[i] = at[w.kk[i]];
+        at[w.kk[i]] = -1;
+    }
+    return walker;
 }
 
 extern "C" int64_t rh_prep_item_bytes(void) { return (int64_t)sizeof(PrepItem); }
@@ -678,7 +744,9 @@
         p[i].row_begin = rows;
         p[i].blk_begin = blks;
         rows += p[i].rows;
-        for (const PackP* q : {&p[i].fwd, &p[i].bwd}) blks += pack_tiles(*q);
+        p[i].shared = pack_pair_shares(p[i].fwd, p[i].bwd, p[i].fslot);
+        if (p[i].shared) blks += pack_tiles(p[i].shared == 1 ? p[i].fwd : p[i].bwd);
+        else for (const PackP* q : {&p[i].fwd, &p[i].bwd}) blks += pack_tiles(*q);
     }
     long* tab = reinterpret_cast<long*>(p + n);
     for (int i = 0; i < n; ++i) { tab[i] = p[i].row_begin; tab[n + i] = p[i].blk_begin; }
@@ -687,9 +755,120 @@
     return RH_OK;
 }
 
+namespace {
+
+struct PackStamp { long gen = -1; unsigned long long capture = 0; };
+struct PackEntry {
+    PackP q;
+    long gen = 0;
+    PackStamp sec[2];
+    int users = 0;
+};
+struct PackGroup { std::vector<std::pair<const float*, int>> ops; };
+
+std::mutex g_pack_mu;
+std::unordered_map<const float*, PackEntry> g_pack_entries;
+std::unordered_map<const void*, PackGroup> g_pack_groups;
+long g_pack_gen = 0;
+std::atomic<long> g_pack_ondemand{0};
+std::atomic<bool> g_pack_any{false};
+
+unsigned long long capture_of(hipStream_t stream) {
+    hipStreamCaptureStatus st = hipStreamCaptureStatusNone;
+    unsigned long long id = 0;
+    if (hipStreamGetCaptureInfo(stream, &st, &id) != hipSuccess) { (void)hipGetLastError(); return 0; }
+    return st == hipStreamCaptureStatusActive ? (id ? id : ~0ull) : 0;
+}
+
+inline int sections_of(const PackP& q) { return q.total ? (kPackF32 | (q.wq ? kPackX6 : 0)) : 0; }
+
+}
+
+int rh_pack_ensure(const float* wp, int sections, hipStream_t stream) {
+    if (!wp || !g_pack_any.load(std::memory_order_acquire)) return RH_OK;
+    std::lock_guard<std::mutex> lock(g_pack_mu);
+    const auto it = g_pack_entries.find(wp);
+    if (it == g_pack_entries.end()) return RH_OK;
+    PackEntry& e = it->second;
+    const unsigned long long cap = capture_of(stream);
+    int stale = 0;
+    for (int s = 0; s < 2; ++s) {
+        const bool current = e.sec[s].gen == e.gen && (e.sec[s].capture == 0 || e.sec[s].capture == cap);
+        if ((sections & sections_of(e.q) & (1 << s)) && !current) stale |= 1 << s;
+    }
+    if (!stale) return RH_OK;
+    PackP a = e.q;
+    a.skip = ~stale & (kPackF32 | kPackX6);
+    const long tiles = pack_tiles(a);
+    if (tiles > 0) {
+        hipLaunchKernelGGL(pack_kernel, dim3((unsigned)tiles, pack_slot_groups(a, PackP{}, tiles)), dim3(256), 0, stream, a, PackP{});
+        if (int rc = rh_check_launch("conv1d_pack_on_demand")) return rc;
+    }
+    for (int s = 0; s < 2; ++s)
+        if (stale & (1 << s)) { e.sec[s].gen = e.gen; e.sec[s].capture = cap; }
+    g_pack_ondemand.fetch_add(1, std::memory_order_relaxed);
+    return RH_OK;
+}
+
+extern "C" int rh_prep_set_sections(void* item, int32_t which, int32_t sections) {
+    RH_REQUIRE(item && (which == 0 || which == 1) && (sections & ~(kPackF32 | kPackX6)) == 0, RH_ERR_INVALID, "prep_set_sections: bad arguments");
+    PackP& q = which == 0 ? ((PrepItem*)item)->fwd : ((PrepItem*)item)->bwd;
+    q.skip = ~sections & (kPackF32 | kPackX6);
+    return RH_OK;
+}
+
+extern "C" int32_t rh_prep_item_sections(const void* item, int32_t which) {
+    if (!item || (which != 0 && which != 1)) return 0;
+    return sections_of(which == 0 ? ((const PrepItem*)item)->fwd : ((const PrepItem*)item)->bwd);
+}
+
+extern "C" int rh_prep_bind(const void* items_host, int32_t n, const void* items_dev) {
+    RH_REQUIRE(items_host && items_dev && n >= 0, RH_ERR_INVALID, "prep_bind: bad arguments");
+    const PrepItem* p = (const PrepItem*)items_host;
+    std::lock_guard<std::mutex> lock(g_pack_mu);
+    RH_REQUIRE(!g_pack_groups.count(items_dev), RH_ERR_INVALID, "prep_bind: this device array is bound already");
+    PackGroup& g = g_pack_groups[items_dev];
+    for (int i = 0; i < n; ++i)
+        for (const PackP* q : {&p[i].fwd, &p[i].bwd}) {
+            if (!q->total) continue;
+            PackEntry& e = g_pack_entries[q->wp];
+            if (e.users++ == 0) { e.q = *q; e.q.skip = 0; }
+            g.ops.emplace_back(q->wp, q->skip);
+        }
+    g_pack_any.store(true, std::memory_order_release);
+    return RH_OK;
+}
+
+extern "C" int rh_prep_unbind(const void* items_dev) {
+    std::lock_guard<std::mutex> lock(g_pack_mu);
+    const auto it = g_pack_groups.find(items_dev);
+    if (it == g_pack_groups.end()) return RH_OK;
+    for (const auto& op : it->second.ops) {
+        const auto e = g_pack_entries.find(op.first);
+        if (e != g_pack_entries.end() && --e->second.users == 0) g_pack_entries.erase(e);
+    }
+    g_pack_groups.erase(it);
+    return RH_OK;
+}
+
+extern "C" int64_t rh_prep_on_demand_packs(void) { return (int64_t)g_pack_ondemand.load(std::memory_order_relaxed); }
+
 extern "C" int rh_prep_run_f32(const void* items_dev, int32_t n, int64_t total_rows, int64_t total_blocks,
                                rh_stream_t stream) {
     RH_REQUIRE(items_dev && n > 0, RH_ERR_INVALID, "prep_run: bad arguments");
+    {
+        std::lock_guard<std::mutex> lock(g_pack_mu);
+        const auto it = g_pack_groups.find(items_dev);
+        RH_REQUIRE(it != g_pack_groups.end(), RH_ERR_INVALID, "prep_run: the item array is not bound (rh_prep_bind)");
+        const unsigned long long cap = capture_of((hipStream_t)stream);
+        const long gen = ++g_pack_gen;
+        for (const auto& op : it->second.ops) {
+            PackEntry& e = g_pack_entries[op.first];
+            e.gen = gen;
+            for (int s = 0; s < 2; ++s)
+                if (!(op.second & (1 << s))) { e.sec[s].gen = gen; e.sec[s].capture = cap; }
+        }
+    }
     if (total_rows > 0) {
         hipLaunchKernelGGL(prep_scales_kernel, dim3((unsigned)total_rows), dim3(256), 0, (hipStream_t)stream,
                            (const PrepItem*)items_dev, n);
@@ -775,6 +954,7 @@
     RH_REQUIRE(x && wp_fwd && y, RH_ERR_INVALID, "conv1d_fwd: null pointer");
     RH_REQUIRE(d->act != RH_ACT_SNAKE || snake_alpha, RH_ERR_INVALID, "conv1d_fwd: snake needs alpha");
     if (rh_smallc_fwd_eligible(d, residual != nullptr)) {
+        if (int e = rh_pack_ensure(wp_fwd, kPackF32, (hipStream_t)stream)) return e;
         return rh_smallc_fwd(d, x, wp_fwd, bias, y, (hipStream_t)stream, p.out_range);
     }
     p.in = x; p.wp = wp_fwd; p.out = y; p.bias = bias; p.add = residual; p.mul_src = nullptr;
@@ -800,6 +980,7 @@
     RH_REQUIRE(d->act == RH_ACT_NONE || x, RH_ERR_INVALID, "conv1d_bwd_data: act needs the forward input");
     RH_REQUIRE(d->act != RH_ACT_SNAKE || snake_alpha, RH_ERR_INVALID, "conv1d_bwd_data: snake needs alpha");
     if (rh_smallc_dgrad_eligible(d, add != nullptr)) {
+        if (int e = rh_pack_ensure(wp_bwd, kPackF32, (hipStream_t)stream)) return e;
         TapPlan t;
         if (int e = build_plan(d, 1, &t)) return e;
         int slot_of_tap[kMaxTaps];
diff --git a/rave_amd/csrc/conv_igemm.hip b/rave_amd/csrc/conv_igemm.hip
--- a/rave_amd/csrc/conv_igemm.hip
+++ b/rave_amd/csrc/conv_igemm.hip
@@ -203,6 +203,7 @@
 
 int rh_conv_launch_sync(ConvP& p, hipStream_t stream, const char* what) {
     if (p.B <= 0 || p.ncols <= 0 || p.M <= 0) return RH_OK;
+    if (int e = rh_pack_ensure(p.wp, kPackF32, stream)) return e;
     int rc;
     if (p.M <= 32) rc = launch_cfg<1, 2, 1, 4>(p, stream, what);
     else if (p.M <= 64) rc = launch_cfg<2, 1, 1, 4>(p, stream, what);
diff --git a/rave_amd/csrc/conv_igemm_dma.hip b/rave_amd/csrc/conv_igemm_dma.hip
--- a/rave_amd/csrc/conv_igemm_dma.hip
+++ b/rave_amd/csrc/conv_igemm_dma.hip
@@ -519,6 +519,7 @@
         if (int e = rh_conv_launch_c2x(p, stream, what, &used)) return e;
         if (used) return rh_range_after(p, stream);
     }
+    if (int e = rh_pack_ensure(p.wp, kPackF32, stream)) return e;
     unsigned* const orange = p.out_range;
     p.out_range = nullptr;
     int rc;
diff --git a/rave_amd/csrc/conv_params.hpp b/rave_amd/csrc/conv_params.hpp
--- a/rave_amd/csrc/conv_params.hpp
+++ b/rave_amd/csrc/conv_params.hpp
@@ -103,7 +103,10 @@
     int kk[kMaxTaps];
     int q2a[kMaxTaps];
     int q2n[kMaxTaps];
+    int skip;
 };
+constexpr int kPackF32 = 1, kPackX6 = 2;
+int rh_pack_ensure(const float* wp, int sections, hipStream_t stream);
 int rh_pack_launch(const PackP& a, const PackP& b, hipStream_t stream, const char* what, const float* w = nullptr, long rows = 0,
                    long cols = 0);
 int64_t rh_bias_grad_workspace(int M);
diff --git a/rave_amd/csrc/conv_x6.hip b/rave_amd/csrc/conv_x6.hip
--- a/rave_amd/csrc/conv_x6.hip
+++ b/rave_amd/csrc/conv_x6.hip
@@ -260,6 +260,7 @@
     ConvP q = p;
     X6Plan pl{};
     if (!plan_x6(q, &pl)) return RH_OK;
+    if (int e = rh_pack_ensure(p.wp, kPackX6, stream)) return e;
     if (pl.part_bytes > 0 && (!ws || ws_bytes < pl.part_bytes || ((uintptr_t)ws & 15) || pl.part_bytes >= 0x7fffffffll)) {
         pl.ksplit = 1;
         pl.chunks_per_split = (q.C * q.is) >> 4;
@@ -324,5 +325,8 @@
     *used = false;
     C2X q;
     if (!x6_enabled() || !fill_c2x_from_1d(p, &q)) return RH_OK;
+    long v[8];
+    if (!rh_conv2d_x6_plan_query(q, v)) return RH_OK;
+    if (int e = rh_pack_ensure(p.wp, kPackX6, stream)) return e;
     return rh_conv2d_x6_launch(q, stream, what, used);
 }
diff --git a/rave_amd/csrc/unit_x6.hip b/rave_amd/csrc/unit_x6.hip
--- a/rave_amd/csrc/unit_x6.hip
+++ b/rave_amd/csrc/unit_x6.hip
@@ -376,6 +376,8 @@
     p.in_range = x_range; p.out_range = y_range; u.h_range = h ? h_range : nullptr;
     RH_REQUIRE((((uintptr_t)wp3_fwd | (uintptr_t)wp1_fwd) & 15) == 0 && ((uintptr_t)x & 3) == 0, RH_ERR_INVALID,
                "residual_unit_fwd: misaligned operand");
+    if (int e = rh_pack_ensure(wp3_fwd, kPackX6, (hipStream_t)stream)) return e;
+    if (int e = rh_pack_ensure(wp1_fwd, kPackX6, (hipStream_t)stream)) return e;
     p.in = x; p.wp = wp3_fwd; p.out = y; p.bias = nullptr; p.add = x; p.mul_src = nullptr;
     p.wq = reinterpret_cast<const unsigned*>(wp3_fwd + p.x6_wofs);
     p.in_alpha = nullptr; p.mul_alpha = nullptr;
diff --git a/rave_amd/prep.py b/rave_amd/prep.py
--- a/rave_amd/prep.py
+++ b/rave_amd/prep.py
@@ -1,6 +1,9 @@
 from __future__ import annotations
 
 import ctypes as C
+import dataclasses
+import os
+import weakref
 from typing import List
 
 import torch
@@ -8,7 +11,11 @@
 
 from . import _lib as L
 from . import cc
-from .ops import ConvGeom, _desc
+from .ops import ACT_LEAKY, ACT_NONE, ConvGeom, _desc
+
+SEC_F32, SEC_X6 = 1, 2
+
+_PLAN_BATCH, _PLAN_LEN = 2, 2048
 
 
 def _geom_of(m: nn.Module) -> ConvGeom:
@@ -21,16 +28,48 @@
     raise TypeError(type(m))
 
 
+def has_x6_section(g: ConvGeom, c_in: int, c_out: int, k: int, which: int) -> bool:
+    d = _desc(g, 1, c_in, c_out, 1, 1, k)
+    m, c = (c_out, c_in) if which == 0 else (c_in, c_out)
+    return L.lib.rh_conv1d_packed_floats(C.byref(d), which) > k * c * ((m + 31) // 32 * 32)
+
+
+def plan_sections(g: ConvGeom, c_in: int, c_out: int, k: int, which: int, has_bias: bool, all_sections: bool = False) -> int:
+    x6 = has_x6_section(g, c_in, c_out, k, which)
+    if all_sections or not x6:
+        return SEC_F32 | (SEC_X6 if x6 else 0)
+    l_in = _PLAN_LEN
+    on_x6 = True
+    for act in (ACT_NONE, ACT_LEAKY):
+        ga = dataclasses.replace(g, act=act)
+        d = _desc(ga, _PLAN_BATCH, c_in, c_out, l_in, ga.out_len(l_in, k), k)
+        for add in (0, 1):
+            on_x6 = on_x6 and L.lib.rh_conv1d_kernel_family(C.byref(d), which, int(has_bias and which == 0), add) == 1
+    return SEC_X6 | (0 if on_x6 else SEC_F32)
+
+
+class _Bound:
+
+    def __init__(self, items: torch.Tensor, bufs):
+        self.items, self.bufs = items, bufs
+        weakref.finalize(self, L.lib.rh_prep_unbind, items.data_ptr())
+
+
 class WeightPrep:
-    def __init__(self, model: nn.Module):
+    def __init__(self, model: nn.Module, all_sections: bool = False):
+        from .blocks import Snake
         self.mods: List[nn.Module] = [m for m in model.modules()
                                       if isinstance(m, (cc.Conv1d, cc.ConvTranspose1d, cc.PlainConv1d, cc.Conv2dK1))
                                       and getattr(m, "weight_g", None) is not None and m.groups == 1
                                       and m.weight_v.is_cuda]
         self.n = len(self.mods)
         self.bufs = []
+        self.sections = []
+        self.available = []
         if self.n == 0:
             return
+        all_sections = all_sections or os.environ.get("RH_PREP_ALL_SECTIONS", "0") != "0" \
+            or any(isinstance(m, Snake) for m in model.modules())
         isz = L.lib.rh_prep_item_bytes()
         host = (C.c_uint8 * L.lib.rh_prep_array_bytes(self.n))()
         dev = self.mods[0].weight_v.device
@@ -39,7 +78,8 @@
             k = v.shape[2]
             transposed = isinstance(m, cc.ConvTranspose1d)
             c_in, c_out = (v.shape[0], v.shape[1]) if transposed else (v.shape[1], v.shape[0])
-            d = _desc(_geom_of(m), 1, c_in, c_out, 1, 1, k)
+            geom = _geom_of(m)
+            d = _desc(geom, 1, c_in, c_out, 1, 1, k)
             dref = C.byref(d)
             rows = v.shape[0]
             ns = torch.empty(4, rows, device=dev, dtype=torch.float32)
@@ -48,11 +88,27 @@
             item = C.cast(C.byref(host, i * isz), C.c_void_p)
             L.check(L.lib.rh_prep_fill_item(dref, L.ptr(v), L.ptr(g), L.ptr(ns[0]), L.ptr(ns[1]), L.ptr(wp_f),
                                             L.ptr(wp_b), item), "prep_fill_item")
+            every = all_sections or isinstance(m, cc.Conv2dK1)
+            masks = tuple(plan_sections(geom, c_in, c_out, k, w, m.bias is not None, every) for w in (0, 1))
+            self.sections.append(masks)
+            self.available.append(tuple(L.lib.rh_prep_item_sections(item, w) for w in (0, 1)))
             self.bufs.append((wp_f, wp_b, ns[0], ns, v.data_ptr(), g.data_ptr()))
-        tr, tb = C.c_int64(0), C.c_int64(0)
-        L.check(L.lib.rh_prep_link(C.cast(host, C.c_void_p), self.n, C.byref(tr), C.byref(tb)), "prep_link")
-        self.total_rows, self.total_blocks = tr.value, tb.value
-        self.items = torch.frombuffer(bytearray(host), dtype=torch.uint8).to(dev)
+        self._tables = {}
+        for need_bwd in (True, False):
+            for i, masks in enumerate(self.sections):
+                item = C.cast(C.byref(host, i * isz), C.c_void_p)
+                L.check(L.lib.rh_prep_set_sections(item, 0, masks[0]), "prep_set_sections")
+                L.check(L.lib.rh_prep_set_sections(item, 1, masks[1] if need_bwd else 0), "prep_set_sections")
+            tr, tb = C.c_int64(0), C.c_int64(0)
+            L.check(L.lib.rh_prep_link(C.cast(host, C.c_void_p), self.n, C.byref(tr), C.byref(tb)), "prep_link")
+            items = torch.frombuffer(bytearray(host), dtype=torch.uint8).to(dev)
+            L.check(L.lib.rh_prep_bind(C.cast(host, C.c_void_p), self.n, items.data_ptr()), "prep_bind")
+            self._tables[need_bwd] = (_Bound(items, self.bufs), tr.value, tb.value)
+        bounds = tuple(t[0] for t in self._tables.values())
+        for b in self.bufs:
+            b[0]._rh_bound = b[1]._rh_bound = bounds
+        self.items = self._tables[True][0].items
+        self.total_rows, self.total_blocks = self._tables[True][1:]
 
     def _versions(self):
         return tuple((m.weight_v._version, m.weight_g._version) for m in self.mods)
@@ -67,10 +123,13 @@
             if m.weight_v.data_ptr() != b[4] or m.weight_g.data_ptr() != b[5]:
                 raise RuntimeError("rave_amd.WeightPrep: a parameter was re-allocated; rebuild the WeightPrep")
         capturing = torch.cuda.is_current_stream_capturing()
-        ver = self._versions()
-        if not reuse or capturing or ver != getattr(self, "_packed_versions", None):
-            L.check(L.lib.rh_prep_run_f32(self.items.data_ptr(), self.n, self.total_rows, self.total_blocks, L.stream()),
-                    "prep_run")
+        need_bwd = torch.is_grad_enabled()
+        ver = (self._versions(), need_bwd)
+        have = getattr(self, "_packed_versions", None)
+        fresh = have is not None and have[0] == ver[0] and (have[1] or not need_bwd)
+        if not reuse or capturing or not fresh:
+            bound, rows, blocks = self._tables[need_bwd]
+            L.check(L.lib.rh_prep_run_f32(bound.items.data_ptr(), self.n, rows, blocks, L.stream()), "prep_run")
             self._packed_versions = None if capturing else ver
         for m, b in zip(self.mods, self.bufs):
             m._prepacked = (b[0], b[1], b[2])
```
